# LabJunBMI/E3-invaraint-diffusion-model

Measured on AMD Instinct MI355X. Metric: denoising-steps/sec (batched pocket graphs), higher is better.
Workload: dtype f32 storage and accumulation, f16x3 products (fp32 grade); 1 GPU; structure_model sampling step, 256 x 256-residue pockets per GPU, 12+12 layers x 768, T=1000 schedule, encoder recomputed every step (as the reference); pockets_per_gpu=256, seq_len=256, parallelism=pocket-sharded x1, no collective

## Files before the change

e3-invaraint-diffusion-model_amd/blocks.py:

```python
import math

import torch
from torch import nn

import contextlib

from . import bert, keyed, ops
from .autograd import functional as F


class SELayer(nn.Module):

    def __init__(self, bert_config, mlp_ratio=4.0):
        super().__init__()
        h = bert_config.hidden_size
        self.norm1 = nn.LayerNorm(h, elementwise_affine=False)
        self.norm2 = nn.LayerNorm(h, elementwise_affine=False)
        self.adaLN_modulation = nn.Sequential(nn.Linear(h, h, bias=True), nn.SiLU(),
                                              nn.Linear(h, 6 * h, bias=True))
        self.attn = bert.BertAttention(bert_config)
        self.mlp = nn.Sequential(nn.Linear(h, int(h * mlp_ratio)), nn.GELU(),
                                 nn.Dropout(bert_config.hidden_dropout_prob),
                                 nn.Linear(int(h * mlp_ratio), h),
                                 nn.Dropout(bert_config.hidden_dropout_prob))
        nn.init.zeros_(self.adaLN_modulation[0].weight)
        nn.init.zeros_(self.adaLN_modulation[0].bias)

    def modulation(self, c):
        m0, m2 = self.adaLN_modulation[0], self.adaLN_modulation[2]
        return F.linear(F.linear(c, m0.weight, m0.bias, ops.ACT_SILU), m2.weight, m2.bias)

    def run(self, x, c, mask, B, L, mod=None, layout=None, row_keys=None):
        if mod is None:
            mod = self.modulation(c)
        if layout is not None:
            assert mod.shape[0] in (1, x.shape[0]), ("a packed batch takes per-token conditioning or one shared row",
                                                     tuple(mod.shape))
            assert bert.dropout_rates(self.attn) == (0.0, 0.0), "packed layouts are inference-only"
        rows_per_cond = x.shape[0] // mod.shape[0]
        assert rows_per_cond in (1, L, B * L) and rows_per_cond * mod.shape[0] == x.shape[0], (x.shape, mod.shape)
        drop = bert.dropout_rates(self.attn)
        if row_keys is not None:
            drop = drop + (row_keys,)
        att = bert.run_self_attention(self.attn, x, mask, B, L, drop, layout=layout)
        x = F.adaln_gate(x, att, mod, 0, rows_per_cond)
        h = F.dropout(F.linear(x, self.mlp[0].weight, self.mlp[0].bias, ops.ACT_GELU), self.mlp[2].p, self.training, row_keys)
        h = F.dropout(F.linear(h, self.mlp[3].weight, self.mlp[3].bias), self.mlp[4].p, self.training, row_keys)
        return F.adaln_gate(x, h, mod, 1, rows_per_cond)


class GaussianFourierProjection(nn.Module):

    def __init__(self, embed_dim=384, scale=2 * math.pi):
        super().__init__()
        self.register_buffer("W", torch.randn(embed_dim // 2) * scale)

    def forward(self, x):
        if x.ndim > 1:
            x = x.squeeze()
        elif x.ndim < 1:
            x = x.unsqueeze(0)
        if x.ndim < 1:
            x = x.unsqueeze(0)
        x_proj = x[:, None] * self.W[None, :] * 2 * torch.pi
        return torch.cat([torch.sin(x_proj), torch.cos(x_proj)], dim=-1)


class BertEmbeddings(nn.Module):

    def __init__(self, in_features, bert_config):
        super().__init__()
        self.linear = nn.Linear(in_features, bert_config.hidden_size)
        self.LayerNorm = nn.LayerNorm(bert_config.hidden_size, eps=bert_config.layer_norm_eps)
        self.dropout = nn.Dropout(bert_config.hidden_dropout_prob)

    def run(self, x2d, post_add=None, rows_per_add=1, row_keys=None):
        if self.training and self.dropout.p > 0:
            e = F.embed_layernorm(x2d, self.linear.weight, self.linear.bias, self.LayerNorm.weight,
                                  self.LayerNorm.bias, self.LayerNorm.eps, None, 1)
            e = F.dropout(e, self.dropout.p, row_keys=row_keys)
            if post_add is not None:
                e = (e.view(-1, rows_per_add, e.shape[1]) + post_add[:, None, :]).view_as(e)
            return e
        return F.embed_layernorm(x2d, self.linear.weight, self.linear.bias, self.LayerNorm.weight,
                                   self.LayerNorm.bias, self.LayerNorm.eps, post_add, rows_per_add)


class Predictor(nn.Module):

    def __init__(self, d_model, d_out, eps=1e-12):
        super().__init__()
        self.d_model, self.d_out = d_model, d_out
        self.dense1 = nn.Linear(d_model, d_model)
        self.layer_norm = nn.LayerNorm(d_model, eps=eps)
        self.dense2 = nn.Linear(d_model, d_out)

    def run(self, x):
        h = F.linear(x, self.dense1.weight, self.dense1.bias, ops.ACT_GELU)
        h = F.residual_layernorm(h, None, self.layer_norm.weight, self.layer_norm.bias, self.layer_norm.eps)
        return F.head_linear(h, self.dense2.weight, self.dense2.bias)


class KeyedDropoutSwitch:

    keyed_dropout = None

    def use_keyed_dropout(self, seed, epoch=None):
        if seed is None:
            self.keyed_dropout = None
            return None
        if epoch is None:
            epoch = keyed.epoch_word(next(self.parameters()).device)
        self.keyed_dropout = (keyed.check_seed(seed), epoch)
        return epoch

    def keyed_dropout_step(self, batch):
        cfgs = (self.encoder_config, self.decoder_config)
        acts = self.training and any(getattr(c, "hidden_dropout_prob", 0.0) > 0 or getattr(c, "attention_probs_dropout_prob", 0.0) > 0
                                     for c in cfgs)
        if self.keyed_dropout is None or not acts:
            return contextlib.nullcontext()
        seed, epoch = self.keyed_dropout
        return ops.keyed_dropout(seed, epoch, keyed.batch_item_ids(batch, batch["ligand_attn_mask"].shape[0]))


def drop_row_keys(stream, L):
    kd = ops.keyed_dropout_state()
    return None if kd is None else kd.row_keys(stream, L)


def flat2d(x):
    return x.reshape(-1, x.shape[-1]).contiguous().float()


def require_gpu(*tensors):
    for t in tensors:
        if t is not None and not t.is_cuda:
            raise RuntimeError("the denoiser runs on HIP kernels only: move the model and its inputs to a "
                               "GPU device (there is no CPU fallback; the CPU oracle lives in oracle/ and is "
                               "test infrastructure)")
```

e3-invaraint-diffusion-model_amd/csrc/gemm_split.hip:

```cpp
#include <type_traits>

#include "e3d_common.h"

namespace {

typedef __bf16 bf16x8 __attribute__((ext_vector_type(8)));
typedef __bf16 bf16x4 __attribute__((ext_vector_type(4)));
typedef _Float16 f16x8 __attribute__((ext_vector_type(8)));
typedef _Float16 f16x4 __attribute__((ext_vector_type(4)));

template <typename E> struct Vec;
template <> struct Vec<__bf16> { typedef bf16x8 x8; typedef bf16x4 x4; };
template <> struct Vec<_Float16> { typedef f16x8 x8; typedef f16x4 x4; };
__device__ __forceinline__ f32x16 mma16(const bf16x8 a, const bf16x8 b, const f32x16 c) {
    return __builtin_amdgcn_mfma_f32_32x32x16_bf16(a, b, c, 0, 0, 0);
}
__device__ __forceinline__ f32x16 mma16(const f16x8 a, const f16x8 b, const f32x16 c) {
    return __builtin_amdgcn_mfma_f32_32x32x16_f16(a, b, c, 0, 0, 0);
}

struct Epi { float* absmax; float scale; };

constexpr int BN = 128, BK = 32;
#ifdef GEMM_STAMPS
__device__ long long gemm_stamps[2][64][8];
#define GSTAMP(slot)                                                                                                    \
    do {                                                                                                                \
        if (stamp_on && kt < 64 && lane == 0) gemm_stamps[wid >> 2][kt][(slot)] = __builtin_readcyclecounter();         \
    } while (0)
#else
#define GSTAMP(slot) do {} while (0)
#endif
#ifndef E3D_GEMM_FRAG_PREFETCH
#define E3D_GEMM_FRAG_PREFETCH 1
#endif
constexpr int ROW_B = 64;
__device__ __forceinline__ int swz_off(int row, int chunk) { return row * ROW_B + ((chunk ^ ((row >> 2) & 3)) << 4); }

template <int NS, typename E>
__device__ __forceinline__ void split4(const f32x4 v, typename Vec<E>::x4 (&parts)[NS]) {
    f32x4 r = v;
#pragma unroll
    for (int s = 0; s < NS; ++s) {
#pragma unroll
        for (int j = 0; j < 4; ++j) {
            const E p = (E)r[j];
            parts[s][j] = p;
            r[j] -= (float)p;
        }
    }
}

template <>
__device__ __forceinline__ void split4<2, _Float16>(const f32x4 v, f16x4 (&parts)[2]) {
    e3d_f16x2 h0, l0, h1, l1;
    e3d_split2_f16(v[0], v[1], h0, l0);
    e3d_split2_f16(v[2], v[3], h1, l1);
    parts[0] = f16x4{h0[0], h0[1], h1[0], h1[1]};
    parts[1] = f16x4{l0[0], l0[1], l1[0], l1[1]};
}

#ifndef GEMM_LAB_RAW
#define GEMM_LAB_RAW 0
#endif
template <int ROWS, bool KMAJ, int NT = 512, bool RAW = false>
struct Stager {
    static constexpr int NV = ROWS * 8 / NT;
    const float* src[NV];
    int off[NV];
    int64_t ld;
    int kbase[NV];
    int roff[NV];

    __device__ __forceinline__ void init(const float* base, int64_t ld_, int row0, int row_limit, int tid) {
        ld = ld_;
#pragma unroll
        for (int i = 0; i < NV; ++i) {
            const int f = tid + NT * i;
            int r, kg;
            if (KMAJ) { r = f % ROWS; kg = f / ROWS; }
            else { r = f >> 3; kg = f & 7; }
            int gr = row0 + r;
            gr = gr < row_limit ? gr : row_limit - 1;
            src[i] = KMAJ ? base : base + (int64_t)gr * ld + kg * 4;
            kbase[i] = KMAJ ? __builtin_amdgcn_readfirstlane(kg * 4) : kg * 4;
            roff[i] = gr;
            off[i] = swz_off(r, kg >> 1) + (kg & 1) * 8;
        }
    }
    __device__ __forceinline__ void load(f32x4 (&v)[NV], int k0, int K) const {
#pragma unroll
        for (int i = 0; i < NV; ++i) {
            if (KMAJ) {
#pragma unroll
                for (int j = 0; j < 4; ++j) {
                    const int k = min(k0 + kbase[i] + j, K - 1);
                    v[i][j] = (src[i] + (int64_t)k * ld)[roff[i]];
                }
            } else {
                v[i] = *reinterpret_cast<const f32x4*>(src[i] + k0);
            }
        }
    }
    __device__ __forceinline__ void load_item(int i, f32x4& v, int k0, int K) const {
        if (KMAJ) {
#pragma unroll
            for (int j = 0; j < 4; ++j) {
                const int k = min(k0 + kbase[i] + j, K - 1);
                v[j] = (src[i] + (int64_t)k * ld)[roff[i]];
            }
        } else {
            v = *reinterpret_cast<const f32x4*>(src[i] + k0);
        }
    }
    template <int NS, typename E>
    __device__ __forceinline__ void store_item(int i, const f32x4& vin, unsigned char* img, int part_bytes, int k0, int K) const {
        f32x4 v = vin;
        if (KMAJ) {
#pragma unroll
            for (int j = 0; j < 4; ++j) v[j] = k0 + kbase[i] + j < K ? v[j] : 0.f;
        }
        typename Vec<E>::x4 p[NS];
        if constexpr (RAW && NS == 2) {
            typedef float f32x2_ __attribute__((ext_vector_type(2)));
            p[0] = __builtin_bit_cast(typename Vec<E>::x4, f32x2_{v[0], v[1]});
            p[1] = __builtin_bit_cast(typename Vec<E>::x4, f32x2_{v[2], v[3]});
        } else {
            split4<NS, E>(v, p);
        }
#pragma unroll
        for (int s = 0; s < NS; ++s) *reinterpret_cast<typename Vec<E>::x4*>(img + s * part_bytes + off[i]) = p[s];
    }
    __device__ __forceinline__ float masked_sum(int i, const f32x4& v, int k0, int K) const {
        float t[4];
#pragma unroll
        for (int j = 0; j < 4; ++j) t[j] = (!KMAJ || k0 + kbase[i] + j < K) ? v[j] : 0.f;
        return (t[0] + t[1]) + (t[2] + t[3]);
    }
    template <int NS, typename E>
    __device__ __forceinline__ void store(const f32x4 (&v)[NV], unsigned char* img, int part_bytes, int k0, int K) const {
#pragma unroll
        for (int i = 0; i < NV; ++i) store_item<NS, E>(i, v[i], img, part_bytes, k0, K);
    }
};

static inline bool e3d_tr_span_ok(int64_t k_len, int64_t ld) {
    return k_len > 0 && ld > 0 && ld < ((int64_t)1 << 24) && k_len * ld * 4 < ((int64_t)1 << 31);
}

template <int ROWS, int NT>
struct StagerT {
    static constexpr int NV = ROWS * 8 / NT;
    static constexpr int PITCH = ROWS * 2, Q = ROWS / 4, KSTEP = NT / Q;
    static_assert(KSTEP * NV == 32, "a k-tile is 32 k-rows");
    const float* ubase;
    int64_t ld;
    int kk0, n4, lim;
    int voff[NV];

    __device__ __forceinline__ void init(const float* base, int64_t ld_, int row0, int row_limit, int tid) {
        ld = ld_;
        ubase = base;
        lim = row_limit;
        n4 = tid % Q;
        kk0 = tid / Q;
        const int gr = min(row0 + 4 * n4, row_limit - 4);
#pragma unroll
        for (int i = 0; i < NV; ++i) voff[i] = (int)(((int64_t)kk(i) * ld + gr) * 4);
    }
    __device__ __forceinline__ int kk(int i) const { return kk0 + KSTEP * i; }
    __device__ __forceinline__ int off(int i) const {
        const int k = kk(i);
        return k * PITCH + (((n4 >> 2) ^ (2 * (k & 3))) << 5) + (n4 & 3) * 8;
    }
    __device__ __forceinline__ __amdgpu_buffer_rsrc_t tile_rsrc(int k0, int K) const {
        return __builtin_amdgcn_make_buffer_rsrc(const_cast<float*>(ubase + (int64_t)k0 * ld), 0,
                                                 (int)(((int64_t)(K - 1 - k0) * ld + lim) * 4), 0x00020000);
    }
    __device__ __forceinline__ void load_item(int i, f32x4& v, int k0, int K) const {
        v = __builtin_bit_cast(f32x4, __builtin_amdgcn_raw_buffer_load_b128(tile_rsrc(k0, K), voff[i], 0, 0));
    }
    __device__ __forceinline__ void load(f32x4 (&v)[NV], int k0, int K) const {
        const auto r = tile_rsrc(k0, K);
#pragma unroll
        for (int i = 0; i < NV; ++i) v[i] = __builtin_bit_cast(f32x4, __builtin_amdgcn_raw_buffer_load_b128(r, voff[i], 0, 0));
    }
    __device__ __forceinline__ f32x4 masked(int, const f32x4& v, int k0, int K) const { return k0 < K ? v : f32x4{0.f, 0.f, 0.f, 0.f}; }
    template <int NS, typename E>
    __device__ __forceinline__ void store_item(int i, const f32x4& v, unsigned char* img, int part_bytes, int, int) const {
        typename Vec<E>::x4 p[NS];
        split4<NS, E>(v, p);
        const int o = off(i);
#pragma unroll
        for (int s = 0; s < NS; ++s) *reinterpret_cast<typename Vec<E>::x4*>(img + s * part_bytes + o) = p[s];
    }
    template <int NS, typename E>
    __device__ __forceinline__ void store(const f32x4 (&v)[NV], unsigned char* img, int part_bytes, int k0, int K) const {
#pragma unroll
        for (int i = 0; i < NV; ++i) store_item<NS, E>(i, v[i], img, part_bytes, k0, K);
    }
    __device__ __forceinline__ float masked_sum(int, const f32x4&, int, int) const { return 0.f; }
};

__device__ __forceinline__ int tr_lane_off(int pitch, int r0, int lane) {
    const int q = (lane >> 2) & 3, g = (lane >> 4) & 1, half = lane >> 5;
    return (4 * half + q) * pitch + ((((r0 >> 4) + g) ^ (2 * q)) << 5) + 8 * (lane & 3);
}
template <typename X8>
__device__ __forceinline__ X8 tr_frag8(const unsigned char* img, int pitch, int lane_off, int ks) {
    typedef short short4v __attribute__((ext_vector_type(4)));
    typedef short short8v __attribute__((ext_vector_type(8)));
    typedef __attribute__((address_space(3))) short4v* lds_p;
    const unsigned char* p0 = img + 16 * ks * pitch + lane_off;
    const short4v a = __builtin_amdgcn_ds_read_tr16_b64_v4i16((lds_p)(p0));
    const short4v b = __builtin_amdgcn_ds_read_tr16_b64_v4i16((lds_p)(p0 + 8 * pitch));
    const short8v c = __builtin_shufflevector(a, b, 0, 1, 2, 3, 4, 5, 6, 7);
    return __builtin_bit_cast(X8, c);
}

template <int NS, int ACT, bool A_KMAJ, bool B_KMAJ, int WM, int WN, typename E, int TN = 2, bool TR = false>
__device__ __forceinline__ void gemm_split_body(unsigned char* smem_raw, const float* __restrict__ A, int64_t lda,
                                                const float* __restrict__ Bm, int64_t ldb,
                                                const float* __restrict__ bias, float* __restrict__ out, int64_t ldc,
                                                int M, int N, int K_total, int tiles_m, int tiles_n, int k_chunk,
                                                int bx, int by, int ny, float* __restrict__ colsum_out, int accumulate,
                                                float* __restrict__ absmax = nullptr, float out_scale = 1.0f) {
    constexpr int NBUF = NS <= 2 ? 2 : 1;
    constexpr int BM = WM * 64, BN = WN * 32 * TN, NT = WM * WN * 64;
    constexpr int A_BYTES = BM * ROW_B, B_BYTES = BN * ROW_B;
    constexpr int BUF_BYTES = NS * (A_BYTES + B_BYTES);

    const int k_begin = by * k_chunk;
    const int K = min(K_total, k_begin + k_chunk);
    const bool split = ny > 1;
    const int lid = bx;
    const int tm = lid / tiles_n, tn = lid % tiles_n;
    const int row0 = tm * BM, col0 = tn * BN;

    const int tid = threadIdx.x, lane = tid & 63, wid = tid >> 6;
    const int wr = wid / WN, wc = wid % WN;
    const int l31 = lane & 31, half = lane >> 5;

    static_assert(!TR || (A_KMAJ && B_KMAJ), "the transposing staging exists for the K-major x K-major layout");
    typedef typename std::conditional<TR, StagerT<BM, NT>, Stager<BM, A_KMAJ, NT, (GEMM_LAB_RAW & 1) && !A_KMAJ && !B_KMAJ>>::type SA;
    typedef typename std::conditional<TR, StagerT<BN, NT>, Stager<BN, B_KMAJ, NT, (GEMM_LAB_RAW & 2) && !A_KMAJ && !B_KMAJ>>::type SB;
    SA sa;
    SB sb;
    sa.init(A, lda, row0, M, tid);
    sb.init(Bm, ldb, col0, N, tid);

    f32x16 acc[2][TN];
#pragma unroll
    for (int m = 0; m < 2; ++m)
#pragma unroll
        for (int n = 0; n < TN; ++n)
#pragma unroll
            for (int r = 0; r < 16; ++r) acc[m][n][r] = 0.f;

    f32x4 ra[SA::NV], rb[SB::NV];
    f32x4 ra1[SA::NV], rb1[SB::NV];
    constexpr bool CS = A_KMAJ && B_KMAJ;
    float cs[SA::NV];
    f32x4 cs4 = {0.f, 0.f, 0.f, 0.f};
#pragma unroll
    for (int i = 0; i < SA::NV; ++i) cs[i] = 0.f;
    auto cs_add = [&](int i, const f32x4& v, int k0) {
        if constexpr (TR) cs4 += sa.masked(i, v, k0, K);
        else cs[i] += sa.masked_sum(i, v, k0, K);
    };
    sa.load(ra, k_begin, K);
    sb.load(rb, k_begin, K);
    if (CS) {
#pragma unroll
        for (int i = 0; i < SA::NV; ++i) cs_add(i, ra[i], k_begin);
    }
    sa.template store<NS, E>(ra, smem_raw, A_BYTES, k_begin, K);
    sb.template store<NS, E>(rb, smem_raw + NS * A_BYTES, B_BYTES, k_begin, K);
    __syncthreads();

    const int nk = (K - k_begin + BK - 1) / BK;
    const int a_row = wr * 64 + l31, b_row = wc * (32 * TN) + l31;
    int cur = 0;
    constexpr bool PIPE = NBUF == 2;
    constexpr int NA_ = SA::NV, NB_ = SB::NV;
    constexpr bool DEEP = PIPE && ((!A_KMAJ && !B_KMAJ) || TR);
    int tr_a[2], tr_b[TN];
    if constexpr (TR) {
#pragma unroll
        for (int m = 0; m < 2; ++m) tr_a[m] = tr_lane_off(2 * BM, wr * 64 + 32 * m, lane);
#pragma unroll
        for (int n = 0; n < TN; ++n) tr_b[n] = tr_lane_off(2 * BN, wc * (32 * TN) + 32 * n, lane);
    }
    if (DEEP) {
        const int k1 = k_begin + (nk > 1 ? BK : 0), k2 = k_begin + (nk > 2 ? 2 : (nk > 1 ? 1 : 0)) * BK;
        sa.load(ra1, k1, K);
        sb.load(rb1, k1, K);
        sa.load(ra, k2, K);
        sb.load(rb, k2, K);
    } else if (PIPE) {
        const int k1 = k_begin + (nk > 1 ? BK : 0);
        sa.load(ra, k1, K);
        sb.load(rb, k1, K);
    }
#ifdef GEMM_STAMPS
    const bool stamp_on = bx == GEMM_STAMPS && by == 0 && (wid & 3) == 0;
#endif
    auto k_step = [&](int kt, f32x4 (&xa)[NA_], f32x4 (&xb)[NB_]) {
        const bool more = kt + 1 < nk;
        GSTAMP(0);
        if (!PIPE && more) {
            sa.load(xa, k_begin + (kt + 1) * BK, K);
            sb.load(xb, k_begin + (kt + 1) * BK, K);
        }
        constexpr int AHEAD = DEEP ? 3 : 2;
        const int k2 = k_begin + (kt + AHEAD < nk ? kt + AHEAD : nk - 1) * BK;
        unsigned char* nxt = smem_raw + (cur ^ 1) * BUF_BYTES;
        const unsigned char* ab = smem_raw + cur * BUF_BYTES;
        const unsigned char* bb = smem_raw + cur * BUF_BYTES + NS * A_BYTES;
        constexpr bool PREF = PIPE && TN == 1 && E3D_GEMM_FRAG_PREFETCH;
        typename Vec<E>::x8 fa2[2][NS][2], fb2[2][NS][TN];
#pragma unroll
        for (int ks = 0; ks < (PREF ? 2 : 0); ++ks)
#pragma unroll
            for (int s = 0; s < NS; ++s) {
#pragma unroll
                for (int m = 0; m < 2; ++m)
                    fa2[ks][s][m] = *reinterpret_cast<const typename Vec<E>::x8*>(ab + s * A_BYTES + swz_off(a_row + 32 * m, 2 * ks + half));
#pragma unroll
                for (int n = 0; n < TN; ++n)
                    fb2[ks][s][n] = *reinterpret_cast<const typename Vec<E>::x8*>(bb + s * B_BYTES + swz_off(b_row + 32 * n, 2 * ks + half));
            }
#ifdef GEMM_STAMPS
        if (PREF) { asm volatile("s_waitcnt lgkmcnt(0)" ::: "memory"); GSTAMP(1); }
#endif
#pragma unroll
        for (int ks = 0; ks < 2; ++ks) {
            typename Vec<E>::x8 fa[NS][2], fb[NS][TN];
#pragma unroll
            for (int s = 0; s < NS; ++s) {
#pragma unroll
                for (int m = 0; m < 2; ++m) {
                    if constexpr (TR) fa[s][m] = tr_frag8<typename Vec<E>::x8>(ab + s * A_BYTES, 2 * BM, tr_a[m], ks);
                    else fa[s][m] = PREF ? fa2[ks][s][m]
                                         : *reinterpret_cast<const typename Vec<E>::x8*>(ab + s * A_BYTES + swz_off(a_row + 32 * m, 2 * ks + half));
                }
#pragma unroll
                for (int n = 0; n < TN; ++n) {
                    if constexpr (TR) fb[s][n] = tr_frag8<typename Vec<E>::x8>(bb + s * B_BYTES, 2 * BN, tr_b[n], ks);
                    else fb[s][n] = PREF ? fb2[ks][s][n]
                                         : *reinterpret_cast<const typename Vec<E>::x8*>(bb + s * B_BYTES + swz_off(b_row + 32 * n, 2 * ks + half));
                }
            }
#pragma unroll
            for (int m = 0; m < 2; ++m) {
                if (PIPE) {
                    const int g = ks * 2 + m;
#pragma unroll
                    for (int i = 0; i < NA_; ++i)
                        if (i * 4 / NA_ == g) {
                            if (CS) cs_add(i, xa[i], k_begin + (kt + 1) * BK);
                            sa.template store_item<NS, E>(i, xa[i], nxt, A_BYTES, k_begin + (kt + 1) * BK, K);
                            sa.load_item(i, xa[i], k2, K);
                        }
#pragma unroll
                    for (int i = 0; i < NB_; ++i)
                        if (i * 4 / NB_ == g) {
                            sb.template store_item<NS, E>(i, xb[i], nxt + NS * A_BYTES, B_BYTES, k_begin + (kt + 1) * BK, K);
                            sb.load_item(i, xb[i], k2, K);
                        }
                }
#pragma unroll
                for (int n = 0; n < TN; ++n) {
                    if constexpr (NS == 3) {
                        acc[m][n] = mma16(fa[1][m], fb[1][n], acc[m][n]);
                        acc[m][n] = mma16(fa[0][m], fb[NS - 1][n], acc[m][n]);
                        acc[m][n] = mma16(fa[NS - 1][m], fb[0][n], acc[m][n]);
                    }
                    if constexpr (NS >= 2) {
                        acc[m][n] = mma16(fa[0][m], fb[1][n], acc[m][n]);
                        acc[m][n] = mma16(fa[1][m], fb[0][n], acc[m][n]);
                    }
                    acc[m][n] = mma16(fa[0][m], fb[0][n], acc[m][n]);
                }
                if (PIPE) __builtin_amdgcn_sched_barrier(0);
            }
        }
        GSTAMP(2);
        if (PIPE) {
#ifdef GEMM_STAMPS
            asm volatile("s_waitcnt vmcnt(0) lgkmcnt(0)" ::: "memory");
            GSTAMP(3);
#endif
            __syncthreads();
            GSTAMP(4);
            cur ^= 1;
        } else {
            __syncthreads();
            if (more) {
                if (CS) {
#pragma unroll
                    for (int i = 0; i < SA::NV; ++i) cs_add(i, xa[i], k_begin + (kt + 1) * BK);
                }
                sa.template store<NS, E>(xa, smem_raw, A_BYTES, k_begin + (kt + 1) * BK, K);
                sb.template store<NS, E>(xb, smem_raw + NS * A_BYTES, B_BYTES, k_begin + (kt + 1) * BK, K);
            }
            __syncthreads();
        }
        };
    for (int kt = 0; kt < nk; kt += 2) {
        if constexpr (DEEP) {
            k_step(kt, ra1, rb1);
            if (kt + 1 < nk) k_step(kt + 1, ra, rb);
        } else {
            k_step(kt, ra, rb);
            if (kt + 1 < nk) k_step(kt + 1, ra, rb);
        }
    }
    unsigned amax = 0;
#pragma unroll
    for (int n = 0; n < TN; ++n) {
        const int col = col0 + wc * (32 * TN) + n * 32 + l31;
        const float bv = (bias && col < N && by == 0) ? bias[col] : 0.f;
#pragma unroll
        for (int m = 0; m < 2; ++m) {
#pragma unroll
            for (int r = 0; r < 16; ++r) {
                const int row = row0 + wr * 64 + m * 32 + mfma32_row(r, half);
                float v = fmaf(acc[m][n][r], out_scale, bv);
                if (ACT == E3D_ACT_GELU) v = gelu_erf(v);
                if (ACT == E3D_ACT_SILU) v = silu(v);
                if (row < M && col < N) {
                    float* o = out + (int64_t)row * ldc + col;
                    if (split) atomicAdd(o, v);
                    else *o = accumulate ? *o + v : v;
                    if (ACT == E3D_ACT_NONE && absmax) e3d_absmax_accum(amax, v);
                }
            }
        }
    }
    if (ACT == E3D_ACT_NONE && absmax) e3d_absmax_commit(amax, absmax, lane);
    if (CS && colsum_out && tn == 0) {
        float* red = reinterpret_cast<float*>(smem_raw);
        if constexpr (TR) {
            static_assert(SA::KSTEP == 8, "8 partial sums per row, as in the dword scheme");
#pragma unroll
            for (int j = 0; j < 4; ++j) red[sa.kk0 * BM + 4 * sa.n4 + j] = cs4[j];
        } else {
#pragma unroll
            for (int i = 0; i < SA::NV; ++i) {
                const int f = tid + NT * i;
                red[(f / BM) * BM + f % BM] = cs[i];
            }
        }
        __syncthreads();
        if (tid < BM && row0 + tid < M) {
            float v = 0.f;
#pragma unroll
            for (int g = 0; g < 8; ++g) v += red[g * BM + tid];
            float* o = colsum_out + row0 + tid;
            if (split) atomicAdd(o, v);
            else *o = accumulate ? *o + v : v;
        }
    }
}

template <int NS, int ACT, bool A_KMAJ, bool B_KMAJ, int WM, int WN, typename E, int TN = 2, bool TR = false>
__global__ __launch_bounds__(WM * WN * 64) void gemm_split_kernel(const float* __restrict__ A, int64_t lda,
                                                         const float* __restrict__ Bm, int64_t ldb,
                                                         const float* __restrict__ bias,
                                                         float* __restrict__ out, int64_t ldc, int M,
                                                         int N, int K_total, int tiles_m, int tiles_n,
                                                         int k_chunk, float* __restrict__ absmax, float out_scale) {
    extern __shared__ __attribute__((aligned(16))) unsigned char smem_raw[];
    gemm_split_body<NS, ACT, A_KMAJ, B_KMAJ, WM, WN, E, TN, TR>(smem_raw, A, lda, Bm, ldb, bias, out, ldc, M, N, K_total, tiles_m,
                                                        tiles_n, k_chunk, xcd_remap(blockIdx.x, tiles_m * tiles_n),
                                                        blockIdx.y, gridDim.y, nullptr, 0, absmax, out_scale);
}

struct WgradGroup {
    const float* dz[64];
    const float* x[64];
    float* dw[64];
    float* db[64];
    unsigned long long accumulate;
};

template <int NS, bool TR>
__global__ __launch_bounds__(512) void gemm_wgrad_grouped_kernel(const WgradGroup g, int64_t ldz, int64_t ldx, int N, int K,
                                                                 int M, int tiles_m, int tiles_n, int count) {
    extern __shared__ __attribute__((aligned(16))) unsigned char smem_raw[];
    const int tiles = tiles_m * tiles_n;
    const int lid = xcd_remap(blockIdx.x, tiles * count);
    const int p = lid / tiles;
    gemm_split_body<NS, E3D_ACT_NONE, true, true, 4, 2, __bf16, 2, TR>(smem_raw, g.dz[p], ldz, g.x[p], ldx, nullptr, g.dw[p], K,
                                                                        N, K, M, tiles_m, tiles_n, M, lid - p * tiles, 0, 1,
                                                                        g.db[p], (int)((g.accumulate >> p) & 1));
}

struct WgradRagged {
    const float* dz[64];
    const float* x[64];
    float* dw[64];
    float* db[64];
    int N[64], K[64], ldz[64], ldx[64];
    int tile_start[65];
    unsigned long long accumulate;
};
static_assert(sizeof(WgradRagged) <= 3400, "kernel arguments are limited to 4 KB");

template <int NS, bool TR>
__global__ __launch_bounds__(512) void gemm_wgrad_ragged_kernel(const WgradRagged g, int M, int count) {
    extern __shared__ __attribute__((aligned(16))) unsigned char smem_raw[];
    const int lid = xcd_remap(blockIdx.x, g.tile_start[count]);
    int lo = 0, hi = count;
    while (hi - lo > 1) {
        const int mid = (lo + hi) >> 1;
        if (g.tile_start[mid] <= lid) lo = mid;
        else hi = mid;
    }
    const int p = lo, N = g.N[p], K = g.K[p];
    const int tiles_m = (N + 255) / 256, tiles_n = (K + 127) / 128;
    gemm_split_body<NS, E3D_ACT_NONE, true, true, 4, 2, __bf16, 2, TR>(smem_raw, g.dz[p], (int64_t)g.ldz[p], g.x[p], (int64_t)g.ldx[p],
                                                                        nullptr, g.dw[p], K, N, K, M, tiles_m, tiles_n, M,
                                                                        lid - g.tile_start[p], 0, 1, g.db[p],
                                                                        (int)((g.accumulate >> p) & 1));
}

constexpr int BT = 256, ROW64 = ROW_B;

#ifdef E3D_STAMPS
__device__ long long e3d_stamps[2][32][8];
#define STAMP(slot)                                                                              \
    do {                                                                                         \
        if (stamp_on && kt < 32 && lane == 0) e3d_stamps[wr][kt][slot] = __builtin_readcyclecounter(); \
    } while (0)
#define STAMP_K(i)                                                                               \
    do {                                                                                         \
        if (blockIdx.x == 300 && (threadIdx.x & 255) == 0) e3d_stamps[threadIdx.x >> 8][i][7] = __builtin_readcyclecounter(); \
    } while (0)
#else
#define STAMP(slot) do {} while (0)
#define STAMP_K(i) do {} while (0)
#endif

template <int NS, int ACT, int WR, int WC, int NBUF, bool PIPE, typename E>
__global__ __launch_bounds__(WR * WC * 64, 2) void gemm_split256_kernel(const float* __restrict__ A, int64_t lda,
                                                                        const float* __restrict__ W,
                                                                        const float* __restrict__ bias,
                                                                        float* __restrict__ out, int64_t ldc,
                                                                        int M, int N, int K, int tiles_m,
                                                                        int tiles_n, float* __restrict__ absmax, float out_scale) {
    static_assert(!PIPE || NBUF == 2, "PIPE needs two LDS buffers");
    STAMP_K(0);
    extern __shared__ __attribute__((aligned(16))) unsigned char smem_raw[];
    constexpr int NT = WR * WC * 64, TM = WR * 128, TN = WC * 64;
    constexpr int A_BYTES = TM * ROW64, B_BYTES = TN * ROW64;
    constexpr int BUF_BYTES = NS * (A_BYTES + B_BYTES);
    constexpr int NA = TM * 8 / NT, NB = TN * 8 / NT;
    constexpr int NI = NA + NB;

    const int lid = xcd_remap(blockIdx.x, tiles_m * tiles_n);
    const int tm = lid / tiles_n, tn = lid % tiles_n;
    const int row0 = tm * TM, col0 = tn * TN;
    const int tid = threadIdx.x, lane = tid & 63, wid = tid >> 6;
    const int wr = wid / WC, wc = wid % WC;
    const int l31 = lane & 31, half = lane >> 5;

    const float* src[NI];
    int dst[NI];
#pragma unroll
    for (int i = 0; i < NI; ++i) {
        const bool is_a = i < NA;
        const int f = tid + NT * (is_a ? i : i - NA), r = f >> 3, kg = f & 7;
        if (is_a) {
            int ar = row0 + r;
            ar = ar < M ? ar : M - 1;
            src[i] = A + (int64_t)ar * lda + kg * 4;
        } else {
            src[i] = W + (int64_t)(col0 + r) * K + kg * 4;
        }
        dst[i] = (is_a ? 0 : NS * A_BYTES) + swz_off(r, kg >> 1) + (kg & 1) * 8;
    }

    f32x16 acc[4][2];
#pragma unroll
    for (int m = 0; m < 4; ++m)
#pragma unroll
        for (int n = 0; n < 2; ++n)
#pragma unroll
            for (int r = 0; r < 16; ++r) acc[m][n][r] = 0.f;

    f32x4 rg[NI];
    auto item_load = [&](int i, int kt) { rg[i] = *reinterpret_cast<const f32x4*>(src[i] + kt * BK); };
    auto item_store = [&](int i, unsigned char* buf) {
        typename Vec<E>::x4 p[NS];
        split4<NS, E>(rg[i], p);
#pragma unroll
        for (int s = 0; s < NS; ++s)
            *reinterpret_cast<typename Vec<E>::x4*>(buf + s * (i < NA ? A_BYTES : B_BYTES) + dst[i]) = p[s];
    };

    STAMP_K(1);
    const int nk = K / BK;
#pragma unroll
    for (int i = 0; i < NI; ++i) item_load(i, 0);
#pragma unroll
    for (int i = 0; i < NI; ++i) item_store(i, smem_raw);
    if (PIPE) {
#pragma unroll
        for (int i = 0; i < NI; ++i) item_load(i, nk > 1 ? 1 : 0);
    }
    __syncthreads();

    int a_row[4], b_row[2];
#pragma unroll
    for (int m = 0; m < 4; ++m) a_row[m] = wr * 128 + m * 32 + l31;
#pragma unroll
    for (int n = 0; n < 2; ++n) b_row[n] = wc * 64 + n * 32 + l31;
    STAMP_K(2);
    int cur = 0;
#ifdef E3D_STAMPS
    const bool stamp_on = blockIdx.x == 300 && (wid & 3) == 0;
#endif
    for (int kt = 0; kt < nk; ++kt) {
        const bool more = kt + 1 < nk;
        STAMP(0);
        if (!PIPE && more) {
#pragma unroll
            for (int i = 0; i < NI; ++i) item_load(i, kt + 1);
        }
        STAMP(1);
        const unsigned char* base = smem_raw + cur * BUF_BYTES;
        unsigned char* next = smem_raw + (cur ^ 1) * BUF_BYTES;
        const int kt2 = kt + 2 < nk ? kt + 2 : nk - 1;
#pragma unroll
        for (int ks = 0; ks < 2; ++ks) {
            typename Vec<E>::x8 fa[NS][4], fb[NS][2];
#pragma unroll
            for (int s = 0; s < NS; ++s) {
#pragma unroll
                for (int n = 0; n < 2; ++n)
                    fb[s][n] = *reinterpret_cast<const typename Vec<E>::x8*>(base + NS * A_BYTES + s * B_BYTES +
                                                                swz_off(b_row[n], 2 * ks + half));
#pragma unroll
                for (int m = 0; m < 4; ++m)
                    fa[s][m] = *reinterpret_cast<const typename Vec<E>::x8*>(base + s * A_BYTES + swz_off(a_row[m], 2 * ks + half));
            }
#pragma unroll
            for (int m = 0; m < 4; ++m) {
                if (PIPE) {
                    const int g = ks * 4 + m;
#pragma unroll
                    for (int i = 0; i < NI; ++i)
                        if (i * 8 / NI == g) {
                            item_store(i, next);
                            item_load(i, kt2);
                        }
                }
#pragma unroll
                for (int n = 0; n < 2; ++n) {
                    if constexpr (NS == 3) {
                        acc[m][n] = mma16(fa[1][m], fb[1][n], acc[m][n]);
                        acc[m][n] = mma16(fa[0][m], fb[NS - 1][n], acc[m][n]);
                        acc[m][n] = mma16(fa[NS - 1][m], fb[0][n], acc[m][n]);
                    }
                    if constexpr (NS >= 2) {
                        acc[m][n] = mma16(fa[0][m], fb[1][n], acc[m][n]);
                        acc[m][n] = mma16(fa[1][m], fb[0][n], acc[m][n]);
                    }
                    acc[m][n] = mma16(fa[0][m], fb[0][n], acc[m][n]);
                }
                if (PIPE) __builtin_amdgcn_sched_barrier(0);
            }
            STAMP(2 + ks);
        }
        if (PIPE) {
            STAMP(5);
            __syncthreads();
            STAMP(6);
            cur ^= 1;
        } else if (NBUF == 2) {
#ifdef E3D_STAMPS
            asm volatile("s_waitcnt vmcnt(0)" ::: "memory");
            STAMP(4);
#endif
            if (more) {
#pragma unroll
                for (int i = 0; i < NI; ++i) item_store(i, next);
            }
            STAMP(5);
            __syncthreads();
            STAMP(6);
            cur ^= 1;
        } else {
            __syncthreads();
            if (more) {
#pragma unroll
                for (int i = 0; i < NI; ++i) item_store(i, smem_raw);
            }
            __syncthreads();
        }
    }

    STAMP_K(3);
    unsigned amax = 0;
#pragma unroll
    for (int m = 0; m < 4; ++m) {
#pragma unroll
        for (int n = 0; n < 2; ++n) {
            const int col = col0 + wc * 64 + n * 32 + l31;
            const float bv = bias ? bias[col] : 0.f;
#pragma unroll
            for (int r = 0; r < 16; ++r) {
                const int row = row0 + wr * 128 + m * 32 + mfma32_row(r, half);
                float v = fmaf(acc[m][n][r], out_scale, bv);
                if (ACT == E3D_ACT_GELU) v = gelu_erf(v);
                if (ACT == E3D_ACT_SILU) v = silu(v);
                if (row < M) {
                    out[(int64_t)row * ldc + col] = v;
                    if (ACT == E3D_ACT_NONE && absmax) e3d_absmax_accum(amax, v);
                }
            }
        }
    }
    if (ACT == E3D_ACT_NONE && absmax) e3d_absmax_commit(amax, absmax, lane);
    STAMP_K(4);
#ifdef E3D_STAMPS
    asm volatile("s_waitcnt vmcnt(0)" ::: "memory");
    STAMP_K(5);
#endif
}

#ifdef E3D_NT_STORES
#define E3D_STORE_OUT(ptr, val) __builtin_nontemporal_store((val), (ptr))
#else
#define E3D_STORE_OUT(ptr, val) (*(ptr) = (val))
#endif

template <int ACT, typename E>
__global__ __launch_bounds__(512, 2) void gemm_split256p_kernel(const float* __restrict__ A, int64_t lda,
                                                                 const float* __restrict__ W,
                                                                 const float* __restrict__ bias,
                                                                 float* __restrict__ out, int64_t ldc, int N, int K,
                                                                 int tiles_m, int tiles_n, float* __restrict__ absmax, float out_scale) {
    extern __shared__ __attribute__((aligned(16))) unsigned char smem_raw[];
    constexpr int NS = 2, T_BYTES = BT * ROW64, BUF_BYTES = 2 * NS * T_BYTES;
    constexpr int NI = 8;
    const int total = tiles_m * tiles_n, nk = K / BK;
    const int tid = threadIdx.x, lane = tid & 63, wid = tid >> 6;
    const int wr = wid >> 2, wc = wid & 3;
    const int l31 = lane & 31, half = lane >> 5;

    unsigned goff[NI];
    int dst[NI];
#pragma unroll
    for (int i = 0; i < NI; ++i) {
        const int f = tid + 512 * (i & 3), r = f >> 3, kg = f & 7;
        goff[i] = (unsigned)(r * (i < 4 ? (int)lda : K) + kg * 4);
        dst[i] = (i < 4 ? 0 : NS * T_BYTES) + swz_off(r, kg >> 1) + (kg & 1) * 8;
    }

    int ld_tile = blockIdx.x, ld_k = 0;
    const float* ld_a;
    const float* ld_w;
    auto cursor_bases = [&]() {
        const int lid = xcd_remap(ld_tile, total);
        ld_a = A + (int64_t)(lid / tiles_n) * BT * lda + ld_k * BK;
        ld_w = W + (int64_t)(lid % tiles_n) * BT * K + ld_k * BK;
    };
    auto cursor_advance = [&]() {
        if (ld_k + 1 < nk) {
            ++ld_k;
            ld_a += BK;
            ld_w += BK;
        } else if (ld_tile + (int)gridDim.x < total) {
            ld_tile += gridDim.x;
            ld_k = 0;
            cursor_bases();
        }
    };
    f32x4 rg[NI];
    auto item_load = [&](int i) { rg[i] = *reinterpret_cast<const f32x4*>((i < 4 ? ld_a : ld_w) + goff[i]); };
    auto item_store = [&](int i, unsigned char* buf) {
        typename Vec<E>::x4 p[NS];
        split4<NS, E>(rg[i], p);
#pragma unroll
        for (int s = 0; s < NS; ++s) *reinterpret_cast<typename Vec<E>::x4*>(buf + s * T_BYTES + dst[i]) = p[s];
    };
    cursor_bases();
#pragma unroll
    for (int i = 0; i < NI; ++i) item_load(i);
    cursor_advance();
#pragma unroll
    for (int i = 0; i < NI; ++i) item_store(i, smem_raw);
#pragma unroll
    for (int i = 0; i < NI; ++i) item_load(i);
    cursor_advance();
    __syncthreads();

    int a_row[4], b_row[2];
#pragma unroll
    for (int m = 0; m < 4; ++m) a_row[m] = wr * 128 + m * 32 + l31;
#pragma unroll
    for (int n = 0; n < 2; ++n) b_row[n] = wc * 64 + n * 32 + l31;
    int cur = 0;
    unsigned amax = 0;

    for (int tile = blockIdx.x; tile < total; tile += gridDim.x) {
        f32x16 acc[4][2];
#pragma unroll
        for (int m = 0; m < 4; ++m)
#pragma unroll
            for (int n = 0; n < 2; ++n)
#pragma unroll
                for (int r = 0; r < 16; ++r) acc[m][n][r] = 0.f;
        for (int kt = 0; kt < nk; ++kt) {
            const unsigned char* base = smem_raw + cur * BUF_BYTES;
            unsigned char* next = smem_raw + (cur ^ 1) * BUF_BYTES;
#pragma unroll
            for (int ks = 0; ks < 2; ++ks) {
                typename Vec<E>::x8 fa[NS][4], fb[NS][2];
#pragma unroll
                for (int s = 0; s < NS; ++s) {
#pragma unroll
                    for (int n = 0; n < 2; ++n)
                        fb[s][n] = *reinterpret_cast<const typename Vec<E>::x8*>(base + (NS + s) * T_BYTES +
                                                                    swz_off(b_row[n], 2 * ks + half));
#pragma unroll
                    for (int m = 0; m < 4; ++m)
                        fa[s][m] = *reinterpret_cast<const typename Vec<E>::x8*>(base + s * T_BYTES + swz_off(a_row[m], 2 * ks + half));
                }
#pragma unroll
                for (int m = 0; m < 4; ++m) {
                    const int g = ks * 4 + m;
                    item_store(g, next);
                    item_load(g);
#pragma unroll
                    for (int n = 0; n < 2; ++n) {
                        acc[m][n] = mma16(fa[0][m], fb[1][n], acc[m][n]);
                        acc[m][n] = mma16(fa[1][m], fb[0][n], acc[m][n]);
                        acc[m][n] = mma16(fa[0][m], fb[0][n], acc[m][n]);
                    }
                    __builtin_amdgcn_sched_barrier(0);
                }
            }
            cursor_advance();
            __syncthreads();
            cur ^= 1;
        }

        const int lid = xcd_remap(tile, total);
        const int row0 = (lid / tiles_n) * BT, col0 = (lid % tiles_n) * BT;
#pragma unroll
        for (int m = 0; m < 4; ++m) {
#pragma unroll
            for (int n = 0; n < 2; ++n) {
                const int col = col0 + wc * 64 + n * 32 + l31;
                const float bv = bias ? bias[col] : 0.f;
                float* o = out + (int64_t)(row0 + wr * 128 + m * 32 + 4 * half) * ldc + col;
#pragma unroll
                for (int r = 0; r < 16; ++r) {
                    float v = fmaf(acc[m][n][r], out_scale, bv);
                    if (ACT == E3D_ACT_GELU) v = gelu_erf(v);
                    if (ACT == E3D_ACT_SILU) v = silu(v);
                    E3D_STORE_OUT(&o[(int64_t)((r & 3) + 8 * (r >> 2)) * ldc], v);
                    if (ACT == E3D_ACT_NONE && absmax) e3d_absmax_accum(amax, v);
                }
            }
        }
    }
    if (ACT == E3D_ACT_NONE && absmax) e3d_absmax_commit(amax, absmax, lane);
}

template <int ACT, typename E>
int launch256p(const float* A, int64_t lda, const float* W, const float* bias, float* out, int64_t ldc, int M, int N,
               int K, Epi epi, hipStream_t s) {
    const int tiles_m = M / BT, tiles_n = N / BT;
    constexpr size_t lds = 2 * 2 * 2 * BT * ROW64;
    static std::atomic<uint64_t> lds_ok{0};
    const int n_cu = e3d_cu_count();
    const int total = tiles_m * tiles_n;
    e3d_allow_lds(lds_ok, gemm_split256p_kernel<ACT, E>, lds);
    hipLaunchKernelGGL((gemm_split256p_kernel<ACT, E>), dim3(total < n_cu ? total : n_cu), dim3(512), lds, s, A, lda, W, bias, out,
                       ldc, N, K, tiles_m, tiles_n, epi.absmax, epi.scale);
    return e3d_launch_status("e3d_gemm_f32_split (persistent 256x256)");
}

int g_general_form = -1;
int g_tile_pref = -1;

template <int NS, int ACT, int WR, int WC, int NBUF, bool PIPE, typename E>
int launch256(const float* A, int64_t lda, const float* W, const float* bias, float* out, int64_t ldc, int M, int N,
              int K, Epi epi, hipStream_t s) {
    constexpr int TM = WR * 128, TN = WC * 64;
    const int tiles_m = (M + TM - 1) / TM, tiles_n = N / TN;
    const size_t lds = (size_t)NBUF * NS * (TM + TN) * ROW64;
    static std::atomic<uint64_t> lds_ok{0};
    e3d_allow_lds(lds_ok, gemm_split256_kernel<NS, ACT, WR, WC, NBUF, PIPE, E>, lds);
    hipLaunchKernelGGL((gemm_split256_kernel<NS, ACT, WR, WC, NBUF, PIPE, E>), dim3(tiles_m * tiles_n), dim3(WR * WC * 64), lds, s,
                       A, lda, W, bias, out, ldc, M, N, K, tiles_m, tiles_n, epi.absmax, epi.scale);
    return e3d_launch_status("e3d_gemm_f32_split (128x64 wave tiles)");
}

template <int NS, int ACT, bool A_KMAJ, bool B_KMAJ, int WM, int WN, typename E, int TN = 2, bool TR = false>
int launch_general(const float* A, int64_t lda, const float* B, int64_t ldb, const float* bias, float* out, int64_t ldc,
                   int M, int N, int K, Epi epi, hipStream_t s);

int p_min() {
    static int v = 0;
    if (!v) {
        const char* e = getenv("E3D_GEMM_P_MIN");
        v = e ? atoi(e) : 160;
    }
    return v;
}

template <int NS, int ACT, bool A_KMAJ, bool B_KMAJ, typename E>
int launch(const float* A, int64_t lda, const float* B, int64_t ldb, const float* bias, float* out, int64_t ldc,
           int M, int N, int K, Epi epi, hipStream_t s) {
    if (g_tile_pref < 0) {
        const char* e = getenv("E3D_GEMM_TILE");
        g_tile_pref = e ? atoi(e) : 4;
    }
    if constexpr (!A_KMAJ && !B_KMAJ) {
        if constexpr (NS == 2) {
            const int64_t n_tiles = (int64_t)(M / BT) * (N / BT);
            if (N % BT == 0 && M % BT == 0 && ldb == K && g_tile_pref >= 4 && K >= 2 * BK && lda < (1 << 22) &&
                (g_tile_pref >= 5 || n_tiles >= p_min() || (n_tiles >= 96 && N >= 6 * BT && !getenv("E3D_GEMM_P_MIN"))))
                return launch256p<ACT, E>(A, lda, B, bias, out, ldc, M, N, K, epi, s);
            if (N % BT == 0 && ldb == K && g_tile_pref >= 3 && (int64_t)((M + BT - 1) / BT) * (N / BT) >= 256)
                return launch256<NS, ACT, 2, 4, 2, true, E>(A, lda, B, bias, out, ldc, M, N, K, epi, s);
        }
        if constexpr (NS == 1) {
            if (N % BT == 0 && ldb == K && g_tile_pref >= 3 && (int64_t)((M + BT - 1) / BT) * (N / BT) >= 160)
                return launch256<NS, ACT, 2, 4, 2, true, E>(A, lda, B, bias, out, ldc, M, N, K, epi, s);
        }
        if (N % BT == 0 && ldb == K && g_tile_pref >= 1 &&
            (int64_t)((M + BT - 1) / BT) * (N / BT) >= 256)
            return launch256<NS, ACT, 2, 4, (NS <= 2 ? 2 : 1), false, E>(A, lda, B, bias, out, ldc, M, N, K, epi, s);
    }
    if (g_general_form < 0) {
        const char* e = getenv("E3D_GEMM_FORM");
        g_general_form = e ? atoi(e) : 0;
    }
    int form = g_general_form;
    if (form != 1 && form != 2 && form != 3 && form != 4) {
        const int64_t g256 = (int64_t)((M + 255) / 256) * ((N + 127) / 128), g128 = (int64_t)((M + 127) / 128) * ((N + 127) / 128);
        const int64_t cus = e3d_cu_count();
        if (NS == 3) form = g256 < 128 && !A_KMAJ && !B_KMAJ ? 2 : 1;
        else if (A_KMAJ && B_KMAJ) form = 1;
        else if (A_KMAJ) form = g128 <= cus ? 2 : (g256 <= cus ? 1 : (45 * ((g128 + 2 * cus - 1) / (2 * cus)) < 37 * ((g256 + cus - 1) / cus) ? 2 : 1));
        else form = 25 * ((g128 + cus - 1) / cus) <= 38 * ((g256 + cus - 1) / cus) ? 3 : 1;
        if (NS == 2 && !A_KMAJ && !B_KMAJ && M <= 2048 && N <= 1024) form = 4;
    }
    if constexpr (NS == 2 && !A_KMAJ && !B_KMAJ) {
        if (form == 4) return launch_general<NS, ACT, A_KMAJ, B_KMAJ, 2, 2, E, 1>(A, lda, B, ldb, bias, out, ldc, M, N, K, epi, s);
    }
    if (form == 4) form = 3;
    if constexpr (NS <= 2 && !A_KMAJ) {
        if (form == 3) return launch_general<NS, ACT, A_KMAJ, B_KMAJ, 2, 4, E, 1>(A, lda, B, ldb, bias, out, ldc, M, N, K, epi, s);
    }
    if (form == 3) form = 2;
    if (form == 2) return launch_general<NS, ACT, A_KMAJ, B_KMAJ, 2, 2, E>(A, lda, B, ldb, bias, out, ldc, M, N, K, epi, s);
    if constexpr (A_KMAJ && B_KMAJ) {
        static const bool tr_on = !getenv("E3D_WGRAD_TR") || atoi(getenv("E3D_WGRAD_TR")) != 0;
        if (tr_on && M % 4 == 0 && N % 4 == 0 && lda % 4 == 0 && ldb % 4 == 0 && ((uintptr_t)A % 16) == 0 && ((uintptr_t)B % 16) == 0 &&
            e3d_tr_span_ok(K, lda) && e3d_tr_span_ok(K, ldb))
            return launch_general<NS, ACT, A_KMAJ, B_KMAJ, 4, 2, E, 2, true>(A, lda, B, ldb, bias, out, ldc, M, N, K, epi, s);
    }
    return launch_general<NS, ACT, A_KMAJ, B_KMAJ, 4, 2, E>(A, lda, B, ldb, bias, out, ldc, M, N, K, epi, s);
}

template <int NS, int ACT, bool A_KMAJ, bool B_KMAJ, int WM, int WN, typename E, int TN, bool TR>
int launch_general(const float* A, int64_t lda, const float* B, int64_t ldb, const float* bias, float* out, int64_t ldc,
                   int M, int N, int K, Epi epi, hipStream_t s) {
    constexpr int BM = WM * 64, BNt = WN * 32 * TN;
    const int tiles_m = (M + BM - 1) / BM, tiles_n = (N + BNt - 1) / BNt;
    constexpr int NBUF = NS <= 2 ? 2 : 1;
    size_t lds = (size_t)NBUF * NS * (BM + BNt) * ROW_B;
    static const bool spread = !getenv("E3D_GEMM_SPREAD") || atoi(getenv("E3D_GEMM_SPREAD")) != 0;
    if (spread && BM * BNt == 128 * 128 && (int64_t)tiles_m * tiles_n <= e3d_cu_count() && lds < (size_t)84 * 1024) lds = (size_t)84 * 1024;
    static std::atomic<uint64_t> lds_ok{0};
    e3d_allow_lds(lds_ok, gemm_split_kernel<NS, ACT, A_KMAJ, B_KMAJ, WM, WN, E, TN, TR>, (size_t)84 * 1024 > lds ? (size_t)84 * 1024 : lds);
    int splits = 1;
    const int resident = e3d_cu_count() * (WM * WN >= 8 ? 1 : 2);
    if (A_KMAJ && B_KMAJ && ACT == E3D_ACT_NONE && tiles_m * tiles_n * 2 < resident && K >= 1024) {
        splits = resident / (tiles_m * tiles_n);
        splits = splits > 16 ? 16 : splits;
        while (splits > 1 && K / splits < 256) --splits;
    }
    int k_chunk = K;
    if (splits > 1) {
        k_chunk = ((K + splits - 1) / splits + BK - 1) / BK * BK;
        splits = (K + k_chunk - 1) / k_chunk;
        hipError_t e = hipSuccess;
        if (ldc == N) e = e3d_zero_async(out, (size_t)M * N, s);
        else {
            hipLaunchKernelGGL(e3d_zero2d_kernel, dim3(1024), dim3(256), 0, s, out, (size_t)ldc, (size_t)M, (size_t)N);
            e = hipGetLastError();
        }
        if (e != hipSuccess) {
            e3d_set_error("gemm_split: split-K memset failed: %s", hipGetErrorString(e));
            return (int)e;
        }
    }
    hipLaunchKernelGGL((gemm_split_kernel<NS, ACT, A_KMAJ, B_KMAJ, WM, WN, E, TN, TR>), dim3(tiles_m * tiles_n, splits),
                       dim3(WM * WN * 64), lds, s, A, lda, B, ldb, bias, out, ldc, M, N, K, tiles_m, tiles_n, k_chunk,
                       splits > 1 ? nullptr : epi.absmax, epi.scale);
    return e3d_launch_status("e3d_gemm_f32_split");
}

template <int NS, typename E>
int dispatch(int act, bool a_kmaj, bool b_kmaj, const float* A, int64_t lda, const float* B, int64_t ldb,
             const float* bias, float* out, int64_t ldc, int M, int N, int K, Epi epi, hipStream_t s) {
    if (!a_kmaj && !b_kmaj) {
        switch (act) {
            case E3D_ACT_NONE: return launch<NS, E3D_ACT_NONE, false, false, E>(A, lda, B, ldb, bias, out, ldc, M, N, K, epi, s);
            case E3D_ACT_GELU: return launch<NS, E3D_ACT_GELU, false, false, E>(A, lda, B, ldb, bias, out, ldc, M, N, K, epi, s);
            case E3D_ACT_SILU: return launch<NS, E3D_ACT_SILU, false, false, E>(A, lda, B, ldb, bias, out, ldc, M, N, K, epi, s);
        }
        e3d_set_error("gemm_split: unknown activation %d", act);
        return -1;
    }
    if (act != E3D_ACT_NONE) {
        e3d_set_error("gemm_split: activations are only fused for the forward (K-contiguous) layout");
        return -1;
    }
    if (!a_kmaj && b_kmaj) return launch<NS, E3D_ACT_NONE, false, true, __bf16>(A, lda, B, ldb, bias, out, ldc, M, N, K, epi, s);
    if (a_kmaj && b_kmaj) return launch<NS, E3D_ACT_NONE, true, true, __bf16>(A, lda, B, ldb, bias, out, ldc, M, N, K, Epi{nullptr, epi.scale}, s);
    return launch<NS, E3D_ACT_NONE, true, false, __bf16>(A, lda, B, ldb, bias, out, ldc, M, N, K, epi, s);
}

}

#ifdef GEMM_STAMPS
extern "C" int e3d_debug_gemm_stamps(long long* t) { return (int)hipMemcpyFromSymbol(t, HIP_SYMBOL(gemm_stamps), sizeof(long long) * 2 * 64 * 8); }
#endif

#ifdef E3D_STAMPS
extern "C" int e3d_debug_read_stamps(long long* host_out) {
    return (int)hipMemcpyFromSymbol(host_out, HIP_SYMBOL(e3d_stamps), sizeof(long long) * 2 * 32 * 8);
}
#endif

extern "C" int e3d_gemm_kernel_select(int pref) {
    if (g_tile_pref < 0) {
        const char* e = getenv("E3D_GEMM_TILE");
        g_tile_pref = e ? atoi(e) : 4;
    }
    const int prev = g_tile_pref;
    if (pref >= 0) g_tile_pref = pref;
    return prev;
}

extern "C" int e3d_gemm_general_select(int form) {
    if (g_general_form < 0) {
        const char* e = getenv("E3D_GEMM_FORM");
        g_general_form = e ? atoi(e) : 0;
    }
    const int prev = g_general_form;
    if (form >= 0) g_general_form = form;
    return prev;
}

static int gemm_split_general(const float* A, int64_t lda, int a_kmajor, const float* B, int64_t ldb, int b_kmajor,
                              const float* bias, float* out, int64_t ldc, int M, int N, int K, int act, int terms,
                              float* absmax, float out_scale, void* stream) {
    const Epi epi{absmax, out_scale};
    E3D_REQUIRE(out_scale == 1.0f || !(a_kmajor && b_kmajor), "gemm_split: out_scale is not available for the split-K layout");
    E3D_REQUIRE(A && B && out, "gemm_split: null pointer");
    E3D_REQUIRE(M > 0 && N > 0 && K > 0, "gemm_split: bad shape M=%d N=%d K=%d", M, N, K);
    E3D_REQUIRE(terms == E3D_TERMS_BF16 || terms == 3 || terms == 6 || terms == E3D_TERMS_F16X3,
                "gemm_split: terms must be 1, 3, 6 or 19 (got %d)", terms);
    E3D_REQUIRE(ldc >= N, "gemm_split: ldc=%lld < N=%d", (long long)ldc, N);
    if (!a_kmajor) E3D_REQUIRE(lda >= K && lda % 4 == 0 && K % BK == 0 && ((uintptr_t)A % 16) == 0,
                               "gemm_split: K-contiguous A needs K%%32==0, lda%%4==0, 16B alignment (K=%d lda=%lld)", K, (long long)lda);
    else E3D_REQUIRE(lda >= M, "gemm_split: K-major A needs lda >= M");
    if (!b_kmajor) E3D_REQUIRE(ldb >= K && ldb % 4 == 0 && K % BK == 0 && ((uintptr_t)B % 16) == 0,
                               "gemm_split: K-contiguous B needs K%%32==0, ldb%%4==0, 16B alignment (K=%d ldb=%lld)", K, (long long)ldb);
    else E3D_REQUIRE(ldb >= N, "gemm_split: K-major B needs ldb >= N");
    hipStream_t s = (hipStream_t)stream;
    E3D_REQUIRE(!absmax || (!(a_kmajor && b_kmajor) && act == E3D_ACT_NONE),
                "gemm_split: out_absmax exists for act = none and not for the split-K (weight-gradient) layout");
    if (terms == E3D_TERMS_BF16) return dispatch<1, __bf16>(act, a_kmajor != 0, b_kmajor != 0, A, lda, B, ldb, bias, out, ldc, M, N, K, epi, s);
    if (terms == 3) return dispatch<2, __bf16>(act, a_kmajor != 0, b_kmajor != 0, A, lda, B, ldb, bias, out, ldc, M, N, K, epi, s);
    if (terms == E3D_TERMS_F16X3) {
        if (!a_kmajor && !b_kmajor) return dispatch<2, _Float16>(act, false, false, A, lda, B, ldb, bias, out, ldc, M, N, K, epi, s);
        return dispatch<3, __bf16>(act, a_kmajor != 0, b_kmajor != 0, A, lda, B, ldb, bias, out, ldc, M, N, K, epi, s);
    }
    return dispatch<3, __bf16>(act, a_kmajor != 0, b_kmajor != 0, A, lda, B, ldb, bias, out, ldc, M, N, K, epi, s);
}

extern "C" int e3d_gemm_f32_split_general(const float* A, int64_t lda, int a_kmajor, const float* B,
                                          int64_t ldb, int b_kmajor, const float* bias, float* out,
                                          int64_t ldc, int M, int N, int K, int act, int terms,
                                          void* stream) {
    return gemm_split_general(A, lda, a_kmajor, B, ldb, b_kmajor, bias, out, ldc, M, N, K, act, terms, nullptr, 1.0f, stream);
}

extern "C" int e3d_gemm_wgrad_grouped_f32_split(const float* const* dz, const float* const* x, float* const* dw,
                                                float* const* db, uint64_t accumulate_bits, int count, int64_t ldz,
                                                int64_t ldx, int N, int K, int M, int terms, void* stream) {
    E3D_REQUIRE(dz && x && dw && count >= 1 && count <= 64, "gemm_wgrad_grouped: 1..64 problems (count=%d)", count);
    E3D_REQUIRE(M > 0 && N > 0 && K > 0 && ldz >= N && ldx >= K, "gemm_wgrad_grouped: bad shape N=%d K=%d M=%d ldz=%lld ldx=%lld",
                N, K, M, (long long)ldz, (long long)ldx);
    E3D_REQUIRE(terms == E3D_TERMS_BF16 || terms == 3 || terms == 6 || terms == E3D_TERMS_F16X3,
                "gemm_wgrad_grouped: terms must be 1, 3, 6 or 19 (got %d)", terms);
    WgradGroup g;
    for (int p = 0; p < 64; ++p) {
        const int q = p < count ? p : 0;
        E3D_REQUIRE(dz[q] && x[q] && dw[q], "gemm_wgrad_grouped: null pointer in problem %d", q);
        g.dz[p] = dz[q]; g.x[p] = x[q]; g.dw[p] = dw[q]; g.db[p] = db ? db[q] : nullptr;
    }
    g.accumulate = accumulate_bits;
    static const bool tr_on = !getenv("E3D_WGRAD_TR") || atoi(getenv("E3D_WGRAD_TR")) != 0;
    bool tr = tr_on && N % 4 == 0 && K % 4 == 0 && ldz % 4 == 0 && ldx % 4 == 0 && e3d_tr_span_ok(M, ldz) && e3d_tr_span_ok(M, ldx);
    for (int p = 0; p < count && tr; ++p) tr = ((uintptr_t)dz[p] % 16) == 0 && ((uintptr_t)x[p] % 16) == 0;
    const int tiles_m = (N + 255) / 256, tiles_n = (K + 127) / 128;
    E3D_REQUIRE((int64_t)tiles_m * tiles_n * count < (1ll << 30), "gemm_wgrad_grouped: too many tiles");
    const dim3 grid(tiles_m * tiles_n * count), block(512);
    hipStream_t s = (hipStream_t)stream;
    auto go = [&](auto kern, size_t lds, std::atomic<uint64_t>& lds_ok) {
        e3d_allow_lds(lds_ok, kern, lds);
        hipLaunchKernelGGL(kern, grid, block, lds, s, g, ldz, ldx, N, K, M, tiles_m, tiles_n, count);
    };
    static std::atomic<uint64_t> ok1{0}, ok1t{0}, ok2{0}, ok2t{0}, ok3{0}, ok3t{0};
    if (terms == E3D_TERMS_BF16) {
        const size_t lds = (size_t)2 * 1 * (256 + 128) * ROW_B;
        if (tr) go(gemm_wgrad_grouped_kernel<1, true>, lds, ok1t);
        else go(gemm_wgrad_grouped_kernel<1, false>, lds, ok1);
    } else if (terms == 3) {
        const size_t lds = (size_t)2 * 2 * (256 + 128) * ROW_B;
        if (tr) go(gemm_wgrad_grouped_kernel<2, true>, lds, ok2t);
        else go(gemm_wgrad_grouped_kernel<2, false>, lds, ok2);
    } else {
        const size_t lds = (size_t)1 * 3 * (256 + 128) * ROW_B;
        if (tr) go(gemm_wgrad_grouped_kernel<3, true>, lds, ok3t);
        else go(gemm_wgrad_grouped_kernel<3, false>, lds, ok3);
    }
    return e3d_launch_status("e3d_gemm_wgrad_grouped_f32_split");
}

extern "C" int e3d_gemm_wgrad_ragged_f32_split(const float* const* dz, const float* const* x, float* const* dw, float* const* db,
                                               const int* N, const int* K, const int64_t* ldz, const int64_t* ldx,
                                               uint64_t accumulate_bits, int count, int M, int terms, void* stream) {
    E3D_REQUIRE(dz && x && dw && N && K && ldz && ldx && count >= 1 && count <= 64, "gemm_wgrad_ragged: 1..64 problems (count=%d)", count);
    E3D_REQUIRE(M > 0, "gemm_wgrad_ragged: bad token count %d", M);
    E3D_REQUIRE(terms == E3D_TERMS_BF16 || terms == 3 || terms == 6 || terms == E3D_TERMS_F16X3,
                "gemm_wgrad_ragged: terms must be 1, 3, 6 or 19 (got %d)", terms);
    WgradRagged g;
    static const bool tr_on = !getenv("E3D_WGRAD_TR") || atoi(getenv("E3D_WGRAD_TR")) != 0;
    bool tr = tr_on;
    int64_t tiles = 0;
    for (int p = 0; p < 64; ++p) {
        const int q = p < count ? p : 0;
        E3D_REQUIRE(dz[q] && x[q] && dw[q], "gemm_wgrad_ragged: null pointer in problem %d", q);
        E3D_REQUIRE(N[q] > 0 && K[q] > 0 && ldz[q] >= N[q] && ldx[q] >= K[q] && ldz[q] < (1ll << 31) && ldx[q] < (1ll << 31),
                    "gemm_wgrad_ragged: bad shape in problem %d: N=%d K=%d ldz=%lld ldx=%lld", q, N[q], K[q], (long long)ldz[q],
                    (long long)ldx[q]);
        g.dz[p] = dz[q]; g.x[p] = x[q]; g.dw[p] = dw[q]; g.db[p] = db ? db[q] : nullptr;
        g.N[p] = N[q]; g.K[p] = K[q]; g.ldz[p] = (int)ldz[q]; g.ldx[p] = (int)ldx[q];
        g.tile_start[p] = (int)tiles;
        if (p < count) {
            tiles += (int64_t)((N[q] + 255) / 256) * ((K[q] + 127) / 128);
            tr = tr && N[q] % 4 == 0 && K[q] % 4 == 0 && ldz[q] % 4 == 0 && ldx[q] % 4 == 0 && ((uintptr_t)dz[q] % 16) == 0 &&
                 ((uintptr_t)x[q] % 16) == 0 && e3d_tr_span_ok(M, ldz[q]) && e3d_tr_span_ok(M, ldx[q]);
        }
    }
    E3D_REQUIRE(tiles < (1ll << 30), "gemm_wgrad_ragged: too many tiles");
    for (int p = count; p <= 64; ++p) g.tile_start[p] = (int)tiles;
    g.accumulate = accumulate_bits;
    const dim3 grid((unsigned)tiles), block(512);
    hipStream_t s = (hipStream_t)stream;
    auto go = [&](auto kern, size_t lds, std::atomic<uint64_t>& lds_ok) {
        e3d_allow_lds(lds_ok, kern, lds);
        hipLaunchKernelGGL(kern, grid, block, lds, s, g, M, count);
    };
    static std::atomic<uint64_t> ok1{0}, ok1t{0}, ok2{0}, ok2t{0}, ok3{0}, ok3t{0};
    if (terms == E3D_TERMS_BF16) {
        const size_t lds = (size_t)2 * 1 * (256 + 128) * ROW_B;
        if (tr) go(gemm_wgrad_ragged_kernel<1, true>, lds, ok1t);
        else go(gemm_wgrad_ragged_kernel<1, false>, lds, ok1);
    } else if (terms == 3) {
        const size_t lds = (size_t)2 * 2 * (256 + 128) * ROW_B;
        if (tr) go(gemm_wgrad_ragged_kernel<2, true>, lds, ok2t);
        else go(gemm_wgrad_ragged_kernel<2, false>, lds, ok2);
    } else {
        const size_t lds = (size_t)1 * 3 * (256 + 128) * ROW_B;
        if (tr) go(gemm_wgrad_ragged_kernel<3, true>, lds, ok3t);
        else go(gemm_wgrad_ragged_kernel<3, false>, lds, ok3);
    }
    return e3d_launch_status("e3d_gemm_wgrad_ragged_f32_split");
}

extern "C" int e3d_gemm_bias_act_f32_split(const float* A, int64_t lda, const float* W,
                                           const float* bias, float* out, int64_t ldc, int M,
                                           int N, int K, int act, int terms, void* stream) {
    E3D_REQUIRE(N % BN == 0, "gemm_split: need N%%128==0 (N=%d)", N);
    return gemm_split_general(A, lda, 0, W, (int64_t)K, 0, bias, out, ldc, M, N, K, act, terms, nullptr, 1.0f, stream);
}

extern "C" int e3d_gemm_bias_act_f32_split_ex(const float* A, int64_t lda, const float* W, const float* bias, float* out,
                                              int64_t ldc, int M, int N, int K, int act, int terms, float* out_absmax,
                                              float out_scale, void* stream) {
    E3D_REQUIRE(N % BN == 0, "gemm_split: need N%%128==0 (N=%d)", N);
    return gemm_split_general(A, lda, 0, W, (int64_t)K, 0, bias, out, ldc, M, N, K, act, terms, out_absmax, out_scale, stream);
}
```

e3-invaraint-diffusion-model_amd/csrc/rowops.hip:

```cpp
#include "e3d_common.h"

namespace {

template <int V>
__device__ __forceinline__ void row_load(f32x4 (&r)[V], const float* p, int lane) {
#pragma unroll
    for (int i = 0; i < V; ++i) r[i] = *reinterpret_cast<const f32x4*>(p + 4 * (64 * i + lane));
}

template <int V>
__device__ __forceinline__ void row_store(const f32x4 (&r)[V], float* p, int lane) {
#pragma unroll
    for (int i = 0; i < V; ++i) *reinterpret_cast<f32x4*>(p + 4 * (64 * i + lane)) = r[i];
}

template <int V>
__device__ __forceinline__ void row_normalize(f32x4 (&r)[V], float eps) {
    constexpr float inv_h = 1.0f / (256 * V);
    float s = 0.f;
#pragma unroll
    for (int i = 0; i < V; ++i) s += (r[i][0] + r[i][1]) + (r[i][2] + r[i][3]);
    const float mean = wave_sum(s) * inv_h;
    float ss = 0.f;
#pragma unroll
    for (int i = 0; i < V; ++i)
#pragma unroll
        for (int j = 0; j < 4; ++j) {
            r[i][j] -= mean;
            ss += r[i][j] * r[i][j];
        }
    const float rstd = 1.0f / sqrtf(wave_sum(ss) * inv_h + eps);
#pragma unroll
    for (int i = 0; i < V; ++i) r[i] *= rstd;
}

template <int V, bool DROP = false, bool KEYED = false>
__global__ __launch_bounds__(256) void residual_layernorm_kernel(
    const float* __restrict__ x, const float* __restrict__ res, const float* __restrict__ gamma,
    const float* __restrict__ beta, float eps, float* __restrict__ s_out, float* __restrict__ out, int M, E3dDrop drop_in = E3dDrop{}) {
    constexpr int H = 256 * V;
    const int lane = threadIdx.x & 63;
    const int row = blockIdx.x * 4 + (threadIdx.x >> 6);
    if (row >= M) return;
    f32x4 r[V], t[V];
    row_load<V>(r, x + (int64_t)row * H, lane);
    if (DROP) {
        const E3dDrop drop = e3d_drop_resolve(drop_in);
        const uint64_t key_term = KEYED ? e3d_drop_hidden_row(drop, row, H / 4) : 0;
#pragma unroll
        for (int i = 0; i < V; ++i) {
            float m[4];
            if (KEYED) e3d_drop_mult4_row(drop, key_term, 64 * i + lane, m);
            else e3d_drop_mult4(drop, (uint64_t)row * (H / 4) + 64 * i + lane, m);
#pragma unroll
            for (int j = 0; j < 4; ++j) r[i][j] *= m[j];
        }
    }
    if (res) {
        row_load<V>(t, res + (int64_t)row * H, lane);
#pragma unroll
        for (int i = 0; i < V; ++i) r[i] += t[i];
    }
    if (s_out) row_store<V>(r, s_out + (int64_t)row * H, lane);
    row_normalize<V>(r, eps);
    f32x4 g[V], b[V];
    row_load<V>(g, gamma, lane);
    row_load<V>(b, beta, lane);
#pragma unroll
    for (int i = 0; i < V; ++i) r[i] = r[i] * g[i] + b[i];
    row_store<V>(r, out + (int64_t)row * H, lane);
}

template <int V>
__global__ __launch_bounds__(256) void adaln_gate_kernel(const float* __restrict__ x,
                                                         const float* __restrict__ y,
                                                         const float* __restrict__ mod, int branch,
                                                         int rows_per_cond, float* __restrict__ out,
                                                         int M) {
    constexpr int H = 256 * V;
    const int lane = threadIdx.x & 63;
    const int row = blockIdx.x * 4 + (threadIdx.x >> 6);
    if (row >= M) return;
    f32x4 r[V], xr[V], sh[V], sc[V], ga[V];
    row_load<V>(r, y + (int64_t)row * H, lane);
    row_normalize<V>(r, 1e-5f);
    const float* mrow = mod + (int64_t)(row / rows_per_cond) * 6 * H + (int64_t)branch * 3 * H;
    row_load<V>(sh, mrow, lane);
    row_load<V>(sc, mrow + H, lane);
    row_load<V>(ga, mrow + 2 * H, lane);
    row_load<V>(xr, x + (int64_t)row * H, lane);
#pragma unroll
    for (int i = 0; i < V; ++i) r[i] = xr[i] + ga[i] * (r[i] * (1.0f + sc[i]) + sh[i]);
    row_store<V>(r, out + (int64_t)row * H, lane);
}

template <int V>
__global__ __launch_bounds__(256) void embed_layernorm_kernel(
    const float* __restrict__ x, int F, const float* __restrict__ W, const float* __restrict__ bias,
    const float* __restrict__ gamma, const float* __restrict__ beta, float eps,
    const float* __restrict__ post_add, int rows_per_add, float* __restrict__ z_out,
    float* __restrict__ out, int M) {
    constexpr int H = 256 * V;
    extern __shared__ __attribute__((aligned(16))) float wt[];
    for (int i = threadIdx.x; i < H * F; i += blockDim.x) wt[(i % F) * H + i / F] = W[i];
    __syncthreads();
    const int lane = threadIdx.x & 63;
    const int wave = blockIdx.x * 4 + (threadIdx.x >> 6), n_waves = gridDim.x * 4;
    f32x4 g[V], b[V], bs[V];
    row_load<V>(g, gamma, lane);
    row_load<V>(b, beta, lane);
    row_load<V>(bs, bias, lane);
    constexpr int R = 4;
    for (int row0 = wave * R; row0 < M; row0 += n_waves * R) {
        const float* xr[R];
#pragma unroll
        for (int k = 0; k < R; ++k) xr[k] = x + (int64_t)min(row0 + k, M - 1) * F;
        f32x4 r[R][V];
#pragma unroll
        for (int k = 0; k < R; ++k)
#pragma unroll
            for (int i = 0; i < V; ++i) r[k][i] = bs[i];
        for (int f = 0; f < F; ++f) {
            float xv[R];
#pragma unroll
            for (int k = 0; k < R; ++k) xv[k] = xr[k][f];
#pragma unroll
            for (int i = 0; i < V; ++i) {
                const f32x4 w = *reinterpret_cast<const f32x4*>(wt + f * H + 4 * (64 * i + lane));
#pragma unroll
                for (int k = 0; k < R; ++k)
#pragma unroll
                    for (int j = 0; j < 4; ++j) r[k][i][j] = __builtin_fmaf(xv[k], w[j], r[k][i][j]);
            }
        }
#pragma unroll
        for (int k = 0; k < R; ++k) {
            const int row = row0 + k;
            if (row >= M) break;
            if (z_out) row_store<V>(r[k], z_out + (int64_t)row * H, lane);
            row_normalize<V>(r[k], eps);
#pragma unroll
            for (int i = 0; i < V; ++i) r[k][i] = r[k][i] * g[i] + b[i];
            if (post_add) {
                f32x4 a[V];
                row_load<V>(a, post_add + (int64_t)(row / rows_per_add) * H, lane);
#pragma unroll
                for (int i = 0; i < V; ++i) r[k][i] += a[i];
            }
            row_store<V>(r[k], out + (int64_t)row * H, lane);
        }
    }
}

template <int V>
__global__ __launch_bounds__(256) void embed_layernorm_rows_kernel(
    const float* __restrict__ x, int F, const float* __restrict__ W, const float* __restrict__ bias,
    const float* __restrict__ gamma, const float* __restrict__ beta, float eps,
    const float* __restrict__ post_add, int rows_per_add, float* __restrict__ z_out,
    float* __restrict__ out, int M) {
    constexpr int H = 256 * V;
    const int lane = threadIdx.x & 63;
    const int row = blockIdx.x * 4 + (threadIdx.x >> 6);
    if (row >= M) return;
    const float* xr = x + (int64_t)row * F;
    f32x4 r[V], g[V], b[V];
    row_load<V>(r, bias, lane);
    row_load<V>(g, gamma, lane);
    row_load<V>(b, beta, lane);
    if ((F & 3) == 0 && ((((uintptr_t)x | (uintptr_t)W) & 15) == 0)) {
        for (int f0 = 0; f0 < F; f0 += 4) {
            const f32x4 xv = *reinterpret_cast<const f32x4*>(xr + f0);
#pragma unroll
            for (int i = 0; i < V; ++i)
#pragma unroll
                for (int j = 0; j < 4; ++j) {
                    const f32x4 w = *reinterpret_cast<const f32x4*>(W + (int64_t)(4 * (64 * i + lane) + j) * F + f0);
#pragma unroll
                    for (int q = 0; q < 4; ++q) r[i][j] = __builtin_fmaf(xv[q], w[q], r[i][j]);
                }
        }
    } else {
        for (int f = 0; f < F; ++f) {
            const float xv = xr[f];
#pragma unroll
            for (int i = 0; i < V; ++i)
#pragma unroll
                for (int j = 0; j < 4; ++j) r[i][j] = __builtin_fmaf(xv, W[(int64_t)(4 * (64 * i + lane) + j) * F + f], r[i][j]);
        }
    }
    if (z_out) row_store<V>(r, z_out + (int64_t)row * H, lane);
    row_normalize<V>(r, eps);
#pragma unroll
    for (int i = 0; i < V; ++i) r[i] = r[i] * g[i] + b[i];
    if (post_add) {
        f32x4 a[V];
        row_load<V>(a, post_add + (int64_t)(row / rows_per_add) * H, lane);
#pragma unroll
        for (int i = 0; i < V; ++i) r[i] += a[i];
    }
    row_store<V>(r, out + (int64_t)row * H, lane);
}

template <int V>
__global__ __launch_bounds__(256) void head_linear_kernel(const float* __restrict__ x,
                                                          const float* __restrict__ W,
                                                          const float* __restrict__ b,
                                                          float* __restrict__ out, int M, int Nout) {
    constexpr int H = 256 * V;
    const int lane = threadIdx.x & 63;
    const int row = blockIdx.x * 4 + (threadIdx.x >> 6);
    if (row >= M) return;
    f32x4 r[V];
    row_load<V>(r, x + (int64_t)row * H, lane);
    float mine = 0.f;
    for (int n = 0; n < Nout; ++n) {
        f32x4 w[V];
        row_load<V>(w, W + (int64_t)n * H, lane);
        float s = 0.f;
#pragma unroll
        for (int i = 0; i < V; ++i)
#pragma unroll
            for (int j = 0; j < 4; ++j) s = fmaf(r[i][j], w[i][j], s);
        s = wave_sum(s);
        if (lane == n) mine = s + b[n];
    }
    if (lane < Nout) out[(int64_t)row * Nout + lane] = mine;
}

#define DISPATCH_V(H, CALL)                                             \
    switch (H) {                                                        \
        case 256: { constexpr int V = 1; CALL; } break;                 \
        case 512: { constexpr int V = 2; CALL; } break;                 \
        case 768: { constexpr int V = 3; CALL; } break;                 \
        case 1024: { constexpr int V = 4; CALL; } break;                \
        default: E3D_REQUIRE(false, "row op: H must be 256/512/768/1024 (H=%d)", H); \
    }

}

extern "C" int e3d_residual_layernorm_fwd(const float* x, const float* residual,
                                          const float* gamma, const float* beta, float eps,
                                          float* s_out, float* out, int M, int H, void* stream) {
    E3D_REQUIRE(x && gamma && beta && out && M > 0, "residual_layernorm: bad arguments");
    const dim3 grid((M + 3) / 4), block(256);
    DISPATCH_V(H, hipLaunchKernelGGL(residual_layernorm_kernel<V>, grid, block, 0, (hipStream_t)stream, x,
                                     residual, gamma, beta, eps, s_out, out, M));
    return e3d_launch_status("e3d_residual_layernorm_fwd");
}

extern "C" int e3d_residual_layernorm_drop_fwd(const float* x, const float* residual, const float* gamma, const float* beta,
                                               float eps, float* s_out, float* out, int M, int H, float drop_p, uint64_t drop_seed,
                                               void* stream) {
    E3D_REQUIRE(x && gamma && beta && out && M > 0, "residual_layernorm_drop: bad arguments");
    E3D_REQUIRE(drop_p >= 0.f && drop_p < 1.f, "residual_layernorm_drop: p = %f", (double)drop_p);
    const dim3 grid((M + 3) / 4), block(256);
    const E3dDrop d = e3d_drop_make(drop_p, drop_seed);
    DISPATCH_V(H, hipLaunchKernelGGL((residual_layernorm_kernel<V, true>), grid, block, 0, (hipStream_t)stream, x, residual, gamma,
                                     beta, eps, s_out, out, M, d));
    return e3d_launch_status("e3d_residual_layernorm_drop_fwd");
}

extern "C" int e3d_residual_layernorm_drop_fwd_keyed(const float* x, const float* residual, const float* gamma, const float* beta,
                                                     float eps, float* s_out, float* out, int M, int H, float drop_p, uint32_t site,
                                                     const uint64_t* row_keys, void* stream) {
    E3D_REQUIRE(x && gamma && beta && out && row_keys && M > 0, "residual_layernorm_drop_keyed: bad arguments");
    E3D_REQUIRE(drop_p >= 0.f && drop_p < 1.f, "residual_layernorm_drop_keyed: p = %f", (double)drop_p);
    E3D_REQUIRE(site < E3D_DROP_MAX_SITE, "residual_layernorm_drop_keyed: site %u does not fit 24 bits", site);
    const dim3 grid((M + 3) / 4), block(256);
    const E3dDrop d = e3d_drop_make_keyed(drop_p, site, row_keys);
    DISPATCH_V(H, hipLaunchKernelGGL((residual_layernorm_kernel<V, true, true>), grid, block, 0, (hipStream_t)stream, x, residual,
                                     gamma, beta, eps, s_out, out, M, d));
    return e3d_launch_status("e3d_residual_layernorm_drop_fwd_keyed");
}

extern "C" int e3d_adaln_gate_fwd(const float* x, const float* y, const float* mod, int branch,
                                  int rows_per_cond, float* out, int M, int H, void* stream) {
    E3D_REQUIRE(x && y && mod && out && M > 0, "adaln_gate: bad arguments");
    E3D_REQUIRE((branch == 0 || branch == 1) && rows_per_cond >= 1, "adaln_gate: branch=%d rows_per_cond=%d",
                branch, rows_per_cond);
    const dim3 grid((M + 3) / 4), block(256);
    DISPATCH_V(H, hipLaunchKernelGGL(adaln_gate_kernel<V>, grid, block, 0, (hipStream_t)stream, x, y, mod, branch,
                                     rows_per_cond, out, M));
    return e3d_launch_status("e3d_adaln_gate_fwd");
}

extern "C" int e3d_embed_layernorm_fwd(const float* x, int F, const float* W, const float* b,
                                       const float* gamma, const float* beta, float eps,
                                       const float* post_add, int rows_per_add, float* z_out,
                                       float* out, int M, int H, void* stream) {
    E3D_REQUIRE(x && W && b && gamma && beta && out && M > 0, "embed_layernorm: bad arguments");
    E3D_REQUIRE(F >= 1 && F <= 32, "embed_layernorm: F must be in [1,32] (F=%d)", F);
    E3D_REQUIRE(!post_add || rows_per_add >= 1, "embed_layernorm: rows_per_add=%d", rows_per_add);
    if (M <= 512) {
        const dim3 grid((M + 3) / 4), block(256);
        DISPATCH_V(H, hipLaunchKernelGGL(embed_layernorm_rows_kernel<V>, grid, block, 0, (hipStream_t)stream, x, F, W, b,
                                         gamma, beta, eps, post_add, rows_per_add, z_out, out, M));
        return e3d_launch_status("e3d_embed_layernorm_fwd");
    }
    int rpb = (M + 255) / 256;
    rpb = rpb < 32 ? 32 : (rpb > 128 ? 128 : rpb);
    int blocks = (M + rpb - 1) / rpb;
    blocks = blocks < 1 ? 1 : (blocks > 512 ? 512 : blocks);
    const dim3 grid(blocks), block(256);
    const size_t lds = (size_t)F * H * sizeof(float);
    DISPATCH_V(H, {
        static std::atomic<uint64_t> lds_ok{0};
        e3d_allow_lds(lds_ok, embed_layernorm_kernel<V>, 32 * (size_t)H * sizeof(float));
        hipLaunchKernelGGL(embed_layernorm_kernel<V>, grid, block, lds, (hipStream_t)stream, x, F, W, b, gamma, beta,
                           eps, post_add, rows_per_add, z_out, out, M);
    });
    return e3d_launch_status("e3d_embed_layernorm_fwd");
}

extern "C" int e3d_head_linear_fwd(const float* x, const float* W, const float* b, float* out,
                                   int M, int H, int Nout, void* stream) {
    E3D_REQUIRE(x && W && b && out && M > 0, "head_linear: bad arguments");
    E3D_REQUIRE(Nout >= 1 && Nout <= 32, "head_linear: Nout must be in [1,32] (Nout=%d)", Nout);
    const dim3 grid((M + 3) / 4), block(256);
    DISPATCH_V(H, hipLaunchKernelGGL(head_linear_kernel<V>, grid, block, 0, (hipStream_t)stream, x, W, b, out, M,
                                     Nout));
    return e3d_launch_status("e3d_head_linear_fwd");
}

namespace {
__global__ __launch_bounds__(256) void absmax_kernel(const float* __restrict__ x, int64_t n, float* __restrict__ target) {
    unsigned m = 0;
    for (int64_t i = (int64_t)blockIdx.x * 256 + threadIdx.x; i < n; i += (int64_t)gridDim.x * 256) e3d_absmax_accum(m, x[i]);
    e3d_absmax_commit(m, target, threadIdx.x & 63);
}
}

extern "C" int e3d_absmax_f32(const float* x, int64_t n, float* target, void* stream) {
    E3D_REQUIRE(x && target && n > 0, "absmax: bad arguments");
    int64_t blocks = (n + 256 * 8 - 1) / (256 * 8);
    blocks = blocks < 1 ? 1 : (blocks > 1024 ? 1024 : blocks);
    hipLaunchKernelGGL(absmax_kernel, dim3((unsigned)blocks), dim3(256), 0, (hipStream_t)stream, x, n, target);
    return e3d_launch_status("e3d_absmax_f32");
}
```

e3-invaraint-diffusion-model_amd/hip.py:

```python
import ctypes
import os
from ctypes import c_char_p, c_float, c_int, c_int64, c_uint32, c_uint64, c_void_p

_HERE = os.path.dirname(os.path.abspath(__file__))
LIB_PATH = os.environ.get("E3D_HIP_LIB", os.path.join(_HERE, "libe3d_hip.so"))
ABI_VERSION = 5

_P = c_void_p
_SIGNATURES = {
    "e3d_abi_version": (c_int, []),
    "e3d_last_error": (c_char_p, []),
    "e3d_gemm_bias_act_f32": (c_int, [_P, c_int64, _P, _P, _P, c_int64, c_int, c_int, c_int, c_int, _P]),
    "e3d_gemm_bias_act_f32_split": (c_int, [_P, c_int64, _P, _P, _P, c_int64, c_int, c_int, c_int, c_int, c_int, _P]),
    "e3d_gemm_bias_act_f32_split_ex": (c_int, [_P, c_int64, _P, _P, _P, c_int64, c_int, c_int, c_int, c_int, c_int, _P, c_float, _P]),
    "e3d_absmax_f32": (c_int, [_P, c_int64, _P, _P]),
    "e3d_relkey_attn_fwd": (c_int, [_P, c_int64, c_int64, _P, c_int64, c_int64, _P, c_int64, c_int64,
                                    _P, c_int, _P, _P, _P, c_int, c_int, c_int, c_int, _P]),
    "e3d_relkey_attn_fwd_split": (c_int, [_P, c_int64, c_int64, _P, c_int64, c_int64, _P, c_int64, c_int64,
                                          _P, c_int, _P, _P, _P, c_int, c_int, c_int, c_int, c_int, _P]),
    "e3d_gemm_skinny_workspace_bytes": (c_int64, [c_int, c_int, c_int]),
    "e3d_gemm_skinny_f32_split": (c_int, [_P, c_int64, _P, _P, _P, c_int64, c_int, c_int, c_int, c_int, c_int, _P, c_int64, _P]),
    "e3d_gemm_skinny_f32_split_ex": (c_int, [_P, c_int64, _P, _P, _P, c_int64, c_int, c_int, c_int, c_int, c_int, _P, c_int64, _P, c_float, _P]),
    "e3d_gemm_skinny_plan_select": (None, [c_int, c_int]),
    "e3d_gemm_skinny_residual_layernorm_f32_split": (c_int, [_P, c_int64, _P, _P, _P, _P, _P, c_float, _P, c_int, c_int, c_int,
                                                     c_int, _P, c_int64, _P]),
    "e3d_gemm_skinny_residual_layernorm_f32_split_ex": (c_int, [_P, c_int64, _P, _P, _P, _P, _P, c_float, _P, c_int, c_int, c_int,
                                                        c_int, _P, c_int64, c_float, _P]),
    "e3d_attn_skip_padded_tiles": (c_int, [c_int]),
    "e3d_gemm_kernel_select": (c_int, [c_int]),
    "e3d_gemm_general_select": (c_int, [c_int]),
    "e3d_attn_rescale_tau": (c_float, [c_float]),
    "e3d_residual_layernorm_fwd": (c_int, [_P, _P, _P, _P, c_float, _P, _P, c_int, c_int, _P]),
    "e3d_adaln_gate_fwd": (c_int, [_P, _P, _P, c_int, c_int, _P, c_int, c_int, _P]),
    "e3d_embed_layernorm_fwd": (c_int, [_P, c_int, _P, _P, _P, _P, c_float, _P, c_int, _P, _P, c_int, c_int, _P]),
    "e3d_nerf_backbone": (c_int, [_P, _P, _P, c_int, c_int, c_int, _P]),
    "e3d_gemm_f32_split_general": (c_int, [_P, c_int64, c_int, _P, c_int64, c_int, _P, _P, c_int64, c_int, c_int,
                                           c_int, c_int, c_int, _P]),
    "e3d_transpose_grouped_f32": (c_int, [_P, _P, c_int, c_int, c_int, c_int64, c_int64, _P]),
    "e3d_gemm_wgrad_grouped_f32_split": (c_int, [_P, _P, _P, _P, c_uint64, c_int, c_int64, c_int64, c_int, c_int, c_int, c_int, _P]),
    "e3d_residual_layernorm_drop_fwd": (c_int, [_P, _P, _P, _P, c_float, _P, _P, c_int, c_int, c_float, c_uint64, _P]),
    "e3d_layernorm_bwd_drop": (c_int, [_P, _P, _P, c_float, _P, _P, _P, _P, c_int, c_int, c_float, c_uint64, _P]),
    "e3d_weight_planes_bytes": (c_int64, [c_int, c_int]),
    "e3d_weight_planes_f32_split": (c_int, [_P, c_int, c_int, c_int, _P, _P]),
    "e3d_gemm_residual_layernorm_supported": (c_int, [c_int, c_int, c_int, c_int64]),
    "e3d_gemm_residual_layernorm_f32_split": (c_int, [_P, c_int64, _P, _P, _P, c_int64, _P, _P, c_float, _P, c_int64,
                                                      c_int, c_int, c_int, c_int, c_float, _P]),
    "e3d_gemm_wgrad_ragged_f32_split": (c_int, [_P, _P, _P, _P, _P, _P, _P, _P, c_uint64, c_int, c_int, c_int, _P]),
    "e3d_relkey_attn_bwd_workspace_floats": (c_int64, [c_int, c_int, c_int, c_int, c_int]),
    "e3d_relkey_attn_bwd": (c_int, [_P, c_int64, c_int64, _P, c_int64, c_int64, _P, c_int64, c_int64, _P, c_int, _P,
                                    _P, _P, _P, _P, c_int64, c_int64, _P, c_int64, c_int64, _P, c_int64, c_int64,
                                    _P, _P, c_int, c_int, c_int, c_int, _P]),
    "e3d_dropout_f32": (c_int, [_P, c_float, c_uint64, _P, c_int64, _P]),
    "e3d_relkey_attn_fwd_split_drop": (c_int, [_P, c_int64, c_int64, _P, c_int64, c_int64, _P, c_int64, c_int64,
                                               _P, c_int, _P, _P, _P, c_int, c_int, c_int, c_int, c_int, c_float,
                                               c_uint64, _P]),
    "e3d_relkey_attn_fwd_split_ex": (c_int, [_P, c_int64, c_int64, _P, c_int64, c_int64, _P, c_int64, c_int64,
                                             _P, c_int, _P, _P, _P, c_int, c_int, c_int, c_int, c_int, c_float,
                                             c_uint64, _P, c_int, _P, _P, _P, _P]),
    "e3d_attn_scratch_bytes": (c_int64, [c_int]),
    "e3d_ddpm_step_wrap_table": (c_int, [_P, _P, _P, _P, _P, c_int, _P, c_int64, _P]),
    "e3d_relkey_attn_bwd_drop": (c_int, [_P, c_int64, c_int64, _P, c_int64, c_int64, _P, c_int64, c_int64, _P, c_int, _P,
                                         _P, _P, _P, _P, c_int64, c_int64, _P, c_int64, c_int64, _P, c_int64, c_int64,
                                         _P, _P, c_int, c_int, c_int, c_int, c_float, c_uint64, _P]),
    "e3d_relkey_attn_bwd_ex": (c_int, [_P, c_int64, c_int64, _P, c_int64, c_int64, _P, c_int64, c_int64, _P, c_int, _P,
                                       _P, _P, _P, _P, c_int64, c_int64, _P, c_int64, c_int64, _P, c_int64, c_int64,
                                       _P, _P, c_int, c_int, c_int, c_int, c_int, c_float, c_uint64, _P]),
    "e3d_attn_dropout_mask": (c_int, [c_int, c_int, c_int, c_int, c_float, c_uint64, _P, _P]),
    "e3d_layernorm_bwd": (c_int, [_P, _P, _P, c_float, _P, _P, _P, c_int, c_int, _P]),
    "e3d_layernorm_bwd_workspace_floats": (c_int64, [c_int, c_int]),
    "e3d_layernorm_bwd_ws": (c_int, [_P, _P, _P, c_float, _P, _P, _P, _P, c_int, c_int, c_float, c_uint64, _P, c_int64, _P]),
    "e3d_adaln_gate_bwd": (c_int, [_P, _P, _P, c_int, c_int, _P, _P, c_int, c_int, _P]),
    "e3d_act_fwd": (c_int, [_P, c_int, _P, c_int64, _P]),
    "e3d_act_bwd": (c_int, [_P, _P, c_int, _P, c_int64, _P]),
    "e3d_colsum": (c_int, [_P, c_int64, _P, c_int, c_int, _P]),
    "e3d_group_sum": (c_int, [_P, c_int, _P, c_int, c_int, _P]),
    "e3d_small_k_wgrad": (c_int, [_P, _P, _P, _P, c_int, c_int, c_int, c_int, _P]),
    "e3d_head_linear_bwd_dx": (c_int, [_P, _P, _P, c_int, c_int, c_int, _P]),
    "e3d_head_linear_fwd": (c_int, [_P, _P, _P, _P, c_int, c_int, c_int, _P]),
    "e3d_ddpm_step_wrap": (c_int, [_P, _P, _P, c_float, c_float, c_float, c_float, c_int, _P, c_int64, _P]),
    "e3d_q_sample_wrap": (c_int, [_P, _P, _P, _P, _P, _P, c_int, c_int64, _P]),
    "e3d_discrete_posterior_sample": (c_int, [_P, _P, _P, _P, _P, c_int, _P, _P, c_int, c_int, c_int, _P]),
    "e3d_discrete_q_sample": (c_int, [_P, _P, _P, c_int, _P, c_int, c_int, c_int, _P]),
    "e3d_optim_chunk_elems": (c_int, []),
    "e3d_grad_global_norm": (c_int, [_P, _P, _P, _P, c_int, c_float, _P, _P, _P]),
    "e3d_adamw_step_dyn": (c_int, [_P, _P, _P, _P, _P, _P, _P, c_int, _P, _P, c_float, c_float, c_float, c_float, _P]),
    "e3d_adamw_step_dev": (c_int, [_P, _P, _P, _P, _P, _P, _P, c_int, _P, _P, _P]),
    "e3d_dropout_set_epoch_ptr": (c_int, [_P]),
    "e3d_adamw_step": (c_int, [_P, _P, _P, _P, _P, _P, _P, c_int, _P, c_float, c_float, c_float, c_float, c_float, c_int, _P]),
    "e3d_attn_varlen_fwd": (c_int, [_P, c_int64, _P, c_int64, _P, c_int64, _P, _P, _P, _P, _P, c_int, _P, c_int, _P,
                                    c_int64, c_int, c_int, c_int, c_int, _P]),
    "e3d_keyed_ddpm_step_wrap": (c_int, [_P, _P, _P, _P, _P, c_uint64, c_int, _P, c_int64, c_int, _P]),
    "e3d_keyed_discrete_posterior_sample": (c_int, [_P, _P, _P, _P, _P, c_uint64, _P, _P, c_int, c_int, c_int, _P]),
    "e3d_keyed_draws": (c_int, [_P, c_uint64, c_int, c_int, c_int, c_int, c_int, c_float, _P, c_int64, _P]),
    "e3d_keyed_timesteps": (c_int, [_P, _P, c_uint64, c_int, c_int, _P, c_int, _P]),
    "e3d_keyed_q_sample_wrap": (c_int, [_P, _P, _P, _P, c_int, c_float, _P, _P, c_uint64, _P, _P, c_int, c_int, c_int, _P]),
    "e3d_keyed_discrete_q_sample": (c_int, [_P, _P, _P, _P, c_uint64, _P, c_int, c_int, c_int, _P]),
    "e3d_keyed_drop_row_keys": (c_int, [_P, c_int, c_int, _P, c_uint64, c_int, _P, _P]),
    "e3d_dropout_f32_keyed": (c_int, [_P, c_float, c_uint32, _P, _P, c_int, c_int, _P]),
    "e3d_keyed_attn_dropout_mask": (c_int, [c_int, c_int, c_int, c_int, c_float, c_uint32, _P, _P, _P]),
    "e3d_residual_layernorm_drop_fwd_keyed": (c_int, [_P, _P, _P, _P, c_float, _P, _P, c_int, c_int, c_float, c_uint32, _P, _P]),
    "e3d_layernorm_bwd_drop_keyed": (c_int, [_P, _P, _P, c_float, _P, _P, _P, _P, c_int, c_int, c_float, c_uint32, _P, _P]),
    "e3d_layernorm_bwd_ws_keyed": (c_int, [_P, _P, _P, c_float, _P, _P, _P, _P, c_int, c_int, c_float, c_uint32, _P, _P, c_int64,
                                           _P]),
    "e3d_relkey_attn_fwd_split_drop_keyed": (c_int, [_P, c_int64, c_int64, _P, c_int64, c_int64, _P, c_int64, c_int64,
                                                     _P, c_int, _P, _P, _P, c_int, c_int, c_int, c_int, c_int, c_float,
                                                     c_uint32, _P, _P]),
    "e3d_relkey_attn_fwd_split_ex_keyed": (c_int, [_P, c_int64, c_int64, _P, c_int64, c_int64, _P, c_int64, c_int64,
                                                   _P, c_int, _P, _P, _P, c_int, c_int, c_int, c_int, c_int, c_float,
                                                   c_uint32, _P, _P, c_int, _P, _P, _P, _P]),
    "e3d_relkey_attn_bwd_drop_keyed": (c_int, [_P, c_int64, c_int64, _P, c_int64, c_int64, _P, c_int64, c_int64, _P, c_int, _P,
                                               _P, _P, _P, _P, c_int64, c_int64, _P, c_int64, c_int64, _P, c_int64, c_int64,
                                               _P, _P, c_int, c_int, c_int, c_int, c_float, c_uint32, _P, _P]),
    "e3d_relkey_attn_bwd_ex_keyed": (c_int, [_P, c_int64, c_int64, _P, c_int64, c_int64, _P, c_int64, c_int64, _P, c_int, _P,
                                             _P, _P, _P, _P, c_int64, c_int64, _P, c_int64, c_int64, _P, c_int64, c_int64,
                                             _P, _P, c_int, c_int, c_int, c_int, c_int, c_float, c_uint32, _P, _P]),
}
EXPORTS = tuple(_SIGNATURES)

_lib = None


class HipExtensionMissing(RuntimeError):
    pass


def lib():
    global _lib
    if _lib is None:
        if not os.path.exists(LIB_PATH):
            raise HipExtensionMissing(
                f"{LIB_PATH} not found: the HIP extension is the only compute path of this package "
                "(no CPU fallback). Build it with `python -c 'import __graft_entry__ as g; g.build()'`.")
        import torch
        handle = ctypes.CDLL(LIB_PATH)
        for name, (res, args) in _SIGNATURES.items():
            fn = getattr(handle, name)
            fn.restype, fn.argtypes = res, args
        got = handle.e3d_abi_version()
        if got != ABI_VERSION:
            raise HipExtensionMissing(f"{LIB_PATH}: ABI version {got}, binding expects {ABI_VERSION}")
        _lib = handle
    return _lib


def check(rc, what):
    if rc != 0:
        msg = lib().e3d_last_error().decode(errors="replace")
        raise RuntimeError(f"{what} failed (rc={rc}): {msg}")
```

e3-invaraint-diffusion-model_amd/ops.py:

```python
import contextlib
import math
import os
import warnings

import torch

from . import hip, keyed

ACT_NONE, ACT_GELU, ACT_SILU = 0, 1, 2


def _stream():
    return torch.cuda.current_stream().cuda_stream


TRACE = None


_ROCTX = None


def _roctx():
    global _ROCTX
    if _ROCTX is None:
        _ROCTX = False
        if os.environ.get("E3D_ROCTX") == "1":
            import ctypes
            for name in ("libroctx64.so", "libroctx64.so.4", "/opt/rocm/lib/libroctx64.so"):
                try:
                    lib = ctypes.CDLL(name)
                    lib.roctxRangePushA.argtypes = [ctypes.c_char_p]
                    _ROCTX = lib
                    break
                except OSError:
                    continue
    return _ROCTX


ROCTX_NAMES = {"attn_relkey": b"K1 relkey_attention_fwd", "attn_cross": b"K2 cross_attention_fwd",
               "attn_bwd": b"K3 attention_bwd", "adaln_gate": b"K4 adaln_gate",
               "residual_layernorm": b"K5 residual_layernorm", "embed_layernorm": b"K5 embed_layernorm",
               "gemm_layernorm": b"K5 gemm_residual_layernorm",
               "gemm": b"K5 gemm_bias_act", "ddpm_step_wrap": b"K6 ddpm_step_wrap",
               "discrete_posterior": b"K7 discrete_posterior_sample", "discrete_q_sample": b"K7 discrete_q_sample"}


class _timed:

    def __init__(self, name, meta=None):
        self.on = TRACE is not None
        self.rx = _roctx()
        self.name = name
        if self.on:
            self.rec = (name, torch.cuda.Event(enable_timing=True), torch.cuda.Event(enable_timing=True), meta)

    def __enter__(self):
        if self.rx:
            self.rx.roctxRangePushA(ROCTX_NAMES.get(self.name, self.name.encode()))
        if self.on:
            self.rec[1].record()

    def __exit__(self, *exc):
        if self.on:
            self.rec[2].record()
            TRACE.append(self.rec)
        if self.rx:
            self.rx.roctxRangePop()


def _chk(t, name, dtype=torch.float32):
    if t is None:
        return
    if not t.is_cuda:
        raise RuntimeError(f"{name}: expected a GPU tensor (this package has no CPU path), got {t.device}")
    if t.dtype != dtype:
        raise TypeError(f"{name}: expected {dtype}, got {t.dtype}")


def _p(t):
    return None if t is None else t.data_ptr()


PARAM_GENERATION = 0


def invalidate_weight_caches(*_args, **_kwargs):
    global PARAM_GENERATION
    PARAM_GENERATION += 1


def weight_key(*tensors):
    return (PARAM_GENERATION,) + tuple((t.data_ptr(), t._version) for t in tensors)


try:
    from torch.optim.optimizer import register_optimizer_step_post_hook as _reg_post_hook
    _reg_post_hook(invalidate_weight_caches)
except ImportError:
    pass


_ABSMAX_POOLS = {}
ABSMAX_POOL_SLOTS = 4096


def absmax_slot(owner, name, device):
    slots = owner.__dict__.setdefault("_e3d_absmax", {})
    key = (name, device.index)
    t = slots.get(key)
    if t is None:
        ent = _ABSMAX_POOLS.get(device.index)
        if ent is None:
            ent = _ABSMAX_POOLS[device.index] = [torch.zeros(ABSMAX_POOL_SLOTS, device=device, dtype=torch.float32), 0, []]
        if ent[1] >= ABSMAX_POOL_SLOTS:
            ent[2].append(ent[0])
            ent[0], ent[1] = torch.zeros(ABSMAX_POOL_SLOTS, device=device, dtype=torch.float32), 0
        t = slots[key] = ent[0][ent[1]:ent[1] + 1]
        ent[1] += 1
    return t


def reset_absmax(device=None):
    idx = torch.cuda.current_device() if device is None else torch.device(device).index
    ent = _ABSMAX_POOLS.get(idx)
    if ent is not None:
        ent[0].zero_()
        for old_pool in ent[2]:
            old_pool.zero_()


def absmax(x, target=None):
    _chk(x, "absmax.x")
    assert x.is_contiguous()
    if target is None:
        target = torch.zeros(1, device=x.device, dtype=torch.float32)
    hip.check(hip.lib().e3d_absmax_f32(_p(x), x.numel(), _p(target), _stream()), "e3d_absmax_f32")
    return target


GEMM_MODES = {"f32": 0, "bf16x3": 3, "bf16x6": 6, "f16x3": 19, "bf16": 1}
GEMM_MODE = os.environ.get("E3D_GEMM_MODE", "f16x3")
if GEMM_MODE not in GEMM_MODES:
    raise ValueError(f"E3D_GEMM_MODE must be one of {sorted(GEMM_MODES)}, got {GEMM_MODE!r}")


def set_gemm_mode(mode):
    global GEMM_MODE
    if mode not in GEMM_MODES:
        raise ValueError(f"gemm mode must be one of {sorted(GEMM_MODES)}, got {mode!r}")
    prev, GEMM_MODE = GEMM_MODE, mode
    return prev


F16_WEIGHT_EXP = 12
_f16_warned = False


def f16_weight(weight):
    global _f16_warned
    ent = getattr(weight, "_e3d_f16w", None)
    key = weight_key(weight)
    if ent is not None and ent[0] == key:
        return ent[1], ent[2]
    if torch.cuda.is_current_stream_capturing():
        raise RuntimeError("f16x3: the pre-scaled copy of a weight is missing inside a stream capture -- run the step eagerly once "
                           "before capturing it (building the copy reads max |w| back to the host)")
    with torch.no_grad():
        amax = float(weight.detach().abs().max())
        if not math.isfinite(amax) or amax == 0.0:
            if not math.isfinite(amax) and not _f16_warned:
                _f16_warned = True
                warnings.warn("f16x3: a weight holds inf / NaN -- used as it is (the outputs will say so)")
            scaled, inv = weight.detach(), 1.0
        else:
            k = max(-120, min(120, F16_WEIGHT_EXP - math.frexp(amax)[1]))
            scaled, inv = (weight.detach() * (2.0 ** k)).contiguous(), 2.0 ** -k
    try:
        weight._e3d_f16w = (key, scaled, inv)
    except AttributeError:
        pass
    return scaled, inv


SKINNY_MAX_M = 1024 if os.environ.get("E3D_GEMM_SKINNY", "1") == "1" else 0
SKINNY_GEMM_MAX_M = int(os.environ.get("E3D_GEMM_SKINNY_MAX_M", "512"))
SKINNY_MAX_TILES = 768
_SKINNY_WS = {}
_SKINNY_RETIRED = []


def _skinny_workspace(device, M, N, K):
    nbytes = hip.lib().e3d_gemm_skinny_workspace_bytes(M, N, K)
    key = (device.index, torch.cuda.current_stream(device).cuda_stream)
    ws = _SKINNY_WS.get(key)
    if ws is None or ws.numel() < nbytes:
        if ws is not None:
            _SKINNY_RETIRED.append(ws)
        ws = _SKINNY_WS[key] = torch.empty(max(nbytes, 8 << 20), dtype=torch.uint8, device=device)
    return ws


def _skinny_ok(terms, M, N, K, a):
    return (terms in (3, 19) and 0 < M <= SKINNY_MAX_M and N % 32 == 0 and K % 16 == 0 and a.stride(0) % 4 == 0
            and -(-M // 32) * (N // 32) <= SKINNY_MAX_TILES)


def gemm(a, weight, bias=None, act=ACT_NONE, out=None, mode=None, absmax=None, prescale=True):
    _chk(a, "gemm.a"); _chk(weight, "gemm.weight"); _chk(bias, "gemm.bias")
    assert a.dim() == 2 and a.stride(1) == 1 and weight.is_contiguous()
    M, K = a.shape
    N = weight.shape[0]
    assert weight.shape[1] == K, (a.shape, weight.shape)
    if out is None:
        out = torch.empty((M, N), device=a.device, dtype=torch.float32)
    assert out.dim() == 2 and out.stride(1) == 1 and out.shape == (M, N)
    terms = GEMM_MODES[GEMM_MODE if mode is None else mode]
    if absmax is not None:
        _chk(absmax, "gemm.absmax")
        assert act == ACT_NONE and absmax.numel() == 1
    scale = 1.0
    if terms == 19 and prescale:
        weight, scale = f16_weight(weight)
    with _timed("gemm", (M, N, K, act)):
        if _skinny_ok(terms, M, N, K, a) and out.stride(0) % 4 == 0 and M <= min(SKINNY_MAX_M, SKINNY_GEMM_MAX_M):
            ws = _skinny_workspace(a.device, M, N, K)
            hip.check(hip.lib().e3d_gemm_skinny_f32_split_ex(_p(a), a.stride(0), _p(weight), _p(bias), _p(out), out.stride(0),
                                                             M, N, K, act, terms, _p(ws), ws.numel(), _p(absmax), scale, _stream()),
                      "e3d_gemm_skinny_f32_split_ex")
        elif terms == 0:
            hip.check(hip.lib().e3d_gemm_bias_act_f32(_p(a), a.stride(0), _p(weight), _p(bias), _p(out),
                                                      out.stride(0), M, N, K, act, _stream()), "e3d_gemm_bias_act_f32")
        else:
            hip.check(hip.lib().e3d_gemm_bias_act_f32_split_ex(
                _p(a), a.stride(0), _p(weight), _p(bias), _p(out), out.stride(0), M, N, K, act, terms, _p(absmax), scale,
                _stream()), "e3d_gemm_bias_act_f32_split_ex")
    return out


class arithmetic:

    def __init__(self, mode, respect_env=True):
        self.gemm = os.environ.get("E3D_GEMM_MODE", mode) if respect_env else mode
        self.attn = os.environ.get("E3D_ATTN_MODE", self.gemm) if respect_env else mode

    def __enter__(self):
        self.prev = (set_gemm_mode(self.gemm), set_attn_mode(self.attn))
        return self

    def __exit__(self, *exc):
        set_gemm_mode(self.prev[0])
        set_attn_mode(self.prev[1])


ATTN_MODE = os.environ.get("E3D_ATTN_MODE", GEMM_MODE)
if ATTN_MODE == "bf16":
    ATTN_MODE = "bf16x3"
if ATTN_MODE not in GEMM_MODES:
    raise ValueError(f"E3D_ATTN_MODE must be one of {sorted(GEMM_MODES)}, got {ATTN_MODE!r}")


def set_attn_mode(mode):
    global ATTN_MODE
    if mode not in GEMM_MODES:
        raise ValueError(f"attention mode must be one of {sorted(GEMM_MODES)}, got {mode!r}")
    if mode == "bf16":
        mode = "bf16x3"
    prev, ATTN_MODE = ATTN_MODE, mode
    return prev


_DROPOUT_EPOCH = {}


def dropout_epoch(device):
    dev = torch.device(device)
    idx = dev.index if dev.index is not None else torch.cuda.current_device()
    t = _DROPOUT_EPOCH.get(idx)
    if t is None:
        t = torch.zeros(1, dtype=torch.int64, device=f"cuda:{idx}")
        with torch.cuda.device(idx):
            hip.check(hip.lib().e3d_dropout_set_epoch_ptr(t.data_ptr()), "e3d_dropout_set_epoch_ptr")
        _DROPOUT_EPOCH[idx] = t
    return t


MAX_DROPOUT_SITES = 1 << 24
MAX_DROPOUT_HEADS = 1 << 16


class KeyedDropout:

    def __init__(self, seed, epoch_word, ids):
        self.seed, self.epoch, self.ids = keyed.check_seed(seed), epoch_word, ids
        self.site = 0
        self._tables = {}

    def next_site(self):
        site = self.site
        if site >= MAX_DROPOUT_SITES:
            raise ValueError(f"keyed dropout holds {MAX_DROPOUT_SITES} sites per step")
        self.site = site + 1
        return site

    def row_keys(self, stream, L):
        t = self._tables.get((stream, L))
        if t is None:
            t = self._tables[(stream, L)] = keyed_drop_row_keys(self.ids, L, self.epoch, self.seed, stream)
        return t


_KEYED_DROPOUT = None


def keyed_dropout_state():
    return _KEYED_DROPOUT


@contextlib.contextmanager
def keyed_dropout(seed, epoch_word, ids):
    global _KEYED_DROPOUT
    prev, _KEYED_DROPOUT = _KEYED_DROPOUT, KeyedDropout(seed, epoch_word, ids)
    try:
        yield _KEYED_DROPOUT
    finally:
        _KEYED_DROPOUT = prev


def next_dropout_seed():
    if _KEYED_DROPOUT is not None:
        return _KEYED_DROPOUT.next_site()
    return int(torch.randint(0, 2 ** 62, (), dtype=torch.int64))


def site_drop(p, row_keys=None):
    if _KEYED_DROPOUT is None:
        if row_keys is not None:
            raise RuntimeError("row keys given to a dropout site outside ops.keyed_dropout")
        return float(p), next_dropout_seed()
    if row_keys is None:
        raise RuntimeError("a dropout site inside ops.keyed_dropout needs the key table of its rows")
    return float(p), next_dropout_seed(), row_keys


def _keyed_drop(drop, rows, what, heads=1):
    p, site, row_keys = drop
    if not 0 <= int(site) < MAX_DROPOUT_SITES:
        raise ValueError(f"{what}: dropout site {site} outside [0, 2^24)")
    if heads >= MAX_DROPOUT_HEADS:
        raise ValueError(f"{what}: keyed dropout holds fewer than 2^16 heads, got {heads}")
    if row_keys.dtype != torch.int64 or not row_keys.is_cuda or not row_keys.is_contiguous() or row_keys.numel() != rows:
        raise ValueError(f"{what}: row keys must be a contiguous int64 device tensor of {rows} keys")
    return float(p), int(site), _p(row_keys)


def keyed_drop_row_keys(ids, L, epoch_word, seed, stream):
    if stream not in (keyed.DROP_LIGAND, keyed.DROP_POCKET):
        raise ValueError(f"dropout row keys live on streams {keyed.DROP_LIGAND} / {keyed.DROP_POCKET}, got {stream}")
    if L > keyed.MAX_POSITION:
        raise ValueError(f"keyed streams hold positions below 2^24, got a frame of {L}")
    B = ids.numel()
    assert ids.dtype == torch.int64 and ids.is_cuda and ids.is_contiguous() and epoch_word.dtype == torch.int64 and epoch_word.is_cuda
    out = torch.empty((B * L,), device=ids.device, dtype=torch.int64)
    hip.check(hip.lib().e3d_keyed_drop_row_keys(_p(ids), B, L, _p(epoch_word), keyed.check_seed(seed), int(stream), _p(out),
                                                _stream()), "e3d_keyed_drop_row_keys")
    return out


def dropout(x, p, seed, out=None, row_keys=None):
    _chk(x, "dropout.x")
    assert x.is_contiguous()
    out = torch.empty_like(x) if out is None else out
    if row_keys is not None:
        H = x.shape[-1]
        M = x.numel() // H
        p, site, keys = _keyed_drop((p, seed, row_keys), M, "dropout")
        hip.check(hip.lib().e3d_dropout_f32_keyed(_p(x), p, site, keys, _p(out), M, H, _stream()), "e3d_dropout_f32_keyed")
        return out
    hip.check(hip.lib().e3d_dropout_f32(_p(x), float(p), int(seed), _p(out), x.numel(), _stream()), "e3d_dropout_f32")
    return out


def keyed_attn_dropout_mask(B, nh, Lq, Lk, p, site, row_keys):
    out = torch.empty((B, nh, Lq, Lk), device=row_keys.device, dtype=torch.float32)
    p, site, keys = _keyed_drop((p, site, row_keys), B * Lq, "keyed_attn_dropout_mask", nh)
    hip.check(hip.lib().e3d_keyed_attn_dropout_mask(B, nh, Lq, Lk, p, site, keys, _p(out), _stream()),
              "e3d_keyed_attn_dropout_mask")
    return out


def attn_dropout_mask(B, nh, Lq, Lk, p, seed, device="cuda"):
    out = torch.empty((B, nh, Lq, Lk), device=device, dtype=torch.float32)
    hip.check(hip.lib().e3d_attn_dropout_mask(B, nh, Lq, Lk, float(p), int(seed), _p(out), _stream()),
              "e3d_attn_dropout_mask")
    return out


def attention(q, k, v, B, nh, Lq, Lk, key_mask=None, dist_emb=None, max_pos=0, want_lse=False, mode=None, drop=None,
              bounds=None):
    for n, t in (("q", q), ("k", k), ("v", v), ("key_mask", key_mask), ("dist_emb", dist_emb)):
        _chk(t, "attention." + n)
    assert q.stride(1) == 1 and k.stride(1) == 1 and v.stride(1) == 1
    assert q.shape[0] == B * Lq and k.shape[0] == B * Lk and v.shape[0] == B * Lk
    if key_mask is not None:
        assert key_mask.is_contiguous() and key_mask.shape == (B, Lk)
    if dist_emb is not None:
        assert dist_emb.is_contiguous() and dist_emb.shape == (2 * max_pos - 1, 64), dist_emb.shape
    out = torch.empty((B * Lq, nh * 64), device=q.device, dtype=torch.float32)
    lse = torch.empty((B, nh, Lq), device=q.device, dtype=torch.float32) if want_lse else None
    terms = GEMM_MODES[ATTN_MODE if mode is None else mode]
    with _timed("attn_relkey" if dist_emb is not None else "attn_cross", (B, nh, Lq, Lk)):
        args = (_p(q), Lq * q.stride(0), q.stride(0), _p(k), Lk * k.stride(0), k.stride(0),
                _p(v), Lk * v.stride(0), v.stride(0), _p(dist_emb), max_pos, _p(key_mask), _p(out), _p(lse),
                B, nh, Lq, Lk)
        dropping = drop is not None and drop[0] > 0
        if terms == 0 and not dropping:
            hip.check(hip.lib().e3d_relkey_attn_fwd(*args, _stream()), "e3d_relkey_attn_fwd")
        else:
            scratch, ready, e_abs = None, 0, None
            q_abs, k_abs = bounds if bounds is not None else (None, None)
            if dist_emb is not None:
                infer = not torch.is_grad_enabled()
                ent = getattr(dist_emb, "_e3d_planes", None) if infer else None
                if ent is not None and ent[0] == weight_key(dist_emb) + (Lk, terms):
                    scratch, ready, e_abs = ent[1], 1, ent[2]
                else:
                    scratch = torch.empty((hip.lib().e3d_attn_scratch_bytes(Lk),), device=q.device, dtype=torch.uint8)
                    e_abs = None
                    have_bounds = q_abs is not None and k_abs is not None
                    if have_bounds and not infer:
                        try:
                            e_abs = absmax_slot(dist_emb, "e", q.device)
                        except AttributeError:
                            e_abs = torch.zeros(1, device=q.device, dtype=torch.float32)
                    elif have_bounds:
                        e_abs = torch.zeros(1, device=q.device, dtype=torch.float32)
                    if infer and not torch.cuda.is_current_stream_capturing():
                        try:
                            if e_abs is None:
                                e_abs = absmax(dist_emb.detach())
                            dist_emb._e3d_planes = (weight_key(dist_emb) + (Lk, terms), scratch, e_abs)
                        except AttributeError:
                            pass
            p, seed = (float(drop[0]), int(drop[1])) if dropping else (0.0, 0)
            if q_abs is None or k_abs is None or (dist_emb is not None and e_abs is None):
                q_abs = k_abs = e_abs = None
            if dropping and len(drop) == 3:
                p, site, keys = _keyed_drop(drop, B * Lq, "attention", nh)
                hip.check(hip.lib().e3d_relkey_attn_fwd_split_ex_keyed(*args, terms or 6, p, site, keys, _p(scratch), ready,
                                                                       _p(q_abs), _p(k_abs), _p(e_abs), _stream()),
                          "e3d_relkey_attn_fwd_split_ex_keyed")
                return (out, lse) if want_lse else out
            hip.check(hip.lib().e3d_relkey_attn_fwd_split_ex(*args, terms or 6, p, seed, _p(scratch), ready, _p(q_abs),
                                                             _p(k_abs), _p(e_abs), _stream()),
                      "e3d_relkey_attn_fwd_split_ex")
    return (out, lse) if want_lse else out


def attention_varlen(q, k, v, q_layout, k_layout, nh, dist_emb=None, max_pos=0, mode=None):
    if torch.is_grad_enabled() and any(t is not None and t.requires_grad for t in (q, k, v, dist_emb)):
        raise RuntimeError("attention_varlen is inference-only: run it under torch.no_grad()")
    for n, t in (("q", q), ("k", k), ("v", v), ("dist_emb", dist_emb)):
        _chk(t, "attention_varlen." + n)
    assert q.dim() == 2 and q.stride(1) == 1 and k.stride(1) == 1 and v.stride(1) == 1
    if q.shape[0] != q_layout.rows or k.shape[0] != k_layout.rows or v.shape[0] != k_layout.rows:
        raise ValueError(f"attention_varlen: rows q {q.shape[0]} / k {k.shape[0]} / v {v.shape[0]} against layouts of "
                         f"{q_layout.rows} / {k_layout.rows} rows")
    if q_layout.B != k_layout.B:
        raise ValueError(f"attention_varlen: {q_layout.B} query segments against {k_layout.B} key segments")
    if dist_emb is not None:
        assert dist_emb.is_contiguous() and dist_emb.shape == (2 * max_pos - 1, 64), dist_emb.shape
        if not q_layout.same_segments(k_layout):
            raise ValueError("attention_varlen: relative_key self-attention needs q_len == k_len for every segment")
    alloc = torch.zeros if q_layout.padded_frame else torch.empty
    out = alloc((q_layout.rows, nh * 64), device=q.device, dtype=torch.float32)
    terms = GEMM_MODES[ATTN_MODE if mode is None else mode]
    if q_layout.n_tiles == 0:
        return out
    with _timed("attn_varlen", (q_layout.B, nh, q_layout.rows, k_layout.rows)):
        hip.check(hip.lib().e3d_attn_varlen_fwd(
            _p(q), q.stride(0), _p(k), k.stride(0), _p(v), v.stride(0), _p(q_layout.start_dev), _p(q_layout.len_dev),
            _p(k_layout.start_dev), _p(k_layout.len_dev), _p(q_layout.tiles), q_layout.n_tiles, _p(dist_emb), max_pos,
            _p(out), q_layout.rows, nh, q_layout.max_len, k_layout.max_len, terms, _stream()), "e3d_attn_varlen_fwd")
    return out


def residual_layernorm(x, residual, gamma, beta, eps, want_s=False, drop=None):
    for n, t in (("x", x), ("residual", residual), ("gamma", gamma), ("beta", beta)):
        _chk(t, "residual_layernorm." + n)
    assert x.is_contiguous() and (residual is None or residual.is_contiguous())
    M, H = x.shape
    out = torch.empty_like(x)
    s = torch.empty_like(x) if want_s else None
    with _timed("residual_layernorm", (M, H)):
        if drop is not None and drop[0] > 0 and len(drop) == 3:
            p, site, keys = _keyed_drop(drop, M, "residual_layernorm")
            hip.check(hip.lib().e3d_residual_layernorm_drop_fwd_keyed(_p(x), _p(residual), _p(gamma), _p(beta), eps, _p(s), _p(out),
                                                                      M, H, p, site, keys, _stream()),
                      "e3d_residual_layernorm_drop_fwd_keyed")
        elif drop is not None and drop[0] > 0:
            hip.check(hip.lib().e3d_residual_layernorm_drop_fwd(_p(x), _p(residual), _p(gamma), _p(beta), eps, _p(s), _p(out), M, H,
                                                                float(drop[0]), int(drop[1]), _stream()),
                      "e3d_residual_layernorm_drop_fwd")
        else:
            hip.check(hip.lib().e3d_residual_layernorm_fwd(_p(x), _p(residual), _p(gamma), _p(beta), eps, _p(s),
                                                           _p(out), M, H, _stream()), "e3d_residual_layernorm_fwd")
    return (out, s) if want_s else out


ROWLN_MIN_M = int(os.environ.get("E3D_GEMM_ROWLN_MIN_M", "8192")) if os.environ.get("E3D_GEMM_ROWLN", "1") == "1" else 1 << 62


def weight_planes(weight, terms):
    ent = getattr(weight, "_e3d_planes_w", None)
    key = weight_key(weight) + (terms,)
    if ent is not None and ent[0] == key:
        return ent[1], ent[2]
    if torch.cuda.is_current_stream_capturing():
        raise RuntimeError("weight_planes: cache miss inside a stream capture (warm the op up before capturing)")
    src, scale = f16_weight(weight) if terms == 19 else (weight.detach(), 1.0)
    N, K = src.shape
    nbytes = hip.lib().e3d_weight_planes_bytes(N, K)
    if nbytes < 0:
        raise ValueError(f"weight_planes: unsupported shape {tuple(src.shape)}")
    planes = torch.empty((nbytes,), dtype=torch.uint8, device=src.device)
    hip.check(hip.lib().e3d_weight_planes_f32_split(_p(src), N, K, terms, _p(planes), _stream()), "e3d_weight_planes_f32_split")
    try:
        weight._e3d_planes_w = (key, planes, scale)
    except AttributeError:
        pass
    return planes, scale


def rowln_ok(terms, M, H, K, a, residual=None):
    return (terms in (3, 19) and M >= ROWLN_MIN_M and a.stride(1) == 1 and a.data_ptr() % 16 == 0
            and (residual is None or (residual.stride(1) == 1 and residual.stride(0) % 4 == 0 and residual.data_ptr() % 16 == 0))
            and bool(hip.lib().e3d_gemm_residual_layernorm_supported(M, H, K, a.stride(0))))


def linear_residual_layernorm(a, weight, bias, residual, gamma, beta, eps, mode=None):
    M, K = a.shape
    H = weight.shape[0]
    terms = GEMM_MODES[GEMM_MODE if mode is None else mode]
    if rowln_ok(terms, M, H, K, a, residual):
        for t, n in ((a, "a"), (weight, "weight"), (bias, "bias"), (residual, "residual"), (gamma, "gamma"), (beta, "beta")):
            _chk(t, "linear_residual_layernorm." + n)
        assert weight.is_contiguous() and weight.shape[1] == K and (residual is None or residual.shape == (M, H))
        planes, scale = weight_planes(weight, terms)
        out = torch.empty((M, H), device=a.device, dtype=torch.float32)
        with _timed("gemm_layernorm", (M, H, K)):
            hip.check(hip.lib().e3d_gemm_residual_layernorm_f32_split(
                _p(a), a.stride(0), _p(planes), _p(bias), _p(residual), residual.stride(0) if residual is not None else 0,
                _p(gamma), _p(beta), eps, _p(out), out.stride(0), M, H, K, terms, scale, _stream()),
                "e3d_gemm_residual_layernorm_f32_split")
        return out
    if not (_skinny_ok(terms, M, H, K, a) and H in (256, 512, 768, 1024) and a.stride(1) == 1):
        return residual_layernorm(gemm(a, weight, bias, mode=mode), residual, gamma, beta, eps)
    for t, n in ((a, "a"), (weight, "weight"), (bias, "bias"), (residual, "residual"), (gamma, "gamma"), (beta, "beta")):
        _chk(t, "linear_residual_layernorm." + n)
    assert weight.is_contiguous() and weight.shape[1] == K and (residual is None or (residual.is_contiguous() and residual.shape == (M, H)))
    out = torch.empty((M, H), device=a.device, dtype=torch.float32)
    ws = _skinny_workspace(a.device, M, H, K)
    scale = 1.0
    if terms == 19:
        weight, scale = f16_weight(weight)
    with _timed("gemm_layernorm", (M, H, K)):
        hip.check(hip.lib().e3d_gemm_skinny_residual_layernorm_f32_split_ex(
            _p(a), a.stride(0), _p(weight), _p(bias), _p(residual), _p(gamma), _p(beta), eps, _p(out), M, H, K, terms,
            _p(ws), ws.numel(), scale, _stream()), "e3d_gemm_skinny_residual_layernorm_f32_split_ex")
    return out

def adaln_gate(x, y, mod, branch, rows_per_cond):
    for n, t in (("x", x), ("y", y), ("mod", mod)):
        _chk(t, "adaln_gate." + n)
    assert x.is_contiguous() and y.is_contiguous() and mod.is_contiguous()
    M, H = x.shape
    assert mod.shape[1] == 6 * H and mod.shape[0] * rows_per_cond == M, (mod.shape, M, rows_per_cond)
    out = torch.empty_like(x)
    with _timed("adaln_gate", (M, H)):
        hip.check(hip.lib().e3d_adaln_gate_fwd(_p(x), _p(y), _p(mod), branch, rows_per_cond, _p(out),
                                               M, H, _stream()), "e3d_adaln_gate_fwd")
    return out


def embed_layernorm(x, weight, bias, gamma, beta, eps, post_add=None, rows_per_add=1, want_z=False):
    for n, t in (("x", x), ("weight", weight), ("bias", bias), ("gamma", gamma), ("beta", beta),
                 ("post_add", post_add)):
        _chk(t, "embed_layernorm." + n)
    assert x.is_contiguous() and weight.is_contiguous()
    M, F = x.shape
    H = weight.shape[0]
    assert weight.shape[1] == F
    if post_add is not None:
        assert post_add.is_contiguous() and post_add.shape == (M // rows_per_add, H)
    out = torch.empty((M, H), device=x.device, dtype=torch.float32)
    z = torch.empty_like(out) if want_z else None
    with _timed("embed_layernorm", (M, H)):
        hip.check(hip.lib().e3d_embed_layernorm_fwd(_p(x), F, _p(weight), _p(bias), _p(gamma), _p(beta), eps,
                                                    _p(post_add), rows_per_add, _p(z), _p(out), M, H, _stream()),
                  "e3d_embed_layernorm_fwd")
    return (out, z) if want_z else out


def head_linear(x, weight, bias):
    for n, t in (("x", x), ("weight", weight), ("bias", bias)):
        _chk(t, "head_linear." + n)
    assert x.is_contiguous() and weight.is_contiguous()
    M, H = x.shape
    n_out = weight.shape[0]
    out = torch.empty((M, n_out), device=x.device, dtype=torch.float32)
    hip.check(hip.lib().e3d_head_linear_fwd(_p(x), _p(weight), _p(bias), _p(out), M, H, n_out, _stream()),
              "e3d_head_linear_fwd")
    return out


def ddpm_step_wrap(x, eps_hat, noise, sqrt_recip_alpha, beta, sqrt_one_minus_ab, sigma, wrap=True, out=None):
    for n, t in (("x", x), ("eps_hat", eps_hat), ("noise", noise)):
        _chk(t, "ddpm_step_wrap." + n)
    assert x.is_contiguous() and eps_hat.is_contiguous() and (noise is None or noise.is_contiguous())
    if out is None:
        out = torch.empty_like(x)
    with _timed("ddpm_step_wrap"):
        hip.check(hip.lib().e3d_ddpm_step_wrap(_p(x), _p(eps_hat), _p(noise), sqrt_recip_alpha, beta,
                                               sqrt_one_minus_ab, sigma, int(wrap), _p(out), x.numel(), _stream()),
                  "e3d_ddpm_step_wrap")
    return out


def ddpm_step_wrap_table(x, eps_hat, noise, coef_table, t_dev, wrap=True, out=None):
    for n, t in (("x", x), ("eps_hat", eps_hat), ("noise", noise), ("coef_table", coef_table)):
        _chk(t, "ddpm_step_wrap_table." + n)
    _chk(t_dev, "ddpm_step_wrap_table.t_dev", torch.int64)
    assert x.is_contiguous() and eps_hat.is_contiguous() and noise.is_contiguous() and coef_table.is_contiguous()
    assert coef_table.dim() == 2 and coef_table.shape[1] == 4
    if out is None:
        out = torch.empty_like(x)
    with _timed("ddpm_step_wrap"):
        hip.check(hip.lib().e3d_ddpm_step_wrap_table(_p(x), _p(eps_hat), _p(noise), _p(coef_table), _p(t_dev), int(wrap),
                                                     _p(out), x.numel(), _stream()), "e3d_ddpm_step_wrap_table")
    return out


def q_sample_wrap(x0, noise, t, sqrt_ab, sqrt_1mab):
    for n, tt in (("x0", x0), ("noise", noise), ("sqrt_ab", sqrt_ab), ("sqrt_1mab", sqrt_1mab)):
        _chk(tt, "q_sample_wrap." + n)
    _chk(t, "q_sample_wrap.t", torch.int64)
    assert x0.is_contiguous() and noise.is_contiguous() and t.is_contiguous()
    B = x0.shape[0]
    out = torch.empty_like(x0)
    hip.check(hip.lib().e3d_q_sample_wrap(_p(x0), _p(noise), _p(t), _p(sqrt_ab), _p(sqrt_1mab), _p(out),
                                          B, x0.numel() // B, _stream()), "e3d_q_sample_wrap")
    return out


def discrete_posterior_sample(xt_idx, logits, qsb, qtb, u=None, want_prob=False):
    _chk(xt_idx, "xt_idx", torch.int32); _chk(logits, "logits"); _chk(qsb, "qsb"); _chk(qtb, "qtb"); _chk(u, "u")
    B, L, C = logits.shape
    assert xt_idx.is_contiguous() and logits.is_contiguous() and qsb.is_contiguous() and qtb.is_contiguous()
    assert qsb.shape == (B, C, C) and qtb.shape == (B, C, C) and xt_idx.shape == (B, L)
    out = torch.empty((B, L), device=logits.device, dtype=torch.int32)
    prob = torch.empty((B, L, C), device=logits.device, dtype=torch.float32) if want_prob else None
    with _timed("discrete_posterior"):
        hip.check(hip.lib().e3d_discrete_posterior_sample(
            _p(xt_idx), _p(logits), _p(qsb), _p(qtb), _p(u), 0 if u is None else 1, _p(out), _p(prob),
            B, L, C, _stream()), "e3d_discrete_posterior_sample")
    return (out, prob) if want_prob else out


def discrete_q_sample(x0_idx, qtb, u=None):
    _chk(x0_idx, "x0_idx", torch.int32); _chk(qtb, "qtb"); _chk(u, "u")
    B, L = x0_idx.shape
    C = qtb.shape[-1]
    assert x0_idx.is_contiguous() and qtb.is_contiguous() and qtb.shape == (B, C, C)
    out = torch.empty((B, L), device=qtb.device, dtype=torch.int32)
    with _timed("discrete_q_sample"):
        hip.check(hip.lib().e3d_discrete_q_sample(_p(x0_idx), _p(qtb), _p(u), 0 if u is None else 1, _p(out),
                                                  B, L, C, _stream()), "e3d_discrete_q_sample")
    return out



def _chk_keys(row_keys, rows, name):
    _chk(row_keys, name + ".row_keys", torch.int64)
    if not (row_keys.is_contiguous() and row_keys.dim() == 2 and row_keys.shape == (rows, 2)):
        raise ValueError(f"{name}: row_keys must be a contiguous [{rows}, 2] table, got {tuple(row_keys.shape)}")


def keyed_ddpm_step_wrap(x, eps_hat, coef_table, t_dev, row_keys, seed, wrap=True, out=None):
    for n, t in (("x", x), ("eps_hat", eps_hat), ("coef_table", coef_table)):
        _chk(t, "keyed_ddpm_step_wrap." + n)
    _chk(t_dev, "keyed_ddpm_step_wrap.t_dev", torch.int64)
    F = x.shape[-1]
    if F % 4:
        raise ValueError(f"keyed_ddpm_step_wrap: the feature count must be a multiple of 4, got {F}")
    rows = x.numel() // F
    _chk_keys(row_keys, rows, "keyed_ddpm_step_wrap")
    assert x.is_contiguous() and eps_hat.is_contiguous() and coef_table.is_contiguous() and eps_hat.shape == x.shape
    assert coef_table.dim() == 2 and coef_table.shape[1] == 4
    if coef_table.shape[0] - 1 > 65535:
        raise ValueError(f"keyed_ddpm_step_wrap: keyed streams hold steps up to 65535, the table has {coef_table.shape[0]}")
    if out is None:
        out = torch.empty_like(x)
    with _timed("keyed_ddpm_step_wrap"):
        hip.check(hip.lib().e3d_keyed_ddpm_step_wrap(_p(x), _p(eps_hat), _p(coef_table), _p(t_dev), _p(row_keys),
                                                     keyed.check_seed(seed), int(wrap), _p(out), rows, F, _stream()),
                  "e3d_keyed_ddpm_step_wrap")
    return out


def keyed_discrete_posterior_sample(xt_idx, logits, qsb, qtb, row_keys, seed, s_dev):
    _chk(xt_idx, "xt_idx", torch.int32); _chk(logits, "logits"); _chk(qsb, "qsb"); _chk(qtb, "qtb")
    _chk(s_dev, "s_dev", torch.int64)
    B, L, C = logits.shape
    _chk_keys(row_keys, B * L, "keyed_discrete_posterior_sample")
    assert xt_idx.is_contiguous() and logits.is_contiguous() and qsb.is_contiguous() and qtb.is_contiguous()
    assert qsb.shape == (B, C, C) and qtb.shape == (B, C, C) and xt_idx.shape == (B, L)
    out = torch.empty((B, L), device=logits.device, dtype=torch.int32)
    with _timed("discrete_posterior"):
        hip.check(hip.lib().e3d_keyed_discrete_posterior_sample(
            _p(xt_idx), _p(logits), _p(qsb), _p(qtb), _p(row_keys), keyed.check_seed(seed), _p(s_dev), _p(out), B, L, C,
            _stream()), "e3d_keyed_discrete_posterior_sample")
    return out


KEYED_NORMAL, KEYED_UNIFORM, KEYED_ONEHOT, KEYED_CLASS = 0, 1, 2, 3


def keyed_draws(row_keys, seed, stream, t, kind, width=0, wrap=False, scale=1.0):
    _chk(row_keys, "keyed_draws.row_keys", torch.int64)
    rows = row_keys.shape[0]
    _chk_keys(row_keys, rows, "keyed_draws")
    if not 0 <= int(t) <= 65535:
        raise ValueError(f"keyed_draws: step {t} outside [0, 65535]")
    if kind == KEYED_NORMAL and width % 4:
        raise ValueError(f"keyed_draws: the feature count must be a multiple of 4, got {width}")
    shape, dtype = {KEYED_NORMAL: ((rows, width), torch.float32), KEYED_UNIFORM: ((rows,), torch.float32),
                    KEYED_ONEHOT: ((rows, width), torch.float32), KEYED_CLASS: ((rows,), torch.int32)}[kind]
    out = torch.empty(shape, device=row_keys.device, dtype=dtype)
    if rows:
        hip.check(hip.lib().e3d_keyed_draws(_p(row_keys), keyed.check_seed(seed), int(stream), int(t), int(kind), int(width),
                                            int(wrap), float(scale), _p(out), rows, _stream()), "e3d_keyed_draws")
    return out


def keyed_initial_angles(row_keys, seed, F, scale=1.0):
    return keyed_draws(row_keys, seed, keyed.STRUCT_XT, 0, KEYED_NORMAL, F, wrap=True, scale=scale)


def keyed_initial_onehot(row_keys, seed, C):
    return keyed_draws(row_keys, seed, keyed.SEQ_XT, 0, KEYED_ONEHOT, C)



def _chk_ids_epoch(item_ids, epoch, B, name):
    _chk(item_ids, name + ".item_ids", torch.int64)
    _chk(epoch, name + ".epoch", torch.int64)
    if not (item_ids.is_contiguous() and item_ids.shape == (B,)):
        raise ValueError(f"{name}: item_ids must be a contiguous int64 [{B}], got {tuple(item_ids.shape)}")
    if epoch.numel() != 1:
        raise ValueError(f"{name}: the epoch is one int64 on the device, got {tuple(epoch.shape)}")


def keyed_timesteps(item_ids, epoch, seed, stream, C):
    if stream not in (keyed.TRAIN_STRUCT_T, keyed.TRAIN_SEQ_T):
        raise ValueError(f"keyed_timesteps: stream {stream} is not a timestep stream")
    if not 1 <= int(C) <= 1 << 24:
        raise ValueError(f"keyed_timesteps: class count {C}")
    B = item_ids.shape[0]
    _chk_ids_epoch(item_ids, epoch, B, "keyed_timesteps")
    out = torch.empty((B,), device=item_ids.device, dtype=torch.int64)
    with _timed("keyed_timesteps"):
        hip.check(hip.lib().e3d_keyed_timesteps(_p(item_ids), _p(epoch), keyed.check_seed(seed), int(stream), int(C),
                                                _p(out), B, _stream()), "e3d_keyed_timesteps")
    return out


def keyed_q_sample_wrap(x0, t, sqrt_ab, sqrt_1mab, scale, item_ids, epoch, seed):
    for n, tt in (("x0", x0), ("sqrt_ab", sqrt_ab), ("sqrt_1mab", sqrt_1mab)):
        _chk(tt, "keyed_q_sample_wrap." + n)
    _chk(t, "keyed_q_sample_wrap.t", torch.int64)
    if x0.dim() != 3 or x0.shape[-1] % 4:
        raise ValueError(f"keyed_q_sample_wrap: x0 must be [B, L, F] with F a multiple of 4, got {tuple(x0.shape)}")
    B, L, F = x0.shape
    if L > keyed.MAX_POSITION:
        raise ValueError(f"keyed streams hold positions below 2^24, got a frame of {L}")
    _chk_ids_epoch(item_ids, epoch, B, "keyed_q_sample_wrap")
    assert x0.is_contiguous() and t.is_contiguous() and t.shape == (B,)
    assert sqrt_ab.is_contiguous() and sqrt_1mab.is_contiguous() and sqrt_ab.shape == sqrt_1mab.shape and sqrt_ab.dim() == 1
    noise, x_t = torch.empty_like(x0), torch.empty_like(x0)
    with _timed("keyed_q_sample_wrap"):
        hip.check(hip.lib().e3d_keyed_q_sample_wrap(_p(x0), _p(t), _p(sqrt_ab), _p(sqrt_1mab), sqrt_ab.shape[0], float(scale),
                                                    _p(item_ids), _p(epoch), keyed.check_seed(seed), _p(noise), _p(x_t),
                                                    B, L, F, _stream()), "e3d_keyed_q_sample_wrap")
    return noise, x_t


def keyed_discrete_q_sample(x0_idx, qtb, item_ids, epoch, seed):
    _chk(x0_idx, "x0_idx", torch.int32); _chk(qtb, "qtb")
    B, L = x0_idx.shape
    C = qtb.shape[-1]
    if L > keyed.MAX_POSITION:
        raise ValueError(f"keyed streams hold positions below 2^24, got a frame of {L}")
    _chk_ids_epoch(item_ids, epoch, B, "keyed_discrete_q_sample")
    assert x0_idx.is_contiguous() and qtb.is_contiguous() and qtb.shape == (B, C, C)
    out = torch.empty((B, L), device=qtb.device, dtype=torch.int32)
    with _timed("discrete_q_sample"):
        hip.check(hip.lib().e3d_keyed_discrete_q_sample(_p(x0_idx), _p(qtb), _p(item_ids), _p(epoch), keyed.check_seed(seed),
                                                        _p(out), B, L, C, _stream()), "e3d_keyed_discrete_q_sample")
    return out
```

e3-invaraint-diffusion-model_amd/structure_model/model.py:

```python
import functools
from typing import List

import torch
from torch import nn

from .. import bert, keyed, ops
from ..blocks import (BertEmbeddings, GaussianFourierProjection, KeyedDropoutSwitch, Predictor, SELayer, drop_row_keys,
                      flat2d, require_gpu)
from ..training import adamw
import os

from .utils import elementwise_form, radian_l1_loss, radian_smooth_l1_loss

MASKED_LOSS = os.environ.get("E3D_MASKED_LOSS", "1") == "1"


class ReceptorCache:

    def __init__(self, encoder_states, cross_kv, mask, B, L, layout=None):
        self.encoder_states, self.cross_kv, self.mask, self.B, self.L = encoder_states, cross_kv, mask, B, L
        self.layout = layout


class ConditionalBertForDiffusionBase(nn.Module):
    def __init__(self, encoder_config, decoder_config, feature_size: int) -> None:
        super().__init__()
        self.encoder_config = encoder_config
        self.decoder_config = decoder_config
        self.receptor_seq_emb = BertEmbeddings(20, encoder_config)
        self.receptor_angle_emb = BertEmbeddings(feature_size, encoder_config)
        self.receptor_emb = SELayer(encoder_config)
        self.encoder = bert.BertEncoder(encoder_config)
        self.ligand_angle_emb = BertEmbeddings(feature_size, decoder_config)
        self.timestep_projector = GaussianFourierProjection(decoder_config.hidden_size)
        self.timestep_emb = SELayer(decoder_config)
        self.decoder = bert.BertEncoder(decoder_config)
        self.angles_predictor = Predictor(decoder_config.hidden_size, feature_size)

    def encode_receptor(self, receptor_seq, receptor_angles, receptor_attention_masks,
                        project_cross_kv=True, layout=None) -> ReceptorCache:
        require_gpu(receptor_seq, receptor_angles, receptor_attention_masks)
        B, L = receptor_angles.shape[:2]
        ops.reset_absmax(receptor_angles.device)
        if layout is not None:
            ang = self.receptor_angle_emb.run(flat2d(layout.pack(receptor_angles)))
            seq = self.receptor_seq_emb.run(flat2d(layout.pack(receptor_seq)))
            x = self.receptor_emb.run(ang, seq, None, 1, layout.rows, layout=layout)
            x = bert.run_encoder(self.encoder, x, None, 1, layout.rows, layout=layout)
            kv = [bert.project_cross_kv(layer.crossattention, x) for layer in self.decoder.layer] if project_cross_kv else None
            return ReceptorCache(x, kv, None, B, L, layout=layout)
        mask = receptor_attention_masks.contiguous().float()
        rk = drop_row_keys(keyed.DROP_POCKET, L)
        ang = self.receptor_angle_emb.run(flat2d(receptor_angles), row_keys=rk)
        seq = self.receptor_seq_emb.run(flat2d(receptor_seq), row_keys=rk)
        x = self.receptor_emb.run(ang, seq, mask, B, L, row_keys=rk)
        x = bert.run_encoder(self.encoder, x, mask, B, L, row_keys=rk)
        kv = None
        if project_cross_kv:
            kv = [bert.project_cross_kv(layer.crossattention, x) for layer in self.decoder.layer]
        return ReceptorCache(x, kv, mask, B, L)

    def timestep_modulation(self, timesteps):
        temb = self.timestep_projector(timesteps.reshape(-1)).contiguous()
        return self.timestep_emb.modulation(temb)

    def decode(self, timestep, noised_ligand_angles, ligand_attention_masks, receptor: ReceptorCache, mod=None,
               layout=None):
        if layout is not None:
            return self._decode_packed(timestep, noised_ligand_angles, receptor, mod, layout)
        require_gpu(timestep, noised_ligand_angles, ligand_attention_masks)
        B, L = noised_ligand_angles.shape[:2]
        mask = ligand_attention_masks.contiguous().float()
        lk = drop_row_keys(keyed.DROP_LIGAND, L)
        x = self.ligand_angle_emb.run(flat2d(noised_ligand_angles), row_keys=lk)
        if mod is None:
            mod = self.timestep_modulation(timestep.squeeze(dim=-1))
        x = self.timestep_emb.run(x, None, mask, B, L, mod=mod, row_keys=lk)
        x = bert.run_encoder(self.decoder, x, mask, B, L, enc=receptor.encoder_states,
                             enc_mask=receptor.mask, Lk=receptor.L, cross_kv=receptor.cross_kv, row_keys=lk)
        return self.angles_predictor.run(x).view(B, L, -1)

    def _decode_packed(self, timestep, x_packed, receptor, mod, layout):
        require_gpu(x_packed)
        if receptor.layout is None:
            raise ValueError("a packed decode needs the pocket packed as well: encode_receptor(..., layout=)")
        assert x_packed.dim() == 2 and x_packed.shape[0] == layout.rows, (tuple(x_packed.shape), layout.rows)
        if mod is None:
            t = timestep.reshape(-1)
            assert bool((t == t[0]).all()), "a packed batch shares one timestep"
            mod = self.timestep_modulation(t[:1])
        assert mod.shape[0] == 1, "a packed batch shares one timestep: mod must be one row [1,6H]"
        x = self.ligand_angle_emb.run(x_packed.contiguous().float())
        x = self.timestep_emb.run(x, None, None, 1, layout.rows, mod=mod, layout=layout)
        x = bert.run_encoder(self.decoder, x, None, 1, layout.rows, enc=receptor.encoder_states,
                             cross_kv=receptor.cross_kv, layout=layout, enc_layout=receptor.layout)
        return self.angles_predictor.run(x)

    def forward(self, timestep, noised_ligand_angles, ligand_attention_masks,
                receptor_seq, receptor_angles, receptor_attention_masks,
                ligand_pos_ids=None, receptor_pos_ids=None):
        rec = self.encode_receptor(receptor_seq, receptor_angles, receptor_attention_masks,
                                   project_cross_kv=False)
        return self.decode(timestep, noised_ligand_angles, ligand_attention_masks, rec)


class ConditionalBertForDiffusion(KeyedDropoutSwitch, ConditionalBertForDiffusionBase):
    diheral_loss_func = radian_l1_loss
    angle_loss_func = functools.partial(radian_smooth_l1_loss, beta=torch.pi / 10)

    def __init__(self, encoder_config, decoder_config, feature_names: List[str], loss_func: List,
                 epochs: int = 1, lr_scheduler=None, l2_lambda: float = 0.0,
                 steps_per_epoch: int = 250, learning_rate: float = 5e-5, **kwargs):
        super().__init__(encoder_config, decoder_config, len(feature_names))
        self.steps_per_epoch = steps_per_epoch
        self.learning_rate = learning_rate
        self.feature_names = feature_names
        self.lr_scheduler = lr_scheduler
        self.loss_func = loss_func
        self.epochs = epochs
        self.l2_lambda = l2_lambda
        self.train_epoch_losses, self.valid_epoch_losses = [], []
        self.train_epoch_counter = 0

    def _get_loss_terms(self, batch) -> torch.Tensor:
        known_noise = batch["known_noise"]
        predicted_noise = self.forward(
            timestep=batch["timestep"], noised_ligand_angles=batch["noised_ligand_angle"],
            ligand_attention_masks=batch["ligand_attn_mask"], receptor_seq=batch["receptor_seq"],
            receptor_angles=batch["receptor_angles"], receptor_attention_masks=batch["receptor_attn_mask"])
        assert known_noise.shape == predicted_noise.shape, f"{known_noise.shape} != {predicted_noise.shape}"
        return self.loss_terms_from_prediction(predicted_noise, known_noise, batch["ligand_attn_mask"])

    def loss_terms_from_prediction(self, predicted_noise, known_noise, ligand_attn_mask):
        n_feat = known_noise.shape[-1]
        fns = [self.loss_func[i] if isinstance(self.loss_func, list) else self.loss_func for i in range(n_feat)]
        elems = [elementwise_form(fn) for fn in fns]
        if all(e is not None for e in elems) and MASKED_LOSS:
            sel = (ligand_attn_mask != 0).unsqueeze(-1)
            count = sel.sum().to(predicted_noise.dtype)
            groups = {}
            for i, fn in enumerate(fns):
                key = (fn.func, tuple(sorted(fn.keywords.items()))) if isinstance(fn, functools.partial) else (fn, ())
                groups.setdefault(key, []).append(i)
            terms = [None] * n_feat
            for idx in groups.values():
                if idx == list(range(idx[0], idx[-1] + 1)):
                    pn, kn = predicted_noise[..., idx[0]:idx[-1] + 1], known_noise[..., idx[0]:idx[-1] + 1]
                else:
                    cache = self.__dict__.setdefault("_e3d_loss_idx", {})
                    it = cache.get((tuple(idx), predicted_noise.device))
                    if it is None:
                        it = cache[(tuple(idx), predicted_noise.device)] = torch.tensor(idx, device=predicted_noise.device)
                    pn, kn = predicted_noise.index_select(-1, it), known_noise.index_select(-1, it)
                e = elems[idx[0]](pn, kn)
                sums = torch.where(sel, e, torch.zeros((), dtype=e.dtype, device=e.device)).sum(dim=(0, 1)) / count
                for j, i in enumerate(idx):
                    terms[i] = sums[j]
            return torch.stack(terms)
        rows, cols = torch.where(ligand_attn_mask)
        terms = []
        for i in range(n_feat):
            terms.append(fns[i](predicted_noise[rows, cols, i], known_noise[rows, cols, i]))
        return torch.stack(terms)

    def training_step(self, batch, batch_idx=0):
        with self.keyed_dropout_step(batch):
            return torch.mean(self._get_loss_terms(batch))

    @torch.no_grad()
    def validation_step(self, batch, batch_idx=0):
        return {"val_loss": torch.mean(self._get_loss_terms(batch))}

    def configure_optimizers(self):
        optim = adamw(self.parameters(), lr=self.learning_rate, weight_decay=self.l2_lambda)
        retval = {"optimizer": optim}
        if self.lr_scheduler == "OneCycleLR":
            retval["lr_scheduler"] = {
                "scheduler": torch.optim.lr_scheduler.OneCycleLR(
                    optim, max_lr=1e-2, epochs=self.epochs, steps_per_epoch=self.steps_per_epoch),
                "interval": "step"}
        elif self.lr_scheduler == "LinearWarmup":
            warmup, total = int(self.epochs * 0.1), self.epochs

            def lr_lambda(step):
                if step < warmup:
                    return float(step) / float(max(1, warmup))
                return max(0.0, float(total - step) / float(max(1, total - warmup)))

            retval["lr_scheduler"] = {"scheduler": torch.optim.lr_scheduler.LambdaLR(optim, lr_lambda),
                                      "interval": "epoch"}
        elif self.lr_scheduler:
            raise ValueError(f"Unknown lr scheduler {self.lr_scheduler}")
        return retval
```

include/e3d_hip.h:

```cpp
#ifndef E3D_HIP_H
#define E3D_HIP_H

#include <stdint.h>

#ifdef __cplusplus
extern "C" {
#endif

#define E3D_ABI_VERSION 5

#define E3D_TERMS_BF16 1
#define E3D_TERMS_BF16X3 3
#define E3D_TERMS_BF16X6 6
#define E3D_TERMS_F16X3 19

#define E3D_ACT_NONE 0
#define E3D_ACT_GELU 1
#define E3D_ACT_SILU 2

int e3d_abi_version(void);
const char* e3d_last_error(void);

int e3d_gemm_bias_act_f32(const float* A, int64_t lda, const float* W, const float* bias,
                          float* out, int64_t ldc, int M, int N, int K, int act, void* stream);

int e3d_gemm_bias_act_f32_split(const float* A, int64_t lda, const float* W, const float* bias,
                                float* out, int64_t ldc, int M, int N, int K, int act, int terms,
                                void* stream);

int e3d_gemm_bias_act_f32_split_ex(const float* A, int64_t lda, const float* W, const float* bias, float* out,
                                   int64_t ldc, int M, int N, int K, int act, int terms, float* out_absmax,
                                   float out_scale, void* stream);
int e3d_absmax_f32(const float* x, int64_t n, float* target, void* stream);

int e3d_relkey_attn_fwd(const float* q, int64_t q_bs, int64_t q_rs,
                        const float* k, int64_t k_bs, int64_t k_rs,
                        const float* v, int64_t v_bs, int64_t v_rs,
                        const float* dist_emb, int P, const float* key_mask,
                        float* out, float* lse, int B, int nh, int Lq, int Lk, void* stream);

int e3d_relkey_attn_fwd_split(const float* q, int64_t q_bs, int64_t q_rs,
                              const float* k, int64_t k_bs, int64_t k_rs,
                              const float* v, int64_t v_bs, int64_t v_rs,
                              const float* dist_emb, int P, const float* key_mask,
                              float* out, float* lse, int B, int nh, int Lq, int Lk, int terms,
                              void* stream);

int64_t e3d_gemm_skinny_workspace_bytes(int M, int N, int K);
int e3d_gemm_skinny_f32_split(const float* A, int64_t lda, const float* W, const float* bias, float* out,
                              int64_t ldc, int M, int N, int K, int act, int terms, void* workspace,
                              int64_t workspace_bytes, void* stream);
int e3d_gemm_skinny_f32_split_ex(const float* A, int64_t lda, const float* W, const float* bias, float* out,
                                 int64_t ldc, int M, int N, int K, int act, int terms, void* workspace,
                                 int64_t workspace_bytes, float* out_absmax, float out_scale, void* stream);
void e3d_gemm_skinny_plan_select(int waves_per_cu_x2, int min_k_slice);
int e3d_gemm_skinny_residual_layernorm_f32_split(const float* A, int64_t lda, const float* W, const float* bias,
                                                 const float* residual, const float* gamma, const float* beta, float eps,
                                                 float* out, int M, int H, int K, int terms, void* workspace,
                                                 int64_t workspace_bytes, void* stream);
int e3d_gemm_skinny_residual_layernorm_f32_split_ex(const float* A, int64_t lda, const float* W, const float* bias,
                                                    const float* residual, const float* gamma, const float* beta,
                                                    float eps, float* out, int M, int H, int K, int terms,
                                                    void* workspace, int64_t workspace_bytes, float out_scale,
                                                    void* stream);

int e3d_gemm_kernel_select(int pref);
int e3d_gemm_general_select(int form);

float e3d_attn_rescale_tau(float tau);

int e3d_attn_skip_padded_tiles(int enable);

int e3d_residual_layernorm_fwd(const float* x, const float* residual, const float* gamma,
                               const float* beta, float eps, float* s_out, float* out, int M,
                               int H, void* stream);

int e3d_adaln_gate_fwd(const float* x, const float* y, const float* mod, int branch,
                       int rows_per_cond, float* out, int M, int H, void* stream);

int e3d_embed_layernorm_fwd(const float* x, int F, const float* W, const float* b,
                            const float* gamma, const float* beta, float eps,
                            const float* post_add, int rows_per_add, float* z_out, float* out,
                            int M, int H, void* stream);

int e3d_head_linear_fwd(const float* x, const float* W, const float* b, float* out, int M,
                        int H, int Nout, void* stream);

int e3d_ddpm_step_wrap(const float* x, const float* eps_hat, const float* noise,
                       float sqrt_recip_alpha, float beta, float sqrt_one_minus_ab, float sigma,
                       int wrap, float* out, int64_t n, void* stream);

int e3d_ddpm_step_wrap_table(const float* x, const float* eps_hat, const float* noise,
                             const float* coef_table, const int64_t* t_dev, int wrap, float* out,
                             int64_t n, void* stream);

int e3d_q_sample_wrap(const float* x0, const float* noise, const int64_t* t,
                      const float* sqrt_ab, const float* sqrt_1mab, float* out, int B,
                      int64_t per, void* stream);

int e3d_discrete_posterior_sample(const int32_t* xt_idx, const float* logits, const float* Qsb,
                                  const float* Qtb, const float* u, int mode, int32_t* out_idx,
                                  float* prob_out, int B, int L, int C, void* stream);

int e3d_discrete_q_sample(const int32_t* x0_idx, const float* Qtb, const float* u, int mode,
                          int32_t* out_idx, int B, int L, int C, void* stream);


int e3d_keyed_ddpm_step_wrap(const float* x, const float* eps_hat, const float* coef_table, const int64_t* t_dev,
                             const int64_t* row_keys, uint64_t seed, int wrap, float* out, int64_t rows, int F,
                             void* stream);

int e3d_keyed_discrete_posterior_sample(const int32_t* xt_idx, const float* logits, const float* Qsb,
                                        const float* Qtb, const int64_t* row_keys, uint64_t seed,
                                        const int64_t* s_dev, int32_t* out_idx, int B, int L, int C, void* stream);

int e3d_keyed_draws(const int64_t* row_keys, uint64_t seed, int stream_id, int t, int kind, int width, int wrap,
                    float scale, void* out, int64_t rows, void* stream);


int e3d_keyed_timesteps(const int64_t* item_ids, const int64_t* epoch_dev, uint64_t seed, int stream_id, int C,
                        int64_t* out, int B, void* stream);

int e3d_keyed_q_sample_wrap(const float* x0, const int64_t* t, const float* sqrt_ab, const float* sqrt_1mab, int T,
                            float scale, const int64_t* item_ids, const int64_t* epoch_dev, uint64_t seed,
                            float* noise_out, float* xt_out, int B, int L, int F, void* stream);

int e3d_keyed_discrete_q_sample(const int32_t* x0_idx, const float* Qtb, const int64_t* item_ids,
                                const int64_t* epoch_dev, uint64_t seed, int32_t* out_idx, int B, int L, int C,
                                void* stream);

int e3d_nerf_backbone(const float* angles, const int32_t* lengths, double* coords, int center,
                      int B, int L, void* stream);


int e3d_gemm_f32_split_general(const float* A, int64_t lda, int a_kmajor, const float* B, int64_t ldb,
                               int b_kmajor, const float* bias, float* out, int64_t ldc, int M, int N,
                               int K, int act, int terms, void* stream);

int e3d_gemm_wgrad_grouped_f32_split(const float* const* dz, const float* const* x, float* const* dw, float* const* db,
                                     uint64_t accumulate_bits, int count, int64_t ldz, int64_t ldx, int N, int K, int M,
                                     int terms, void* stream);

int e3d_gemm_wgrad_ragged_f32_split(const float* const* dz, const float* const* x, float* const* dw, float* const* db,
                                    const int* N, const int* K, const int64_t* ldz, const int64_t* ldx,
                                    uint64_t accumulate_bits, int count, int M, int terms, void* stream);

int64_t e3d_relkey_attn_bwd_workspace_floats(int B, int nh, int Lq, int Lk, int relkey);
int e3d_relkey_attn_bwd(const float* q, int64_t q_bs, int64_t q_rs, const float* k, int64_t k_bs,
                        int64_t k_rs, const float* v, int64_t v_bs, int64_t v_rs,
                        const float* dist_emb, int P, const float* key_mask, const float* out,
                        const float* lse, const float* dout, float* dq, int64_t dq_bs, int64_t dq_rs,
                        float* dk, int64_t dk_bs, int64_t dk_rs, float* dv, int64_t dv_bs,
                        int64_t dv_rs, float* d_dist_emb, float* workspace, int B, int nh, int Lq,
                        int Lk, void* stream);

int e3d_dropout_f32(const float* x, float p, uint64_t seed, float* out, int64_t n, void* stream);

int e3d_relkey_attn_fwd_split_drop(const float* q, int64_t q_bs, int64_t q_rs, const float* k, int64_t k_bs,
                                   int64_t k_rs, const float* v, int64_t v_bs, int64_t v_rs,
                                   const float* dist_emb, int P, const float* key_mask, float* out,
                                   float* lse, int B, int nh, int Lq, int Lk, int terms, float drop_p,
                                   uint64_t drop_seed, void* stream);

int64_t e3d_attn_scratch_bytes(int Lk);
int e3d_relkey_attn_fwd_split_ex(const float* q, int64_t q_bs, int64_t q_rs, const float* k, int64_t k_bs,
                                 int64_t k_rs, const float* v, int64_t v_bs, int64_t v_rs,
                                 const float* dist_emb, int P, const float* key_mask, float* out,
                                 float* lse, int B, int nh, int Lq, int Lk, int terms, float drop_p,
                                 uint64_t drop_seed, void* e_scratch, int e_scratch_ready, const float* q_absmax,
                                 const float* k_absmax, float* e_absmax, void* stream);

int e3d_attn_varlen_fwd(const float* q, int64_t q_rs, const float* k, int64_t k_rs, const float* v, int64_t v_rs,
                        const int* q_start, const int* q_len, const int* k_start, const int* k_len, const int* tiles,
                        int n_tiles, const float* dist_emb, int P, float* out, int64_t out_rows, int nh, int max_q_len,
                        int max_k_len, int terms, void* stream);

int e3d_relkey_attn_bwd_drop(const float* q, int64_t q_bs, int64_t q_rs, const float* k, int64_t k_bs,
                             int64_t k_rs, const float* v, int64_t v_bs, int64_t v_rs,
                             const float* dist_emb, int P, const float* key_mask, const float* out,
                             const float* lse, const float* dout, float* dq, int64_t dq_bs,
                             int64_t dq_rs, float* dk, int64_t dk_bs, int64_t dk_rs, float* dv,
                             int64_t dv_bs, int64_t dv_rs, float* d_dist_emb, float* workspace, int B,
                             int nh, int Lq, int Lk, float drop_p, uint64_t drop_seed, void* stream);

int e3d_relkey_attn_bwd_ex(const float* q, int64_t q_bs, int64_t q_rs, const float* k, int64_t k_bs,
                           int64_t k_rs, const float* v, int64_t v_bs, int64_t v_rs,
                           const float* dist_emb, int P, const float* key_mask, const float* out,
                           const float* lse, const float* dout, float* dq, int64_t dq_bs, int64_t dq_rs,
                           float* dk, int64_t dk_bs, int64_t dk_rs, float* dv, int64_t dv_bs,
                           int64_t dv_rs, float* d_dist_emb, float* workspace, int B, int nh, int Lq,
                           int Lk, int terms, float drop_p, uint64_t drop_seed, void* stream);

int e3d_attn_dropout_mask(int B, int nh, int Lq, int Lk, float p, uint64_t seed, float* out, void* stream);

int e3d_layernorm_bwd(const float* dy, const float* s, const float* gamma, float eps, float* ds,
                      float* dgamma, float* dbeta, int M, int H, void* stream);

int e3d_adaln_gate_bwd(const float* dout, const float* y, const float* mod, int branch,
                       int rows_per_cond, float* dy, float* dmod, int M, int H, void* stream);

int e3d_act_fwd(const float* z, int act, float* out, int64_t n, void* stream);
int e3d_act_bwd(const float* dh, const float* z, int act, float* dz, int64_t n, void* stream);

int e3d_colsum(const float* x, int64_t ld, float* out, int M, int N, void* stream);
int e3d_transpose_grouped_f32(const float* const* src, float* const* dst, int count, int rows, int cols, int64_t ld_src,
                              int64_t ld_dst, void* stream);
int e3d_group_sum(const float* x, int rows_per_group, float* out, int M, int H, void* stream);

int e3d_small_k_wgrad(const float* g, const float* x, float* dW, float* db, int M, int H, int F,
                      int transpose_out, void* stream);

int e3d_head_linear_bwd_dx(const float* dout, const float* W, float* dx, int M, int H, int Nout,
                           void* stream);

int e3d_residual_layernorm_drop_fwd(const float* x, const float* residual, const float* gamma, const float* beta, float eps,
                                    float* s_out, float* out, int M, int H, float drop_p, uint64_t drop_seed, void* stream);
int e3d_layernorm_bwd_drop(const float* dy, const float* s, const float* gamma, float eps, float* ds, float* ds_dropped,
                           float* dgamma, float* dbeta, int M, int H, float drop_p, uint64_t drop_seed, void* stream);
int64_t e3d_layernorm_bwd_workspace_floats(int M, int H);
int e3d_layernorm_bwd_ws(const float* dy, const float* s, const float* gamma, float eps, float* ds, float* ds_dropped,
                         float* dgamma, float* dbeta, int M, int H, float drop_p, uint64_t drop_seed, float* workspace,
                         int64_t workspace_floats, void* stream);

int64_t e3d_weight_planes_bytes(int N, int K);
int e3d_weight_planes_f32_split(const float* W, int N, int K, int terms, void* planes, void* stream);
int e3d_gemm_residual_layernorm_supported(int M, int N, int K, int64_t lda);
int e3d_gemm_residual_layernorm_f32_split(const float* A, int64_t lda, const void* w_planes, const float* bias,
                                          const float* residual, int64_t ldr, const float* gamma, const float* beta, float eps,
                                          float* out, int64_t ldo, int M, int N, int K, int terms, float out_scale, void* stream);

int e3d_adamw_step_dyn(float* const* params, const float* const* grads, float* const* exp_avg, float* const* exp_avg_sq,
                       const int64_t* numel, const int* chunk_tensor, const int64_t* chunk_first, int n_chunks,
                       const float* norm_and_clip, const float* lr_and_step, float beta1, float beta2, float eps,
                       float weight_decay, void* stream);
int e3d_adamw_step_dev(float* const* params, const float* const* grads, float* const* exp_avg, float* const* exp_avg_sq,
                       const int64_t* numel, const int* chunk_tensor, const int64_t* chunk_first, int n_chunks,
                       const float* norm_and_clip, const float* hyper, void* stream);
int e3d_dropout_set_epoch_ptr(const uint64_t* device_word);
int e3d_optim_chunk_elems(void);
int e3d_grad_global_norm(const float* const* grads, const int64_t* numel, const int* chunk_tensor, const int64_t* chunk_first,
                         int n_chunks, float max_norm, float* partial, float* norm_and_clip, void* stream);
int e3d_adamw_step(float* const* params, const float* const* grads, float* const* exp_avg, float* const* exp_avg_sq,
                   const int64_t* numel, const int* chunk_tensor, const int64_t* chunk_first, int n_chunks,
                   const float* norm_and_clip, float lr, float beta1, float beta2, float eps, float weight_decay, int step,
                   void* stream);

int e3d_keyed_drop_row_keys(const int64_t* ids, int B, int L, const int64_t* epoch_word, uint64_t seed, int stream,
                            uint64_t* out, void* st);
int e3d_dropout_f32_keyed(const float* x, float p, uint32_t site, const uint64_t* row_keys, float* out, int M, int H,
                          void* stream);
int e3d_keyed_attn_dropout_mask(int B, int nh, int Lq, int Lk, float p, uint32_t site, const uint64_t* row_keys, float* out,
                                void* stream);
int e3d_residual_layernorm_drop_fwd_keyed(const float* x, const float* residual, const float* gamma, const float* beta, float eps,
                                          float* s_out, float* out, int M, int H, float drop_p, uint32_t site,
                                          const uint64_t* row_keys, void* stream);
int e3d_layernorm_bwd_drop_keyed(const float* dy, const float* s, const float* gamma, float eps, float* ds, float* ds_dropped,
                                 float* dgamma, float* dbeta, int M, int H, float drop_p, uint32_t site, const uint64_t* row_keys,
                                 void* stream);
int e3d_layernorm_bwd_ws_keyed(const float* dy, const float* s, const float* gamma, float eps, float* ds, float* ds_dropped,
                               float* dgamma, float* dbeta, int M, int H, float drop_p, uint32_t site, const uint64_t* row_keys,
                               float* workspace, int64_t workspace_floats, void* stream);
int e3d_relkey_attn_fwd_split_drop_keyed(const float* q, int64_t q_bs, int64_t q_rs, const float* k, int64_t k_bs,
                                         int64_t k_rs, const float* v, int64_t v_bs, int64_t v_rs, const float* dist_emb,
                                         int P, const float* key_mask, float* out, float* lse, int B, int nh, int Lq, int Lk,
                                         int terms, float drop_p, uint32_t site, const uint64_t* row_keys, void* stream);
int e3d_relkey_attn_fwd_split_ex_keyed(const float* q, int64_t q_bs, int64_t q_rs, const float* k, int64_t k_bs,
                                       int64_t k_rs, const float* v, int64_t v_bs, int64_t v_rs, const float* dist_emb,
                                       int P, const float* key_mask, float* out, float* lse, int B, int nh, int Lq, int Lk,
                                       int terms, float drop_p, uint32_t site, const uint64_t* row_keys, void* e_scratch,
                                       int e_scratch_ready, const float* q_absmax, const float* k_absmax, float* e_absmax,
                                       void* stream);
int e3d_relkey_attn_bwd_drop_keyed(const float* q, int64_t q_bs, int64_t q_rs, const float* k, int64_t k_bs, int64_t k_rs,
                                   const float* v, int64_t v_bs, int64_t v_rs, const float* dist_emb, int P,
                                   const float* key_mask, const float* out, const float* lse, const float* dout, float* dq,
                                   int64_t dq_bs, int64_t dq_rs, float* dk, int64_t dk_bs, int64_t dk_rs, float* dv,
                                   int64_t dv_bs, int64_t dv_rs, float* d_dist_emb, float* workspace, int B, int nh, int Lq,
                                   int Lk, float drop_p, uint32_t site, const uint64_t* row_keys, void* stream);
int e3d_relkey_attn_bwd_ex_keyed(const float* q, int64_t q_bs, int64_t q_rs, const float* k, int64_t k_bs, int64_t k_rs,
                                 const float* v, int64_t v_bs, int64_t v_rs, const float* dist_emb, int P,
                                 const float* key_mask, const float* out, const float* lse, const float* dout, float* dq,
                                 int64_t dq_bs, int64_t dq_rs, float* dk, int64_t dk_bs, int64_t dk_rs, float* dv,
                                 int64_t dv_bs, int64_t dv_rs, float* d_dist_emb, float* workspace, int B, int nh, int Lq,
                                 int Lk, int terms, float drop_p, uint32_t site, const uint64_t* row_keys, void* stream);

#ifdef __cplusplus
}
#endif
#endif
```

Measured before the change: 4080 pocket-steps/s.

## Compute adaLN modulation from a one-hot residue table instead of per-token GEMMs

The receptor embedding layer's adaLN modulation is computed per token from the one-hot residue-sequence embedding, which costs two GEMMs over all M tokens (768->768 and 768->4608). This change classifies each row as one-hot or zero on the GPU. It computes the modulation for a small table of canonical rows, and the gate kernel gathers the modulation by index. The full per-token path still exists but only runs, via a device-side run_if flag, when some row is not one-hot. This needs extra kernels and launch planning keyed to the full M, so gated launches still cost launch overhead when they exit early.

```diff
diff --git a/e3-invaraint-diffusion-model_amd/blocks.py b/e3-invaraint-diffusion-model_amd/blocks.py
--- a/e3-invaraint-diffusion-model_amd/blocks.py
+++ b/e3-invaraint-diffusion-model_amd/blocks.py
@@ -4,9 +4,49 @@
 from torch import nn
 
 import contextlib
+import os
 
 from . import bert, keyed, ops
 from .autograd import functional as F
+
+ADALN_TABLE = os.environ.get("E3D_ADALN_TABLE", "1") == "1"
+TABLE_ROWS = 256
+_CANONICAL_ROWS = {}
+
+
+class IndexedModulation:
+
+    def __init__(self, idx, table, mod, other_rows):
+        self.idx, self.table, self.mod, self.other_rows = idx, table, mod, other_rows
+        self.shape = mod.shape
+
+
+def _canonical_rows(F_in, device):
+    key = (F_in, device)
+    t = _CANONICAL_ROWS.get(key)
+    if t is None:
+        t = torch.zeros(TABLE_ROWS, F_in, device=device, dtype=torch.float32)
+        t[:F_in] = torch.eye(F_in, device=device, dtype=torch.float32)
+        _CANONICAL_ROWS[key] = t
+    return t
+
+
+def onehot_modulation(layer, emb, x2d):
+    m0, m2 = layer.adaLN_modulation[0], layer.adaLN_modulation[2]
+    M, F_in = x2d.shape
+    H = m0.weight.shape[0]
+    params = (emb.linear.weight, emb.linear.bias, emb.LayerNorm.weight, emb.LayerNorm.bias, m0.weight, m0.bias, m2.weight, m2.bias)
+    if (not ADALN_TABLE or F_in >= TABLE_ROWS or F_in > 32 or not ops.gemm_is_tiled(M)
+            or (emb.training and emb.dropout.p > 0)
+            or (torch.is_grad_enabled() and any(t.requires_grad for t in params + (x2d,)))):
+        return None
+    ln = emb.LayerNorm
+    idx, other_rows = ops.classify_onehot_rows(x2d)
+    e = ops.embed_layernorm(_canonical_rows(F_in, x2d.device), emb.linear.weight, emb.linear.bias, ln.weight, ln.bias, ln.eps)
+    table = ops.gemm(ops.gemm(e, m0.weight, m0.bias, ops.ACT_SILU, plan_m=M), m2.weight, m2.bias, plan_m=M)
+    c = ops.embed_layernorm(x2d, emb.linear.weight, emb.linear.bias, ln.weight, ln.bias, ln.eps, run_if=other_rows)
+    mod = ops.gemm(ops.gemm(c, m0.weight, m0.bias, ops.ACT_SILU, run_if=other_rows), m2.weight, m2.bias, run_if=other_rows)
+    return IndexedModulation(idx, table, mod, other_rows)
 
 
 class SELayer(nn.Module):
@@ -43,10 +83,15 @@
         if row_keys is not None:
             drop = drop + (row_keys,)
         att = bert.run_self_attention(self.attn, x, mask, B, L, drop, layout=layout)
-        x = F.adaln_gate(x, att, mod, 0, rows_per_cond)
+        if isinstance(mod, IndexedModulation):
+            assert rows_per_cond == 1
+            gate = lambda a, y, branch: ops.adaln_gate_indexed(a, y, mod.idx, mod.table, mod.mod, branch)
+        else:
+            gate = lambda a, y, branch: F.adaln_gate(a, y, mod, branch, rows_per_cond)
+        x = gate(x, att, 0)
         h = F.dropout(F.linear(x, self.mlp[0].weight, self.mlp[0].bias, ops.ACT_GELU), self.mlp[2].p, self.training, row_keys)
         h = F.dropout(F.linear(h, self.mlp[3].weight, self.mlp[3].bias), self.mlp[4].p, self.training, row_keys)
-        return F.adaln_gate(x, h, mod, 1, rows_per_cond)
+        return gate(x, h, 1)
 
 
 class GaussianFourierProjection(nn.Module):
diff --git a/e3-invaraint-diffusion-model_amd/csrc/gemm_split.hip b/e3-invaraint-diffusion-model_amd/csrc/gemm_split.hip
--- a/e3-invaraint-diffusion-model_amd/csrc/gemm_split.hip
+++ b/e3-invaraint-diffusion-model_amd/csrc/gemm_split.hip
@@ -19,7 +19,7 @@
     return __builtin_amdgcn_mfma_f32_32x32x16_f16(a, b, c, 0, 0, 0);
 }
 
-struct Epi { float* absmax; float scale; };
+struct Epi { float* absmax; float scale; int plan_m = 0; const int* run_if = nullptr; };
 
 constexpr int BN = 128, BK = 32;
 #ifdef GEMM_STAMPS
@@ -470,7 +470,9 @@
                                                          const float* __restrict__ bias,
                                                          float* __restrict__ out, int64_t ldc, int M,
                                                          int N, int K_total, int tiles_m, int tiles_n,
-                                                         int k_chunk, float* __restrict__ absmax, float out_scale) {
+                                                         int k_chunk, float* __restrict__ absmax, float out_scale,
+                                                         const int* __restrict__ run_if) {
+    if (run_if && *run_if == 0) return;
     extern __shared__ __attribute__((aligned(16))) unsigned char smem_raw[];
     gemm_split_body<NS, ACT, A_KMAJ, B_KMAJ, WM, WN, E, TN, TR>(smem_raw, A, lda, Bm, ldb, bias, out, ldc, M, N, K_total, tiles_m,
                                                         tiles_n, k_chunk, xcd_remap(blockIdx.x, tiles_m * tiles_n),
@@ -549,8 +551,10 @@
                                                                         const float* __restrict__ bias,
                                                                         float* __restrict__ out, int64_t ldc,
                                                                         int M, int N, int K, int tiles_m,
-                                                                        int tiles_n, float* __restrict__ absmax, float out_scale) {
+                                                                        int tiles_n, float* __restrict__ absmax, float out_scale,
+                                                                        const int* __restrict__ run_if) {
     static_assert(!PIPE || NBUF == 2, "PIPE needs two LDS buffers");
+    if (run_if && *run_if == 0) return;
     STAMP_K(0);
     extern __shared__ __attribute__((aligned(16))) unsigned char smem_raw[];
     constexpr int NT = WR * WC * 64, TM = WR * 128, TN = WC * 64;
@@ -742,7 +746,9 @@
                                                                  const float* __restrict__ W,
                                                                  const float* __restrict__ bias,
                                                                  float* __restrict__ out, int64_t ldc, int N, int K,
-                                                                 int tiles_m, int tiles_n, float* __restrict__ absmax, float out_scale) {
+                                                                 int tiles_m, int tiles_n, float* __restrict__ absmax, float out_scale,
+                                                                 const int* __restrict__ run_if) {
+    if (run_if && *run_if == 0) return;
     extern __shared__ __attribute__((aligned(16))) unsigned char smem_raw[];
     constexpr int NS = 2, T_BYTES = BT * ROW64, BUF_BYTES = 2 * NS * T_BYTES;
     constexpr int NI = 8;
@@ -882,7 +888,7 @@
     const int total = tiles_m * tiles_n;
     e3d_allow_lds(lds_ok, gemm_split256p_kernel<ACT, E>, lds);
     hipLaunchKernelGGL((gemm_split256p_kernel<ACT, E>), dim3(total < n_cu ? total : n_cu), dim3(512), lds, s, A, lda, W, bias, out,
-                       ldc, N, K, tiles_m, tiles_n, epi.absmax, epi.scale);
+                       ldc, N, K, tiles_m, tiles_n, epi.absmax, epi.scale, epi.run_if);
     return e3d_launch_status("e3d_gemm_f32_split (persistent 256x256)");
 }
 
@@ -898,7 +904,7 @@
     static std::atomic<uint64_t> lds_ok{0};
     e3d_allow_lds(lds_ok, gemm_split256_kernel<NS, ACT, WR, WC, NBUF, PIPE, E>, lds);
     hipLaunchKernelGGL((gemm_split256_kernel<NS, ACT, WR, WC, NBUF, PIPE, E>), dim3(tiles_m * tiles_n), dim3(WR * WC * 64), lds, s,
-                       A, lda, W, bias, out, ldc, M, N, K, tiles_m, tiles_n, epi.absmax, epi.scale);
+                       A, lda, W, bias, out, ldc, M, N, K, tiles_m, tiles_n, epi.absmax, epi.scale, epi.run_if);
     return e3d_launch_status("e3d_gemm_f32_split (128x64 wave tiles)");
 }
 
@@ -922,21 +928,22 @@
         const char* e = getenv("E3D_GEMM_TILE");
         g_tile_pref = e ? atoi(e) : 4;
     }
+    const int Mp = epi.plan_m > 0 ? epi.plan_m : M;
     if constexpr (!A_KMAJ && !B_KMAJ) {
         if constexpr (NS == 2) {
-            const int64_t n_tiles = (int64_t)(M / BT) * (N / BT);
-            if (N % BT == 0 && M % BT == 0 && ldb == K && g_tile_pref >= 4 && K >= 2 * BK && lda < (1 << 22) &&
+            const int64_t n_tiles = (int64_t)(Mp / BT) * (N / BT);
+            if (N % BT == 0 && M % BT == 0 && Mp % BT == 0 && ldb == K && g_tile_pref >= 4 && K >= 2 * BK && lda < (1 << 22) &&
                 (g_tile_pref >= 5 || n_tiles >= p_min() || (n_tiles >= 96 && N >= 6 * BT && !getenv("E3D_GEMM_P_MIN"))))
                 return launch256p<ACT, E>(A, lda, B, bias, out, ldc, M, N, K, epi, s);
-            if (N % BT == 0 && ldb == K && g_tile_pref >= 3 && (int64_t)((M + BT - 1) / BT) * (N / BT) >= 256)
+            if (N % BT == 0 && ldb == K && g_tile_pref >= 3 && (int64_t)((Mp + BT - 1) / BT) * (N / BT) >= 256)
                 return launch256<NS, ACT, 2, 4, 2, true, E>(A, lda, B, bias, out, ldc, M, N, K, epi, s);
         }
         if constexpr (NS == 1) {
-            if (N % BT == 0 && ldb == K && g_tile_pref >= 3 && (int64_t)((M + BT - 1) / BT) * (N / BT) >= 160)
+            if (N % BT == 0 && ldb == K && g_tile_pref >= 3 && (int64_t)((Mp + BT - 1) / BT) * (N / BT) >= 160)
                 return launch256<NS, ACT, 2, 4, 2, true, E>(A, lda, B, bias, out, ldc, M, N, K, epi, s);
         }
         if (N % BT == 0 && ldb == K && g_tile_pref >= 1 &&
-            (int64_t)((M + BT - 1) / BT) * (N / BT) >= 256)
+            (int64_t)((Mp + BT - 1) / BT) * (N / BT) >= 256)
             return launch256<NS, ACT, 2, 4, (NS <= 2 ? 2 : 1), false, E>(A, lda, B, bias, out, ldc, M, N, K, epi, s);
     }
     if (g_general_form < 0) {
@@ -945,13 +952,13 @@
     }
     int form = g_general_form;
     if (form != 1 && form != 2 && form != 3 && form != 4) {
-        const int64_t g256 = (int64_t)((M + 255) / 256) * ((N + 127) / 128), g128 = (int64_t)((M + 127) / 128) * ((N + 127) / 128);
+        const int64_t g256 = (int64_t)((Mp + 255) / 256) * ((N + 127) / 128), g128 = (int64_t)((Mp + 127) / 128) * ((N + 127) / 128);
         const int64_t cus = e3d_cu_count();
         if (NS == 3) form = g256 < 128 && !A_KMAJ && !B_KMAJ ? 2 : 1;
         else if (A_KMAJ && B_KMAJ) form = 1;
         else if (A_KMAJ) form = g128 <= cus ? 2 : (g256 <= cus ? 1 : (45 * ((g128 + 2 * cus - 1) / (2 * cus)) < 37 * ((g256 + cus - 1) / cus) ? 2 : 1));
         else form = 25 * ((g128 + cus - 1) / cus) <= 38 * ((g256 + cus - 1) / cus) ? 3 : 1;
-        if (NS == 2 && !A_KMAJ && !B_KMAJ && M <= 2048 && N <= 1024) form = 4;
+        if (NS == 2 && !A_KMAJ && !B_KMAJ && Mp <= 2048 && N <= 1024) form = 4;
     }
     if constexpr (NS == 2 && !A_KMAJ && !B_KMAJ) {
         if (form == 4) return launch_general<NS, ACT, A_KMAJ, B_KMAJ, 2, 2, E, 1>(A, lda, B, ldb, bias, out, ldc, M, N, K, epi, s);
@@ -1006,7 +1013,7 @@
     }
     hipLaunchKernelGGL((gemm_split_kernel<NS, ACT, A_KMAJ, B_KMAJ, WM, WN, E, TN, TR>), dim3(tiles_m * tiles_n, splits),
                        dim3(WM * WN * 64), lds, s, A, lda, B, ldb, bias, out, ldc, M, N, K, tiles_m, tiles_n, k_chunk,
-                       splits > 1 ? nullptr : epi.absmax, epi.scale);
+                       splits > 1 ? nullptr : epi.absmax, epi.scale, epi.run_if);
     return e3d_launch_status("e3d_gemm_f32_split");
 }
 
@@ -1065,8 +1072,10 @@
 
 static int gemm_split_general(const float* A, int64_t lda, int a_kmajor, const float* B, int64_t ldb, int b_kmajor,
                               const float* bias, float* out, int64_t ldc, int M, int N, int K, int act, int terms,
-                              float* absmax, float out_scale, void* stream) {
-    const Epi epi{absmax, out_scale};
+                              float* absmax, float out_scale, void* stream, int plan_m = 0, const int* run_if = nullptr) {
+    const Epi epi{absmax, out_scale, plan_m, run_if};
+    E3D_REQUIRE(plan_m >= 0 && (!(a_kmajor || b_kmajor) || (plan_m == 0 && !run_if)),
+                "gemm_split: plan_m / run_if exist for the forward (K-contiguous) layout (plan_m=%d)", plan_m);
     E3D_REQUIRE(out_scale == 1.0f || !(a_kmajor && b_kmajor), "gemm_split: out_scale is not available for the split-K layout");
     E3D_REQUIRE(A && B && out, "gemm_split: null pointer");
     E3D_REQUIRE(M > 0 && N > 0 && K > 0, "gemm_split: bad shape M=%d N=%d K=%d", M, N, K);
@@ -1206,3 +1215,11 @@
     E3D_REQUIRE(N % BN == 0, "gemm_split: need N%%128==0 (N=%d)", N);
     return gemm_split_general(A, lda, 0, W, (int64_t)K, 0, bias, out, ldc, M, N, K, act, terms, out_absmax, out_scale, stream);
 }
+
+extern "C" int e3d_gemm_bias_act_f32_split_gated(const float* A, int64_t lda, const float* W, const float* bias, float* out,
+                                                 int64_t ldc, int M, int N, int K, int act, int terms, float* out_absmax,
+                                                 float out_scale, int plan_m, const int* run_if, void* stream) {
+    E3D_REQUIRE(N % BN == 0, "gemm_split: need N%%128==0 (N=%d)", N);
+    return gemm_split_general(A, lda, 0, W, (int64_t)K, 0, bias, out, ldc, M, N, K, act, terms, out_absmax, out_scale, stream,
+                              plan_m, run_if);
+}
diff --git a/e3-invaraint-diffusion-model_amd/csrc/rowops.hip b/e3-invaraint-diffusion-model_amd/csrc/rowops.hip
--- a/e3-invaraint-diffusion-model_amd/csrc/rowops.hip
+++ b/e3-invaraint-diffusion-model_amd/csrc/rowops.hip
@@ -95,12 +95,62 @@
 }
 
 template <int V>
+__global__ __launch_bounds__(256) void adaln_gate_indexed_kernel(const float* __restrict__ x, const float* __restrict__ y,
+                                                                 const int* __restrict__ idx, const float* __restrict__ table,
+                                                                 int table_rows, const float* __restrict__ mod, int branch,
+                                                                 float* __restrict__ out, int M) {
+    constexpr int H = 256 * V;
+    const int lane = threadIdx.x & 63;
+    const int row = blockIdx.x * 4 + (threadIdx.x >> 6);
+    if (row >= M) return;
+    f32x4 r[V], xr[V], sh[V], sc[V], ga[V];
+    row_load<V>(r, y + (int64_t)row * H, lane);
+    row_normalize<V>(r, 1e-5f);
+    const int t = idx[row];
+    const float* mrow = ((unsigned)t < (unsigned)table_rows ? table + (int64_t)t * 6 * H : mod + (int64_t)row * 6 * H) +
+                        (int64_t)branch * 3 * H;
+    row_load<V>(sh, mrow, lane);
+    row_load<V>(sc, mrow + H, lane);
+    row_load<V>(ga, mrow + 2 * H, lane);
+    row_load<V>(xr, x + (int64_t)row * H, lane);
+#pragma unroll
+    for (int i = 0; i < V; ++i) r[i] = xr[i] + ga[i] * (r[i] * (1.0f + sc[i]) + sh[i]);
+    row_store<V>(r, out + (int64_t)row * H, lane);
+}
+
+template <bool VEC>
+__global__ __launch_bounds__(256) void classify_onehot_kernel(const float* __restrict__ x, int F, int* __restrict__ idx,
+                                                              int* __restrict__ flag, int M) {
+    const int row = blockIdx.x * 256 + threadIdx.x;
+    if (row >= M) return;
+    const float* xr = x + (int64_t)row * F;
+    int nonzero = 0, ones = 0, pos = 0;
+    auto see = [&](float v, int f) {
+        nonzero += !(v == 0.0f);
+        if (v == 1.0f) { ++ones; pos = f; }
+    };
+    if (VEC) {
+        for (int f0 = 0; f0 < F; f0 += 4) {
+            const f32x4 v = *reinterpret_cast<const f32x4*>(xr + f0);
+#pragma unroll
+            for (int j = 0; j < 4; ++j) see(v[j], f0 + j);
+        }
+    } else {
+        for (int f = 0; f < F; ++f) see(xr[f], f);
+    }
+    const int k = nonzero == 0 ? F : (nonzero == 1 && ones == 1 ? pos : -1);
+    idx[row] = k;
+    if (k < 0) atomicOr(flag, 1);
+}
+
+template <int V>
 __global__ __launch_bounds__(256) void embed_layernorm_kernel(
     const float* __restrict__ x, int F, const float* __restrict__ W, const float* __restrict__ bias,
     const float* __restrict__ gamma, const float* __restrict__ beta, float eps,
     const float* __restrict__ post_add, int rows_per_add, float* __restrict__ z_out,
-    float* __restrict__ out, int M) {
-    constexpr int H = 256 * V;
+    float* __restrict__ out, int M, const int* __restrict__ run_if) {
+    constexpr int H = 256 * V;
+    if (run_if && *run_if == 0) return;
     extern __shared__ __attribute__((aligned(16))) float wt[];
     for (int i = threadIdx.x; i < H * F; i += blockDim.x) wt[(i % F) * H + i / F] = W[i];
     __syncthreads();
@@ -157,11 +207,11 @@
     const float* __restrict__ x, int F, const float* __restrict__ W, const float* __restrict__ bias,
     const float* __restrict__ gamma, const float* __restrict__ beta, float eps,
     const float* __restrict__ post_add, int rows_per_add, float* __restrict__ z_out,
-    float* __restrict__ out, int M) {
+    float* __restrict__ out, int M, const int* __restrict__ run_if) {
     constexpr int H = 256 * V;
     const int lane = threadIdx.x & 63;
     const int row = blockIdx.x * 4 + (threadIdx.x >> 6);
-    if (row >= M) return;
+    if (row >= M || (run_if && *run_if == 0)) return;
     const float* xr = x + (int64_t)row * F;
     f32x4 r[V], g[V], b[V];
     row_load<V>(r, bias, lane);
@@ -284,17 +334,17 @@
     return e3d_launch_status("e3d_adaln_gate_fwd");
 }
 
-extern "C" int e3d_embed_layernorm_fwd(const float* x, int F, const float* W, const float* b,
-                                       const float* gamma, const float* beta, float eps,
-                                       const float* post_add, int rows_per_add, float* z_out,
-                                       float* out, int M, int H, void* stream) {
+extern "C" int e3d_embed_layernorm_fwd_ex(const float* x, int F, const float* W, const float* b,
+                                          const float* gamma, const float* beta, float eps,
+                                          const float* post_add, int rows_per_add, float* z_out,
+                                          float* out, int M, int H, const int* run_if, void* stream) {
     E3D_REQUIRE(x && W && b && gamma && beta && out && M > 0, "embed_layernorm: bad arguments");
     E3D_REQUIRE(F >= 1 && F <= 32, "embed_layernorm: F must be in [1,32] (F=%d)", F);
     E3D_REQUIRE(!post_add || rows_per_add >= 1, "embed_layernorm: rows_per_add=%d", rows_per_add);
     if (M <= 512) {
         const dim3 grid((M + 3) / 4), block(256);
         DISPATCH_V(H, hipLaunchKernelGGL(embed_layernorm_rows_kernel<V>, grid, block, 0, (hipStream_t)stream, x, F, W, b,
-                                         gamma, beta, eps, post_add, rows_per_add, z_out, out, M));
+                                         gamma, beta, eps, post_add, rows_per_add, z_out, out, M, run_if));
         return e3d_launch_status("e3d_embed_layernorm_fwd");
     }
     int rpb = (M + 255) / 256;
@@ -307,9 +357,37 @@
         static std::atomic<uint64_t> lds_ok{0};
         e3d_allow_lds(lds_ok, embed_layernorm_kernel<V>, 32 * (size_t)H * sizeof(float));
         hipLaunchKernelGGL(embed_layernorm_kernel<V>, grid, block, lds, (hipStream_t)stream, x, F, W, b, gamma, beta,
-                           eps, post_add, rows_per_add, z_out, out, M);
+                           eps, post_add, rows_per_add, z_out, out, M, run_if);
     });
     return e3d_launch_status("e3d_embed_layernorm_fwd");
+}
+
+extern "C" int e3d_embed_layernorm_fwd(const float* x, int F, const float* W, const float* b,
+                                       const float* gamma, const float* beta, float eps,
+                                       const float* post_add, int rows_per_add, float* z_out,
+                                       float* out, int M, int H, void* stream) {
+    return e3d_embed_layernorm_fwd_ex(x, F, W, b, gamma, beta, eps, post_add, rows_per_add, z_out, out, M, H, nullptr, stream);
+}
+
+extern "C" int e3d_classify_onehot_rows(const float* x, int F, int* idx, int* flag, int M, void* stream) {
+    E3D_REQUIRE(x && idx && flag && M > 0, "classify_onehot_rows: bad arguments");
+    E3D_REQUIRE(F >= 1 && F <= 32, "classify_onehot_rows: F must be in [1,32] (F=%d)", F);
+    const dim3 grid((M + 255) / 256), block(256);
+    if (F % 4 == 0 && ((uintptr_t)x % 16) == 0)
+        hipLaunchKernelGGL(classify_onehot_kernel<true>, grid, block, 0, (hipStream_t)stream, x, F, idx, flag, M);
+    else
+        hipLaunchKernelGGL(classify_onehot_kernel<false>, grid, block, 0, (hipStream_t)stream, x, F, idx, flag, M);
+    return e3d_launch_status("e3d_classify_onehot_rows");
+}
+
+extern "C" int e3d_adaln_gate_indexed_fwd(const float* x, const float* y, const int* idx, const float* table, int table_rows,
+                                          const float* mod, int branch, float* out, int M, int H, void* stream) {
+    E3D_REQUIRE(x && y && idx && table && mod && out && M > 0 && table_rows > 0, "adaln_gate_indexed: bad arguments");
+    E3D_REQUIRE(branch == 0 || branch == 1, "adaln_gate_indexed: branch=%d", branch);
+    const dim3 grid((M + 3) / 4), block(256);
+    DISPATCH_V(H, hipLaunchKernelGGL(adaln_gate_indexed_kernel<V>, grid, block, 0, (hipStream_t)stream, x, y, idx, table,
+                                     table_rows, mod, branch, out, M));
+    return e3d_launch_status("e3d_adaln_gate_indexed_fwd");
 }
 
 extern "C" int e3d_head_linear_fwd(const float* x, const float* W, const float* b, float* out,
diff --git a/e3-invaraint-diffusion-model_amd/hip.py b/e3-invaraint-diffusion-model_amd/hip.py
--- a/e3-invaraint-diffusion-model_amd/hip.py
+++ b/e3-invaraint-diffusion-model_amd/hip.py
@@ -13,6 +13,8 @@
     "e3d_gemm_bias_act_f32": (c_int, [_P, c_int64, _P, _P, _P, c_int64, c_int, c_int, c_int, c_int, _P]),
     "e3d_gemm_bias_act_f32_split": (c_int, [_P, c_int64, _P, _P, _P, c_int64, c_int, c_int, c_int, c_int, c_int, _P]),
     "e3d_gemm_bias_act_f32_split_ex": (c_int, [_P, c_int64, _P, _P, _P, c_int64, c_int, c_int, c_int, c_int, c_int, _P, c_float, _P]),
+    "e3d_gemm_bias_act_f32_split_gated": (c_int, [_P, c_int64, _P, _P, _P, c_int64, c_int, c_int, c_int, c_int, c_int, _P, c_float,
+                                                  c_int, _P, _P]),
     "e3d_absmax_f32": (c_int, [_P, c_int64, _P, _P]),
     "e3d_relkey_attn_fwd": (c_int, [_P, c_int64, c_int64, _P, c_int64, c_int64, _P, c_int64, c_int64,
                                     _P, c_int, _P, _P, _P, c_int, c_int, c_int, c_int, _P]),
@@ -33,6 +35,9 @@
     "e3d_residual_layernorm_fwd": (c_int, [_P, _P, _P, _P, c_float, _P, _P, c_int, c_int, _P]),
     "e3d_adaln_gate_fwd": (c_int, [_P, _P, _P, c_int, c_int, _P, c_int, c_int, _P]),
     "e3d_embed_layernorm_fwd": (c_int, [_P, c_int, _P, _P, _P, _P, c_float, _P, c_int, _P, _P, c_int, c_int, _P]),
+    "e3d_adaln_gate_indexed_fwd": (c_int, [_P, _P, _P, _P, c_int, _P, c_int, _P, c_int, c_int, _P]),
+    "e3d_classify_onehot_rows": (c_int, [_P, c_int, _P, _P, c_int, _P]),
+    "e3d_embed_layernorm_fwd_ex": (c_int, [_P, c_int, _P, _P, _P, _P, c_float, _P, c_int, _P, _P, c_int, c_int, _P, _P]),
     "e3d_nerf_backbone": (c_int, [_P, _P, _P, c_int, c_int, c_int, _P]),
     "e3d_gemm_f32_split_general": (c_int, [_P, c_int64, c_int, _P, c_int64, c_int, _P, _P, c_int64, c_int, c_int,
                                            c_int, c_int, c_int, _P]),
diff --git a/e3-invaraint-diffusion-model_amd/ops.py b/e3-invaraint-diffusion-model_amd/ops.py
--- a/e3-invaraint-diffusion-model_amd/ops.py
+++ b/e3-invaraint-diffusion-model_amd/ops.py
@@ -205,7 +205,12 @@
             and -(-M // 32) * (N // 32) <= SKINNY_MAX_TILES)
 
 
-def gemm(a, weight, bias=None, act=ACT_NONE, out=None, mode=None, absmax=None, prescale=True):
+def gemm_is_tiled(M, mode=None):
+    terms = GEMM_MODES[GEMM_MODE if mode is None else mode]
+    return terms != 0 and not (terms in (3, 19) and M <= min(SKINNY_MAX_M, SKINNY_GEMM_MAX_M))
+
+
+def gemm(a, weight, bias=None, act=ACT_NONE, out=None, mode=None, absmax=None, prescale=True, plan_m=None, run_if=None):
     _chk(a, "gemm.a"); _chk(weight, "gemm.weight"); _chk(bias, "gemm.bias")
     assert a.dim() == 2 and a.stride(1) == 1 and weight.is_contiguous()
     M, K = a.shape
@@ -221,6 +226,16 @@
     scale = 1.0
     if terms == 19 and prescale:
         weight, scale = f16_weight(weight)
+    if plan_m is not None or run_if is not None:
+        _chk(run_if, "gemm.run_if", torch.int32)
+        plan_m = M if plan_m is None else plan_m
+        if not gemm_is_tiled(plan_m, mode):
+            raise ValueError(f"gemm: plan_m / run_if exist on the tiled split kernels only (plan_m={plan_m}, mode={mode or GEMM_MODE})")
+        with _timed("gemm" if run_if is None else "gemm_gated", (M, N, K, act)):
+            hip.check(hip.lib().e3d_gemm_bias_act_f32_split_gated(
+                _p(a), a.stride(0), _p(weight), _p(bias), _p(out), out.stride(0), M, N, K, act, terms, _p(absmax), scale,
+                plan_m, _p(run_if), _stream()), "e3d_gemm_bias_act_f32_split_gated")
+        return out
     with _timed("gemm", (M, N, K, act)):
         if _skinny_ok(terms, M, N, K, a) and out.stride(0) % 4 == 0 and M <= min(SKINNY_MAX_M, SKINNY_GEMM_MAX_M):
             ws = _skinny_workspace(a.device, M, N, K)
@@ -582,7 +597,34 @@
     return out
 
 
-def embed_layernorm(x, weight, bias, gamma, beta, eps, post_add=None, rows_per_add=1, want_z=False):
+def adaln_gate_indexed(x, y, idx, table, mod, branch):
+    for n, t in (("x", x), ("y", y), ("table", table), ("mod", mod)):
+        _chk(t, "adaln_gate_indexed." + n)
+    _chk(idx, "adaln_gate_indexed.idx", torch.int32)
+    assert x.is_contiguous() and y.is_contiguous() and mod.is_contiguous() and table.is_contiguous() and idx.is_contiguous()
+    M, H = x.shape
+    assert y.shape == x.shape and mod.shape == (M, 6 * H) and table.shape[1] == 6 * H and idx.shape == (M,), (mod.shape, table.shape, idx.shape)
+    out = torch.empty_like(x)
+    with _timed("adaln_gate", (M, H)):
+        hip.check(hip.lib().e3d_adaln_gate_indexed_fwd(_p(x), _p(y), _p(idx), _p(table), table.shape[0], _p(mod), branch,
+                                                       _p(out), M, H, _stream()), "e3d_adaln_gate_indexed_fwd")
+    return out
+
+
+def classify_onehot_rows(x, flag=None):
+    _chk(x, "classify_onehot_rows.x")
+    assert x.dim() == 2 and x.is_contiguous()
+    M, F = x.shape
+    if flag is None:
+        flag = torch.zeros(1, device=x.device, dtype=torch.int32)
+    _chk(flag, "classify_onehot_rows.flag", torch.int32)
+    idx = torch.empty(M, device=x.device, dtype=torch.int32)
+    with _timed("classify_onehot", (M, F)):
+        hip.check(hip.lib().e3d_classify_onehot_rows(_p(x), F, _p(idx), _p(flag), M, _stream()), "e3d_classify_onehot_rows")
+    return idx, flag
+
+
+def embed_layernorm(x, weight, bias, gamma, beta, eps, post_add=None, rows_per_add=1, want_z=False, run_if=None):
     for n, t in (("x", x), ("weight", weight), ("bias", bias), ("gamma", gamma), ("beta", beta),
                  ("post_add", post_add)):
         _chk(t, "embed_layernorm." + n)
@@ -594,10 +636,11 @@
         assert post_add.is_contiguous() and post_add.shape == (M // rows_per_add, H)
     out = torch.empty((M, H), device=x.device, dtype=torch.float32)
     z = torch.empty_like(out) if want_z else None
+    _chk(run_if, "embed_layernorm.run_if", torch.int32)
     with _timed("embed_layernorm", (M, H)):
-        hip.check(hip.lib().e3d_embed_layernorm_fwd(_p(x), F, _p(weight), _p(bias), _p(gamma), _p(beta), eps,
-                                                    _p(post_add), rows_per_add, _p(z), _p(out), M, H, _stream()),
-                  "e3d_embed_layernorm_fwd")
+        hip.check(hip.lib().e3d_embed_layernorm_fwd_ex(_p(x), F, _p(weight), _p(bias), _p(gamma), _p(beta), eps,
+                                                       _p(post_add), rows_per_add, _p(z), _p(out), M, H, _p(run_if),
+                                                       _stream()), "e3d_embed_layernorm_fwd_ex")
     return (out, z) if want_z else out
 
 
diff --git a/e3-invaraint-diffusion-model_amd/structure_model/model.py b/e3-invaraint-diffusion-model_amd/structure_model/model.py
--- a/e3-invaraint-diffusion-model_amd/structure_model/model.py
+++ b/e3-invaraint-diffusion-model_amd/structure_model/model.py
@@ -6,7 +6,7 @@
 
 from .. import bert, keyed, ops
 from ..blocks import (BertEmbeddings, GaussianFourierProjection, KeyedDropoutSwitch, Predictor, SELayer, drop_row_keys,
-                      flat2d, require_gpu)
+                      flat2d, onehot_modulation, require_gpu)
 from ..training import adamw
 import os
 
@@ -44,16 +44,20 @@
         ops.reset_absmax(receptor_angles.device)
         if layout is not None:
             ang = self.receptor_angle_emb.run(flat2d(layout.pack(receptor_angles)))
-            seq = self.receptor_seq_emb.run(flat2d(layout.pack(receptor_seq)))
-            x = self.receptor_emb.run(ang, seq, None, 1, layout.rows, layout=layout)
+            seq2d = flat2d(layout.pack(receptor_seq))
+            mod = onehot_modulation(self.receptor_emb, self.receptor_seq_emb, seq2d)
+            seq = self.receptor_seq_emb.run(seq2d) if mod is None else None
+            x = self.receptor_emb.run(ang, seq, None, 1, layout.rows, mod=mod, layout=layout)
             x = bert.run_encoder(self.encoder, x, None, 1, layout.rows, layout=layout)
             kv = [bert.project_cross_kv(layer.crossattention, x) for layer in self.decoder.layer] if project_cross_kv else None
             return ReceptorCache(x, kv, None, B, L, layout=layout)
         mask = receptor_attention_masks.contiguous().float()
         rk = drop_row_keys(keyed.DROP_POCKET, L)
         ang = self.receptor_angle_emb.run(flat2d(receptor_angles), row_keys=rk)
-        seq = self.receptor_seq_emb.run(flat2d(receptor_seq), row_keys=rk)
-        x = self.receptor_emb.run(ang, seq, mask, B, L, row_keys=rk)
+        seq2d = flat2d(receptor_seq)
+        mod = onehot_modulation(self.receptor_emb, self.receptor_seq_emb, seq2d)
+        seq = self.receptor_seq_emb.run(seq2d, row_keys=rk) if mod is None else None
+        x = self.receptor_emb.run(ang, seq, mask, B, L, mod=mod, row_keys=rk)
         x = bert.run_encoder(self.encoder, x, mask, B, L, row_keys=rk)
         kv = None
         if project_cross_kv:
diff --git a/include/e3d_hip.h b/include/e3d_hip.h
--- a/include/e3d_hip.h
+++ b/include/e3d_hip.h
@@ -31,6 +31,9 @@
 int e3d_gemm_bias_act_f32_split_ex(const float* A, int64_t lda, const float* W, const float* bias, float* out,
                                    int64_t ldc, int M, int N, int K, int act, int terms, float* out_absmax,
                                    float out_scale, void* stream);
+int e3d_gemm_bias_act_f32_split_gated(const float* A, int64_t lda, const float* W, const float* bias, float* out,
+                                      int64_t ldc, int M, int N, int K, int act, int terms, float* out_absmax,
+                                      float out_scale, int plan_m, const int* run_if, void* stream);
 int e3d_absmax_f32(const float* x, int64_t n, float* target, void* stream);
 
 int e3d_relkey_attn_fwd(const float* q, int64_t q_bs, int64_t q_rs,
@@ -78,10 +81,19 @@
 int e3d_adaln_gate_fwd(const float* x, const float* y, const float* mod, int branch,
                        int rows_per_cond, float* out, int M, int H, void* stream);
 
+int e3d_adaln_gate_indexed_fwd(const float* x, const float* y, const int* idx, const float* table, int table_rows,
+                               const float* mod, int branch, float* out, int M, int H, void* stream);
+
+int e3d_classify_onehot_rows(const float* x, int F, int* idx, int* flag, int M, void* stream);
+
 int e3d_embed_layernorm_fwd(const float* x, int F, const float* W, const float* b,
                             const float* gamma, const float* beta, float eps,
                             const float* post_add, int rows_per_add, float* z_out, float* out,
                             int M, int H, void* stream);
+int e3d_embed_layernorm_fwd_ex(const float* x, int F, const float* W, const float* b,
+                               const float* gamma, const float* beta, float eps,
+                               const float* post_add, int rows_per_add, float* z_out, float* out,
+                               int M, int H, const int* run_if, void* stream);
 
 int e3d_head_linear_fwd(const float* x, const float* W, const float* b, float* out, int M,
                         int H, int Nout, void* stream);
```

New measurement: 4183 pocket-steps/s (median of 6 runs). +2.5%, better.
